# chunhualiao/Smith-Waterman

Measured on AMD Instinct MI355X. Metric: GCUPS (DP cell updates/s) on NxN random DNA pair, higher is better.
Workload: dtype int32; 1 GPU; 16384x16384 random DNA pair (reference generator, seed 1+rank), linear gap 3/-3/-2, int32 H + int32 P written to HBM, arg-max tracked; per_gpu=one pair per GPU, max_pos=268369846, max_score=11583, grid=256, column_tiles=1, strips=131, placement_held_gib=0, preheat_fills=640

## Files before the change

smith-waterman_amd/csrc/sw_api.hip:

```cpp
#include <hip/hip_runtime.h>
#include <algorithm>
#include <chrono>
#include <cstdio>
#include <cstdlib>
#include <cstring>
#include <iterator>
#include <map>
#include <mutex>
#include <string>
#include <thread>
#include <vector>
#include "sw_kernels.h"
#include "sw_plan.h"

namespace swh { void set_err(const char* fmt, ...); }
extern "C" int sw_place_pair_ratio(void* d_X, size_t xbytes, void* d_Y, size_t ybytes, float* ratio, float* ms_together);
using swh::set_err;

#define HIP_TRY(expr)                                                                 \
    do {                                                                              \
        hipError_t e_ = (expr);                                                       \
        if (e_ != hipSuccess) {                                                       \
            set_err("%s failed: %s (%s:%d)", #expr, hipGetErrorString(e_), __FILE__, __LINE__); \
            return SW_EDEVICE;                                                        \
        }                                                                             \
    } while (0)

struct DevState {
    std::mutex mu;
    bool any = false;
    hipStream_t last_stream = nullptr;
    hipEvent_t ev = nullptr;
    int concurrent_ok = 0;
};
static DevState g_dev[64];

struct sw_ctx {
    int device = 0;
    int num_cus = 256;
    unsigned epoch = 0;
    unsigned long long* d_edge = nullptr;
    size_t edge_cap = 0;
    unsigned long long* d_key = nullptr;
    unsigned long long* d_keys = nullptr; size_t keys_cap = 0;
    unsigned char* d_cb = nullptr;
    size_t cb_cap = 0;
    unsigned int* d_edge4 = nullptr;
    size_t edge4_cap = 0;
    unsigned epoch8 = 0;
    unsigned char* d_alpha = nullptr;
    unsigned int* d_part = nullptr;
    unsigned int* d_sync = nullptr;
    unsigned char* d_priv = nullptr; size_t priv_cap = 0;
    int64_t opt_place_hold_gib = 0;
    int64_t opt_place_budget_ms = 1500;
    int place_spacer_gib = 0;
    int64_t last_place_held_gib = 0;
    float last_place_ratio = 0.f;
    bool key_dirty = false;
    bool last_fused = false;
    swp::PlanOptions opt;
    swp::FillPlan last_plan;
    int64_t last_grid = 0;
    int s2_per_cu = 0;
    int64_t opt_xcd_order = 0;
    int64_t opt_pace_ps = 0;
    int64_t opt_dbg_ptr = 0;
    int64_t opt_band_wait_ms = 20000;
    unsigned char* d_bcodes = nullptr; size_t bcodes_cap = 0;
    int* d_bnd = nullptr; size_t bnd_cap = 0;
    int64_t opt_batch_lds = 0;
    int64_t last_batch_kernel = 0;
    signed char* d_sprof = nullptr; size_t sprof_cap = 0;
    int* d_sbnd = nullptr; size_t sbnd_cap = 0;
    swk::SearchItem* d_sitems = nullptr; swk::SearchItem* h_sitems = nullptr; size_t sitems_cap = 0;
    hipEvent_t sitems_ev = nullptr;
    unsigned int* d_sctr = nullptr;
    int64_t last_search_grid = 0;
    int search_per_cu[swp::kSearchKernels] = {};
    bool search_per_cu_known = false;
    bool xcd_round_robin = false;
    std::map<void*, void*> out_base;
    std::map<void*, float> pair_ratio;
};

template <typename K> struct Indexed { int index; K k; };
template <typename K, size_t N> constexpr bool at_their_indices(const Indexed<K> (&t)[N]) {
    for (size_t i = 0; i < N; ++i)
        if (t[i].index != (int)i) return false;
    return true;
}

extern "C" {

int sw_create(int device, sw_ctx** out) {
    if (!out) { set_err("sw_create: out is NULL"); return SW_EINVAL; }
    int n = 0;
    if (hipGetDeviceCount(&n) != hipSuccess || n <= 0) { set_err("sw_create: no HIP device"); return SW_ENODEV; }
    if (device < 0 || device >= n) { set_err("sw_create: device %d out of range (%d)", device, n); return SW_EINVAL; }
    HIP_TRY(hipSetDevice(device));
    sw_ctx* c = new sw_ctx();
    c->device = device;
    hipDeviceProp_t prop;
    HIP_TRY(hipGetDeviceProperties(&prop, device));
    c->num_cus = prop.multiProcessorCount;
    HIP_TRY(hipMalloc((void**)&c->d_key, 64));
    HIP_TRY(hipMemset(c->d_key, 0, 64));
    HIP_TRY(hipMalloc((void**)&c->d_alpha, 2048));
    HIP_TRY(hipMemset(c->d_alpha, 0, 2048));
    HIP_TRY(hipMalloc((void**)&c->d_part, 2048 * 32));
    HIP_TRY(hipMalloc((void**)&c->d_sync, 256));
    HIP_TRY(hipMemset(c->d_sync, 0, 256));
    if (c->num_cus == 256) {
        unsigned int h[256];
        hipLaunchKernelGGL(swk::sw_xcc_probe, dim3(256), dim3(768), 0, nullptr, c->d_part);
        if (hipMemcpy(h, c->d_part, sizeof h, hipMemcpyDeviceToHost) == hipSuccess) {
            c->xcd_round_robin = true;
            for (int i = 0; i < 256; ++i) c->xcd_round_robin = c->xcd_round_robin && h[i] == (unsigned)(i & 7);
        } else {
            (void)hipGetLastError();
        }
    }
    *out = c;
    return SW_OK;
}

void sw_destroy(sw_ctx* c) {
    if (!c) return;
    (void)hipSetDevice(c->device);
    if (c->d_edge) (void)hipFree(c->d_edge);
    if (c->d_key) (void)hipFree(c->d_key);
    if (c->d_cb) (void)hipFree(c->d_cb);
    if (c->d_edge4) (void)hipFree(c->d_edge4);
    if (c->d_alpha) (void)hipFree(c->d_alpha);
    if (c->d_part) (void)hipFree(c->d_part);
    if (c->d_sync) (void)hipFree(c->d_sync);
    if (c->d_priv) (void)hipFree(c->d_priv);
    if (c->d_keys) (void)hipFree(c->d_keys);
    if (c->d_bcodes) (void)hipFree(c->d_bcodes);
    if (c->d_bnd) (void)hipFree(c->d_bnd);
    if (c->sitems_ev) { (void)hipEventSynchronize(c->sitems_ev); (void)hipEventDestroy(c->sitems_ev); }
    if (c->d_sprof) (void)hipFree(c->d_sprof);
    if (c->d_sbnd) (void)hipFree(c->d_sbnd);
    if (c->d_sitems) (void)hipFree(c->d_sitems);
    if (c->h_sitems) (void)hipHostFree(c->h_sitems);
    if (c->d_sctr) (void)hipFree(c->d_sctr);
    delete c;
}

int sw_set_option(sw_ctx* c, const char* name, int64_t v) {
    if (!c || !name) { set_err("sw_set_option: bad argument"); return SW_EINVAL; }
    if (!strcmp(name, "waves_per_block")) {
        if (v != 0 && v != 1 && v != 2 && v != 4 && v != 8) { set_err("waves_per_block must be 1,2,4,8"); return SW_EINVAL; }
        c->opt.waves_per_block = v ? v : 4;
        return SW_OK;
    }
    if (!strcmp(name, "max_blocks")) { c->opt.max_blocks = v < 0 ? 0 : v; return SW_OK; }
    if (!strcmp(name, "strips_per_group")) { c->opt.strips_per_group = v; return SW_OK; }
    if (!strcmp(name, "consumers")) { c->opt.consumers = v; return SW_OK; }
    if (!strcmp(name, "debug_flags")) { c->opt.debug_flags = v; return SW_OK; }
    if (!strcmp(name, "xcd_chain")) { c->opt.xcd_chain = v; return SW_OK; }
    if (!strcmp(name, "filler_hop_ps")) { c->opt.filler_hop_ps = v < 0 ? 0 : v; return SW_OK; }
    if (!strcmp(name, "filler_tau_ps")) { c->opt.filler_tau_ps = v < 1000 ? 1000 : v; return SW_OK; }
    if (!strcmp(name, "filler_bw_gbs")) { c->opt.filler_bw_gbs = v < 100 ? 100 : v; return SW_OK; }
    if (!strcmp(name, "pace_ps")) { c->opt_pace_ps = v; return SW_OK; }
    if (!strcmp(name, "store_policy")) { if (v < 0 || v > 2) return SW_EINVAL; c->opt.store_policy = v; return SW_OK; }
    if (!strcmp(name, "xcd_order")) { c->opt_xcd_order = v ? 1 : 0; return SW_OK; }
    if (!strcmp(name, "importers")) { if (v < 0 || v > 8) return SW_EINVAL; c->opt.importers = v; return SW_OK; }
    if (!strcmp(name, "debug_buf")) { c->opt_dbg_ptr = v; return SW_OK; }
    if (!strcmp(name, "batch_lds")) { c->opt_batch_lds = v < 0 ? 0 : v; return SW_OK; }
    if (!strcmp(name, "band_wait_ms")) { c->opt_band_wait_ms = v > 0 ? v : 20000; return SW_OK; }
    if (!strcmp(name, "placement_budget_ms")) { c->opt_place_budget_ms = v > 0 ? v : 1500; return SW_OK; }
    if (!strcmp(name, "placement_hold_gib")) { c->opt_place_hold_gib = v < 0 ? 0 : (v > 128 ? 128 : v); return SW_OK; }
    if (!strcmp(name, "probe_foreign_pairs")) { c->opt.probe_foreign_pairs = v ? 1 : 0; return SW_OK; }
    if (!strcmp(name, "s2w")) { if (v != 0 && v != 126 && v != 110) return SW_EINVAL; c->opt.s2w = v; return SW_OK; }
    if (!strcmp(name, "split_blk")) { c->opt.split_blk = v > 0 ? v : 0; return SW_OK; }
    if (!strcmp(name, "split_from")) { c->opt.split_from = v > 0 ? v : 0; return SW_OK; }
    if (!strcmp(name, "debug_epoch8")) { c->epoch8 = (unsigned)(v & 255); return SW_OK; }
    if (!strcmp(name, "engine")) {
        if (v != 0 && v != 1) { set_err("engine must be 0 (systolic) or 1 (strip_scan)"); return SW_EINVAL; }
        c->opt.engine = v;
        return SW_OK;
    }
    set_err("sw_set_option: unknown option '%s'", name);
    return SW_EINVAL;
}

int64_t sw_get_option(sw_ctx* c, const char* name) {
    if (!c || !name) return -1;
    if (!strcmp(name, "waves_per_block")) return c->opt.waves_per_block;
    if (!strcmp(name, "max_blocks")) return c->opt.max_blocks;
    if (!strcmp(name, "engine")) return c->opt.engine;
    if (!strcmp(name, "strips_per_group")) return c->opt.strips_per_group;
    if (!strcmp(name, "consumers")) return c->opt.consumers;
    if (!strcmp(name, "store_policy")) return c->opt.store_policy;
    if (!strcmp(name, "xcd_order")) return c->opt_xcd_order;
    if (!strcmp(name, "importers")) return c->opt.importers;
    if (!strcmp(name, "pace_ps")) return c->opt_pace_ps;
    if (!strcmp(name, "band_wait_ms")) return c->opt_band_wait_ms;
    if (!strcmp(name, "num_cus")) return c->num_cus;
    if (!strcmp(name, "debug_edge4_ptr")) return (int64_t)(uintptr_t)c->d_edge4;
    if (!strcmp(name, "debug_edge4_cap")) return (int64_t)c->edge4_cap;
    if (!strcmp(name, "last_grid")) return c->last_grid;
    const swp::TilePlan& last_tile = c->last_plan.tile[c->last_plan.ntile - 1];
    if (!strcmp(name, "last_strips")) return c->last_plan.S;
    if (!strcmp(name, "last_strips2")) return last_tile.strips;
    if (!strcmp(name, "last_scouts")) return last_tile.nscout;
    if (!strcmp(name, "last_xcd_mode")) return last_tile.xcd_mode;
    if (!strcmp(name, "last_tiles")) return c->last_plan.ntile;
    if (!strcmp(name, "last_split_from")) return last_tile.split_blk ? last_tile.split_from : 0;
    if (!strcmp(name, "xcd_round_robin")) return c->xcd_round_robin ? 1 : 0;
    if (!strcmp(name, "last_batch_kernel")) return c->last_batch_kernel;
    if (!strcmp(name, "last_search_grid")) return c->last_search_grid;
    if (!strcmp(name, "placement_budget_ms")) return c->opt_place_budget_ms;
    if (!strcmp(name, "placement_hold_gib")) return c->opt_place_hold_gib;
    if (!strcmp(name, "probe_foreign_pairs")) return c->opt.probe_foreign_pairs;
    if (!strcmp(name, "last_placement_held_gib")) return c->last_place_held_gib;
    if (!strcmp(name, "last_placement_ratio_x1000")) return (int64_t)(c->last_place_ratio * 1000.f);
    return -1;
}

static int check_dims(int64_t cols, int64_t rows, const sw_scores* sc, int64_t gc = -1, int64_t gr = -1) {
    if (gc < cols) gc = cols;
    if (gr < rows) gr = rows;
    if (cols < 0 || rows < 0 || cols > swk::SW_MAX_DIM || rows > swk::SW_MAX_DIM || gc > swk::SW_MAX_DIM || gr > swk::SW_MAX_DIM) {
        set_err("dimensions out of range: cols=%lld rows=%lld (max %lld)", (long long)cols, (long long)rows,
                (long long)swk::SW_MAX_DIM);
        return SW_EINVAL;
    }
    if (sc->gap > 0) { set_err("gap score must be <= 0 (got %d)", sc->gap); return SW_EINVAL; }
    if (sc->match < 0) { set_err("match score must be >= 0 (got %d)", sc->match); return SW_EINVAL; }
    if (sc->mismatch > sc->match) { set_err("mismatch score must not exceed the match score"); return SW_EINVAL; }
    const int64_t lo = std::min(gc, gr);
    const int64_t gmax = (int64_t)sc->match * lo + (int64_t)(-sc->gap) * (rows + cols + 2);
    const int64_t step = std::max<int64_t>(std::llabs((int64_t)sc->mismatch), (int64_t)sc->match) + 2 * (int64_t)(-sc->gap);
    if (gmax + step >= (1ll << 31) || step >= (1ll << 24) || (int64_t)sc->match * lo >= (1ll << 24)) {
        set_err("scores too large for this problem size (32-bit cell / 24-bit arg-max key)");
        return SW_EINVAL;
    }
    return SW_OK;
}

struct FillJob {
    const char* d_a; int64_t cols; const char* d_b; int64_t rows;
    void* d_H; int h_elem_bytes; void* d_P; int64_t stride;
    const int32_t* d_top; const int32_t* d_left; int32_t* d_right;
    int64_t npairs; int64_t a_pstride, b_pstride, hp_pstride;
    unsigned long long* d_keys;
    int p_elem_bytes = 4;
    const unsigned long long* d_top_gran = nullptr; unsigned long long* d_bot_gran = nullptr; unsigned int* d_bot_done = nullptr;
    unsigned int top_tag = 0, bot_tag = 0;
    int reserve_cus = 0;
    bool concurrent = false;
    int64_t total_rows = 0;
    bool zero_key = false;
    sw_result* d_result = nullptr;
};

static int order_after_previous_fill(DevState& d, hipStream_t stream, bool allow_concurrent) {
    if (d.any && d.last_stream != stream && !allow_concurrent && d.ev) HIP_TRY(hipStreamWaitEvent(stream, d.ev, 0));
    return SW_OK;
}

struct DevOrder {
    std::unique_lock<std::mutex> lk;
    DevState& d;
    hipStream_t stream;
    int rc;
    DevOrder(sw_ctx* c, hipStream_t st, bool concurrent) : lk(g_dev[c->device & 63].mu), d(g_dev[c->device & 63]), stream(st) {
        rc = order_after_previous_fill(d, stream, concurrent);
    }
    ~DevOrder() {
        if (!d.ev && hipEventCreateWithFlags(&d.ev, hipEventDisableTiming) != hipSuccess) { d.ev = nullptr; (void)hipGetLastError(); }
        if (d.ev && hipEventRecord(d.ev, stream) == hipSuccess) { d.any = true; d.last_stream = stream; }
        else { (void)hipGetLastError(); d.any = false; }
    }
};

static int grow_workspace(void** buf, size_t& cap, size_t need, size_t elem, size_t slack, hipStream_t stream, bool& fresh) {
    fresh = false;
    if (need <= cap) return SW_OK;
    HIP_TRY(hipStreamSynchronize(stream));
    if (*buf) HIP_TRY(hipFree(*buf));
    *buf = nullptr; cap = 0;
    const size_t bytes = need * elem + slack;
    if (hipMalloc(buf, bytes) != hipSuccess) { set_err("workspace allocation of %zu bytes failed", bytes); return SW_ENOMEM; }
    cap = need; fresh = true;
    return SW_OK;
}

static int ensure_workspaces(sw_ctx* c, const swp::FillPlan& f, hipStream_t stream) {
    bool fresh = false;
    if (int rc = grow_workspace((void**)&c->d_edge, c->edge_cap, f.edge_need, 8, 0, stream, fresh)) return rc;
    if (fresh) { HIP_TRY(hipMemsetAsync(c->d_edge, 0, c->edge_cap * 8, stream)); c->epoch = 0; }
    if (int rc = grow_workspace((void**)&c->d_cb, c->cb_cap, f.cb_need, 4, 64, stream, fresh)) return rc;
    if (int rc = grow_workspace((void**)&c->d_edge4, c->edge4_cap, f.edge4_need, 4, 0, stream, fresh)) return rc;
    if (fresh) c->epoch8 = 255;
    return grow_workspace((void**)&c->d_priv, c->priv_cap, f.priv_need, 1, 0, stream, fresh);
}

static unsigned next_gbias(sw_ctx* c, hipStream_t stream) {
    if (++c->epoch8 >= (unsigned)((c->opt.debug_flags & swk::DBG_EPOCH8_WRAP_EARLY) ? 4 : 256)) {
        const unsigned nb = (unsigned)std::max<size_t>(1, std::min<size_t>((c->edge4_cap + 255) / 256, 2048));
        hipLaunchKernelGGL(swk::sw_wipe_u32, dim3(nb), dim3(256), 0, stream, c->d_edge4, c->edge4_cap);
        c->epoch8 = 1;
    }
    return (c->epoch8 << 24) | 0x10000u;
}

static swp::DeviceFacts device_facts(const sw_ctx* c) {
    swp::DeviceFacts dev;
    dev.num_cus = c->num_cus; dev.xcd_round_robin = c->xcd_round_robin; dev.s2_per_cu = c->s2_per_cu;
    std::copy(std::begin(c->search_per_cu), std::end(c->search_per_cu), dev.search_per_cu);
    return dev;
}

static int plan_for(sw_ctx* c, const swp::PlanJob& pj, swp::FillPlan& plan) {
    if (c->opt.engine == 0 && c->s2_per_cu < 1)
        HIP_TRY(hipOccupancyMaxActiveBlocksPerMultiprocessor(&c->s2_per_cu, swk::sw_systolic2<6, false>, 768, 0));
    plan = swp::plan_fill(pj, device_facts(c), c->opt);
    return SW_OK;
}

using SystolicKernel = void (*)(const unsigned char*, const unsigned char*, const unsigned char*, swk::FillParams);
static const struct { int ns, nc; SystolicKernel h32, h64; } kSystolic[] = {
    {2, 2, swk::sw_systolic<int32_t, 2, 2>, swk::sw_systolic<int64_t, 2, 2>}, {2, 3, swk::sw_systolic<int32_t, 2, 3>, swk::sw_systolic<int64_t, 2, 3>},
    {2, 4, swk::sw_systolic<int32_t, 2, 4>, swk::sw_systolic<int64_t, 2, 4>}, {1, 2, swk::sw_systolic<int32_t, 1, 2>, swk::sw_systolic<int64_t, 1, 2>},
    {1, 3, swk::sw_systolic<int32_t, 1, 3>, swk::sw_systolic<int64_t, 1, 3>}, {1, 4, swk::sw_systolic<int32_t, 1, 4>, swk::sw_systolic<int64_t, 1, 4>},
    {1, 6, swk::sw_systolic<int32_t, 1, 6>, swk::sw_systolic<int64_t, 1, 6>}, {1, 7, swk::sw_systolic<int32_t, 1, 7>, swk::sw_systolic<int64_t, 1, 7>},
};
using Systolic2Kernel = void (*)(const unsigned char*, const unsigned char*, swk::FillParams);
static const Systolic2Kernel kSystolic2[4][2] = {
    {swk::sw_systolic2<4, false>, swk::sw_systolic2<4, true>}, {swk::sw_systolic2<5, false>, swk::sw_systolic2<5, true>},
    {swk::sw_systolic2<6, false>, swk::sw_systolic2<6, true>}, {swk::sw_systolic2<7, false>, swk::sw_systolic2<7, true>},
};

static swp::PlanJob plan_job(const FillJob& j, const sw_scores* sc) {
    swp::PlanJob pj;
    pj.cols = j.cols; pj.rows = j.rows; pj.npairs = j.npairs; pj.full_stride = j.stride == j.cols + 1;
    pj.h_elem_bytes = j.h_elem_bytes; pj.p_elem_bytes = j.p_elem_bytes; pj.has_H = j.d_H; pj.has_P = j.d_P;
    pj.has_top = j.d_top; pj.has_left = j.d_left; pj.has_right = j.d_right; pj.has_top_gran = j.d_top_gran; pj.has_bot_gran = j.d_bot_gran;
    pj.has_result = j.d_result; pj.total_rows = j.total_rows; pj.reserve_cus = j.reserve_cus;
    pj.h_aligned = ((uintptr_t)j.d_H & (j.h_elem_bytes == 8 ? 15u : 7u)) == 0; pj.p_aligned = ((uintptr_t)j.d_P & 7u) == 0;
    pj.match = sc->match; pj.mismatch = sc->mismatch; pj.gap = sc->gap;
    return pj;
}

static int launch_fill(sw_ctx* c, const sw_scores* sc, const FillJob& j, hipStream_t stream) {
    const int64_t cols = j.cols, rows = j.rows;
    const bool systolic = (c->opt.engine == 0);
    c->last_fused = false;
    const bool tile_features = j.d_left || j.d_right || j.stride != cols + 1 || j.npairs != 1 || !j.d_H || !j.d_P || j.d_top_gran || j.d_bot_gran;
    if (!systolic && tile_features) { set_err("tiles / batches / bands / matrix-less fills need the systolic engine (engine 0)"); return SW_EINVAL; }
    if (j.p_elem_bytes == 1 && !systolic) { set_err("compact (int8) P needs the systolic engine"); return SW_EINVAL; }
    if (((uintptr_t)j.d_b & 15) != 0 || (j.b_pstride & 15) != 0) { set_err("d_b (and the batch stride of b) must be 16-byte aligned"); return SW_EINVAL; }
    swp::PlanJob pj = plan_job(j, sc);
    auto known = j.d_P ? c->pair_ratio.find(j.d_P) : c->pair_ratio.end();
    if (known != c->pair_ratio.end()) pj.pair_ratio = known->second;
    swp::FillPlan plan;
    if (int rc = plan_for(c, pj, plan)) return rc;
    if (plan.probe_pair_class) {
        float r = 0.f, ms = 0.f;
        if (c->pair_ratio.size() >= 64) c->pair_ratio.clear();
        if (hipStreamSynchronize(stream) == hipSuccess && sw_place_pair_ratio(j.d_H, plan.h_bytes, j.d_P, plan.p_bytes, &r, &ms) == SW_OK) {
            c->pair_ratio[j.d_P] = pj.pair_ratio = r;
            if (int rc = plan_for(c, pj, plan)) return rc;
        }
    }
    const auto* one_col = systolic ? std::find_if(std::begin(kSystolic), std::end(kSystolic), [&](const auto& k) { return k.ns == plan.NS && k.nc == plan.NC; })
                                   : std::end(kSystolic);
    if (systolic && one_col == std::end(kSystolic)) { set_err("unsupported strips_per_group/consumers combination %d/%d", plan.NS, plan.NC); return SW_EINVAL; }
    if (int rc = ensure_workspaces(c, plan, stream)) return rc;
    if (++c->epoch >= 4096) {
        HIP_TRY(hipMemsetAsync(c->d_edge, 0, c->edge_cap * 8, stream));
        c->epoch = 1;
    }
    c->last_plan = plan;
    const int64_t S = plan.S;
    swk::FillParams p;
    memset(&p, 0, sizeof p);
    p.cols = cols; p.rows = rows; p.M = j.stride;
    p.H = j.d_H; p.P = (int32_t*)j.d_P; p.top = j.d_top; p.left = j.d_left; p.right = j.d_right;
    p.top_gran = j.d_top_gran; p.bot_gran = j.d_bot_gran; p.bot_done = j.d_bot_done; p.top_tag = j.top_tag; p.bot_tag = j.bot_tag;
    p.top_wait_ticks = (unsigned)std::min<int64_t>(0x7fffffff, c->opt_band_wait_ms * 100000 >> 10);
    p.mm = sc->match - 2 * sc->gap; p.xm = sc->mismatch - 2 * sc->gap; p.ngap = -sc->gap;
    p.edge = c->d_edge; p.tag_base = c->epoch << 20;
    p.result_key = j.d_keys; p.abort_flag = (unsigned int*)(c->d_key + 1);
    p.nstrips = (int)S;
    p.debug_flags = (int)c->opt.debug_flags;
    p.pace_ps = (int)c->opt_pace_ps;
    p.store_nt = plan.store_nt;
    p.xcd_order = (int)c->opt_xcd_order;
    p.dbg = (unsigned long long*)(uintptr_t)c->opt_dbg_ptr;
    p.npairs = (int)j.npairs; p.store_hp = (j.d_H || j.d_P) ? 1 : 0;
    p.p_bytes = j.p_elem_bytes;
    p.a_pstride = j.a_pstride; p.b_pstride = j.b_pstride; p.hp_pstride = j.hp_pstride;
    p.edge_pstride = S * (rows + 1);
    const unsigned char* ua = (const unsigned char*)j.d_a;
    const unsigned char* ub = (const unsigned char*)j.d_b;
    if (!systolic) {
        c->key_dirty = true;
        c->last_grid = plan.grid;
        if (j.h_elem_bytes == 4)
            hipLaunchKernelGGL((swk::sw_strip_scan<int32_t, 16>), dim3(plan.grid), dim3(plan.threads), 0, stream, ua, ub, p);
        else
            hipLaunchKernelGGL((swk::sw_strip_scan<int64_t, 16>), dim3(plan.grid), dim3(plan.threads), 0, stream, ua, ub, p);
        HIP_TRY(hipGetLastError());
        return SW_OK;
    }
    const size_t cb16 = ((c->cb_cap + 15) / 16) * 16;
    unsigned short* d_cb16 = (unsigned short*)(c->d_cb + cb16);
    unsigned char* d_cbc = c->d_cb + cb16 + ((2 * c->cb_cap + 15) / 16) * 16;
    if (plan.perm) {
        p.edge4 = c->d_edge4; p.e4stride = plan.e4stride; p.edge4_pstride = S * plan.e4stride;
        p.gbias = next_gbias(c, stream);
    }
    p.bcode = d_cbc;
    p.atab = c->d_alpha + 64;
    p.phi_base = plan.fast ? (int)S - 1 : -1;
    p.bfront = (int)plan.bfront;
    p.bpad16 = d_cb16;
    p.bpad8 = c->d_cb;
    p.bpad_pstride = plan.per;
    if (plan.two_cols) {
        if (c->key_dirty) { HIP_TRY(hipMemsetAsync(c->d_key, 0, 16, stream)); c->key_dirty = false; }
        for (int64_t tile = 0; tile < plan.ntile; ++tile) {
            const swp::TilePlan& t = plan.tile[tile];
            swk::FillParams p2 = p;
            p2.nstrips = (int)t.strips; p2.cols = t.cols; p2.h_bytes = j.h_elem_bytes; p2.s2w = plan.W2; p2.store_nt = t.store_nt;
            p2.alpha_a = ua; p2.alpha_cols = cols;
            p2.idx_off = t.c0; p2.final_launch = tile + 1 == plan.ntile ? 1 : 0;
            if (plan.ntile > 1) {
                p2.H = (char*)j.d_H + t.c0 * 4; p2.P = (int32_t*)((char*)j.d_P + t.c0 * 4);
                p2.tile_left = tile ? (const int32_t*)j.d_H + t.c0 : nullptr;
                if (tile) p2.gbias = next_gbias(c, stream);
            }
            p2.nscout = t.nscout; p2.scout_double = t.scout_double; p2.xcd_mode = t.xcd_mode;
            p2.split_blk = t.split_blk; p2.split_from = t.split_from; p2.split_extra = t.split_extra;
            p2.filler_end_steps = t.filler_end_steps; p2.filler_full_steps = t.filler_full_steps;
            p2.filler_hop_ps = t.filler_hop_ps; p2.filler_tau_ps = t.filler_tau_ps; p2.filler_bw_gbs = t.filler_bw_gbs;
            p2.sync = c->d_sync; p2.priv = c->d_priv; p2.priv_stride = plan.priv_stride;
            p2.bpad16_w = d_cb16; p2.bpad8_w = c->d_cb; p2.bcode_w = d_cbc; p2.atab_w = c->d_alpha + 64;
            p2.result = j.d_result; p2.skip_row0 = (j.d_top || j.d_top_gran) ? 1 : 0;
            hipLaunchKernelGGL(kSystolic2[t.consumers - 4][plan.W2 == 110], dim3(t.grid), dim3(768), 0, stream, ua + t.c0, ub, p2);
        }
        p.skip_if_perm = 1;
        p.sync = c->d_sync; p.atab_w = c->d_alpha + 64; p.result = j.d_result; p.final_launch = 1;
        c->last_fused = true;
    } else {
        const int64_t total = (cols + rows) * j.npairs;
        const unsigned nscan = (unsigned)std::max<int64_t>(1, std::min<int64_t>((total + 1023) / 1024, 2048));
        hipLaunchKernelGGL(swk::sw_prep_scan, dim3(nscan), dim3(256), 0, stream, ua, cols, j.a_pstride, ub, rows, j.b_pstride, j.npairs, c->d_part);
        const unsigned npad = (unsigned)((plan.per + 255) / 256);
        hipLaunchKernelGGL(swk::sw_prep_code, dim3(npad, (unsigned)j.npairs), dim3(256), 0, stream, ub, rows, plan.bfront, j.b_pstride, c->d_cb, d_cb16,
                           d_cbc, (const unsigned int*)c->d_part, (int)nscan, c->d_alpha + 64, plan.per, (int)npad, (void*)nullptr, j.h_elem_bytes,
                           (void*)nullptr, j.p_elem_bytes, cols + 1, rows + 1, 0, j.zero_key ? j.d_keys : nullptr);
        c->key_dirty = true;
    }
    const SystolicKernel kern = j.h_elem_bytes == 4 ? one_col->h32 : one_col->h64;
    int per_cu = 0;
    HIP_TRY(hipOccupancyMaxActiveBlocksPerMultiprocessor(&per_cu, kern, plan.threads, 0));
    if (per_cu < 1) { set_err("the fill kernel does not fit a CU on this device"); return SW_EDEVICE; }
    c->last_grid = std::min<int64_t>(plan.grid, (int64_t)per_cu * c->num_cus);
    hipLaunchKernelGGL(kern, dim3((unsigned)c->last_grid), dim3(plan.threads), 0, stream, ua, ub, (const unsigned char*)c->d_cb, p);
    HIP_TRY(hipGetLastError());
    return SW_OK;
}

static const sw_scores kDefaultScores = {3, -3, -2};

static int fill_one(sw_ctx* c, const sw_scores* scores, FillJob j, int64_t gcols, int64_t grows, sw_result* d_result, void* stream_,
                    const char* who) {
    const sw_scores* sc = scores ? scores : &kDefaultScores;
    const int64_t cols = j.cols, rows = j.rows;
    if (!c || !d_result || (j.h_elem_bytes != 4 && j.h_elem_bytes != 8) || (j.p_elem_bytes != 4 && j.p_elem_bytes != 1) ||
        j.stride < cols + 1) {
        set_err("%s: bad argument", who);
        return SW_EINVAL;
    }
    if (int rc = check_dims(cols, rows, sc, gcols, grows)) return rc;
    if ((cols > 0 && !j.d_a) || (rows > 0 && !j.d_b)) { set_err("%s: NULL sequence", who); return SW_EINVAL; }
    hipStream_t stream = (hipStream_t)stream_;
    HIP_TRY(hipSetDevice(c->device));
    DevOrder order(c, stream, j.concurrent);
    if (order.rc) return order.rc;
    j.d_keys = c->d_key;
    j.d_result = d_result;
    j.zero_key = c->opt.engine == 0 && cols > 0 && rows > 0;
    if (!j.zero_key) { HIP_TRY(hipMemsetAsync(c->d_key, 0, 16, stream)); c->key_dirty = true; }
    c->last_fused = false;
    if (cols == 0 || rows == 0) {
        if (j.stride != cols + 1 || j.d_left || j.d_right || j.d_top_gran || j.d_bot_gran) { set_err("%s: empty tiles / bands are not supported", who); return SW_EINVAL; }
        const int64_t M = cols + 1;
        if (j.d_H) HIP_TRY(hipMemsetAsync(j.d_H, 0, (size_t)(M * (rows + 1)) * j.h_elem_bytes, stream));
        if (j.d_P) HIP_TRY(hipMemsetAsync(j.d_P, 0, (size_t)(M * (rows + 1)) * j.p_elem_bytes, stream));
        if (j.d_H && j.d_top && j.h_elem_bytes == 4) HIP_TRY(hipMemcpyAsync(j.d_H, j.d_top, (size_t)M * 4, hipMemcpyDeviceToDevice, stream));
        if (j.d_H && j.d_top && j.h_elem_bytes == 8) { set_err("top halo with an empty int64 band is unsupported"); return SW_EINVAL; }
    } else {
        if (int rc = launch_fill(c, sc, j, stream)) return rc;
    }
    if (!c->last_fused) hipLaunchKernelGGL(swk::sw_finalize, dim3(1), dim3(64), 0, stream, c->d_key, (const unsigned int*)(c->d_key + 1), d_result, 1);
    HIP_TRY(hipGetLastError());
    return SW_OK;
}

static FillJob make_job(const char* d_a, int64_t cols, const char* d_b, int64_t rows, void* d_H, int h_elem_bytes, void* d_P, int p_elem_bytes,
                        int64_t row_stride, const int32_t* d_top, const int32_t* d_left, int32_t* d_right) {
    FillJob j = {d_a, cols, d_b, rows, d_H, h_elem_bytes, d_P, row_stride, d_top, d_left, d_right, 1, 0, 0, 0, nullptr};
    j.p_elem_bytes = p_elem_bytes;
    return j;
}

int sw_fill_tile_device(sw_ctx* c, const char* d_a, int64_t cols, const char* d_b, int64_t rows, const sw_scores* scores,
                        void* d_H, int h_elem_bytes, int32_t* d_P, int64_t row_stride, const int32_t* d_top,
                        const int32_t* d_left, int32_t* d_right, sw_result* d_result, void* stream_) {
    if (!d_H || !d_P) { set_err("sw_fill_tile_device: bad argument"); return SW_EINVAL; }
    return fill_one(c, scores, make_job(d_a, cols, d_b, rows, d_H, h_elem_bytes, d_P, 4, row_stride, d_top, d_left, d_right), -1, -1, d_result,
                    stream_, "sw_fill_tile_device");
}

int sw_fill_device(sw_ctx* c, const char* d_a, int64_t cols, const char* d_b, int64_t rows, const sw_scores* scores,
                   void* d_H, int h_elem_bytes, int32_t* d_P, const int32_t* d_top, sw_result* d_result, void* stream_) {
    if (!d_H || !d_P) { set_err("sw_fill_device: bad argument"); return SW_EINVAL; }
    return fill_one(c, scores, make_job(d_a, cols, d_b, rows, d_H, h_elem_bytes, d_P, 4, cols + 1, d_top, nullptr, nullptr), -1, -1, d_result,
                    stream_, "sw_fill_device");
}

int sw_fill_device_ex(sw_ctx* c, const char* d_a, int64_t cols, const char* d_b, int64_t rows, const sw_scores* scores,
                      void* d_H, int h_elem_bytes, void* d_P, int p_elem_bytes, const int32_t* d_top, sw_result* d_result,
                      void* stream_) {
    return fill_one(c, scores, make_job(d_a, cols, d_b, rows, d_H, h_elem_bytes, d_P, p_elem_bytes, cols + 1, d_top, nullptr, nullptr), -1, -1,
                    d_result, stream_, "sw_fill_device_ex");
}

int sw_fill_band_device(sw_ctx* c, const char* d_a, int64_t cols, const char* d_b, int64_t rows, int64_t total_rows,
                        const sw_scores* scores, void* d_H, int h_elem_bytes, void* d_P, int p_elem_bytes,
                        const uint64_t* d_top_gran, uint32_t top_tag, uint64_t* d_bot_gran, uint32_t bot_tag, uint32_t* d_bot_done,
                        int reserve_cus, int concurrent, sw_result* d_result, void* stream_) {
    if ((d_top_gran && top_tag == 0) || (d_bot_gran && bot_tag == 0) || (d_bot_done && !d_bot_gran) || reserve_cus < 0 || total_rows < rows) {
        set_err("sw_fill_band_device: bad argument");
        return SW_EINVAL;
    }
    if (c && c->opt.engine != 0) { set_err("sw_fill_band_device needs the systolic engine"); return SW_EINVAL; }
    FillJob j = make_job(d_a, cols, d_b, rows, d_H, h_elem_bytes, d_P, p_elem_bytes, cols + 1, nullptr, nullptr, nullptr);
    j.d_top_gran = (const unsigned long long*)d_top_gran; j.d_bot_gran = (unsigned long long*)d_bot_gran; j.d_bot_done = d_bot_done;
    j.top_tag = top_tag; j.bot_tag = bot_tag; j.reserve_cus = reserve_cus; j.concurrent = concurrent != 0; j.total_rows = total_rows;
    return fill_one(c, scores, j, cols, total_rows, d_result, stream_, "sw_fill_band_device");
}

using BatchKernel = void (*)(swk::BatchParams);
static constexpr Indexed<BatchKernel> kBatch[] = {
    {swp::batch_wave_index(4, 0), swk::sw_batch_wave<4, 0>}, {swp::batch_wave_index(4, 1), swk::sw_batch_wave<4, 1>},
    {swp::batch_wave_index(4, 4), swk::sw_batch_wave<4, 4>}, {swp::batch_wave_index(8, 0), swk::sw_batch_wave<8, 0>},
    {swp::batch_wave_index(8, 1), swk::sw_batch_wave<8, 1>}, {swp::batch_wave_index(8, 4), swk::sw_batch_wave<8, 4>},
    {swp::batch_wave_index(16, 0), swk::sw_batch_wave<16, 0>}, {swp::batch_wave_index(16, 1), swk::sw_batch_wave<16, 1>},
    {swp::batch_wave_index(16, 4), swk::sw_batch_wave<16, 4>},
    {swp::batch_wave16_index(false, false, false), swk::sw_batch_wave16<false, false, false>},
    {swp::batch_wave16_index(false, false, true), swk::sw_batch_wave16<false, false, true>},
    {swp::batch_wave16_index(false, true, false), swk::sw_batch_wave16<false, true, false>},
    {swp::batch_wave16_index(false, true, true), swk::sw_batch_wave16<false, true, true>},
    {swp::batch_wave16_index(true, false, false), swk::sw_batch_wave16<true, false, false>},
    {swp::batch_wave16_index(true, false, true), swk::sw_batch_wave16<true, false, true>},
    {swp::batch_wave16_index(true, true, false), swk::sw_batch_wave16<true, true, false>},
    {swp::batch_wave16_index(true, true, true), swk::sw_batch_wave16<true, true, true>},
};
static_assert(std::size(kBatch) == swp::kBatchKernels && at_their_indices(kBatch));

static int batch_one_pair_per_wave(sw_ctx* c, const swp::BatchPlan& plan, const char* d_a, int64_t a_stride, int64_t cols, const char* d_b,
                                   int64_t b_stride, int64_t rows, int64_t npairs, const sw_scores* sc, int32_t* d_H, void* d_P, int p_elem_bytes,
                                   sw_result* d_results, hipStream_t stream) {
    bool fresh = false;
    if (int rc = grow_workspace((void**)&c->d_bcodes, c->bcodes_cap, plan.bcodes_need, 1, 64, stream, fresh)) return rc;
    if (int rc = grow_workspace((void**)&c->d_bnd, c->bnd_cap, plan.bnd_need, 4, 0, stream, fresh)) return rc;
    const unsigned char* ua = (const unsigned char*)d_a;
    const unsigned char* ub = (const unsigned char*)d_b;
    hipLaunchKernelGGL(swk::sw_prep_scan, dim3((unsigned)plan.scan_blocks), dim3(256), 0, stream, ua, cols, a_stride, ub, rows, b_stride, npairs, c->d_part);
    hipLaunchKernelGGL(swk::sw_prep_reduce, dim3(1), dim3(256), 0, stream, c->d_part, plan.scan_blocks);
    if (plan.bnd_need) HIP_TRY(hipMemsetAsync(c->d_bnd, 0, plan.bnd_need * 4, stream));
    const int64_t cells = (cols + 1) * (rows + 1);
    const int pb = d_P ? p_elem_bytes : 0;
    unsigned int nletters = 0;
    for (int64_t k0 = 0; k0 < npairs; k0 += plan.chunk) {
        const int64_t n = std::min(plan.chunk, npairs - k0);
        hipLaunchKernelGGL(swk::sw_batch_codes, dim3((unsigned)plan.codes_blocks, (unsigned)std::min<int64_t>(n, 65535)), dim3(256), 0, stream,
                           ub + k0 * b_stride, rows, b_stride, c->d_bcodes, plan.per, plan.front, (const unsigned int*)c->d_part, 1, c->d_alpha + 64, n);
        HIP_TRY(hipGetLastError());
        if (k0 == 0) {
            HIP_TRY(hipMemcpyAsync(&nletters, c->d_alpha + 64 + 256, 4, hipMemcpyDeviceToHost, stream));
            HIP_TRY(hipStreamSynchronize(stream));
        }
        const int k = swp::batch_kernel(plan, nletters, n, pb);
        if (k < 0) return 1;
        swk::BatchParams bp;
        memset(&bp, 0, sizeof bp);
        bp.a = ua + k0 * a_stride; bp.a_pstride = a_stride; bp.cols = cols;
        bp.bcode = c->d_bcodes; bp.bcode_pstride = plan.per; bp.bfront = plan.front;
        bp.rows = rows; bp.npairs = n; bp.atab = c->d_alpha + 64;
        bp.H = d_H ? d_H + k0 * cells : nullptr;
        bp.P = d_P ? (void*)((char*)d_P + k0 * cells * p_elem_bytes) : nullptr;
        bp.hp_pstride = cells;
        bp.match = sc->match; bp.mismatch = sc->mismatch; bp.ngap = -sc->gap;
        bp.bnd = c->d_bnd; bp.bnd_pstride = plan.bnd_per;
        bp.results = d_results + k0;
        bp.debug = (int)(c->opt.debug_flags & swk::DBG_BATCH_MASK);
        const bool two = k >= swp::kBatchWave16;
        const int64_t per_block = two ? 8 : 4;
        hipLaunchKernelGGL(kBatch[k].k, dim3((unsigned)((n + per_block - 1) / per_block)), dim3(256), two ? 0 : (size_t)c->opt_batch_lds, stream, bp);
        HIP_TRY(hipGetLastError());
        if (two) c->last_batch_kernel = 2;
    }
    if (c->last_batch_kernel != 2) c->last_batch_kernel = 1;
    c->last_grid = plan.grid; c->last_plan.S = plan.nstrips;
    return SW_OK;
}

int sw_fill_band_reserve(sw_ctx* c, int64_t cols, int64_t rows, int64_t total_rows, const sw_scores* scores, int h_elem_bytes, int p_elem_bytes, int want_h,
                         void* stream_) {
    const sw_scores* sc = scores ? scores : &kDefaultScores;
    if (!c || cols <= 0 || rows <= 0) { set_err("sw_fill_band_reserve: bad argument"); return SW_EINVAL; }
    if (c->opt.engine != 0) { set_err("sw_fill_band_reserve needs the systolic engine"); return SW_EINVAL; }
    if (int rc = check_dims(cols, rows, sc, cols, total_rows)) return rc;
    HIP_TRY(hipSetDevice(c->device));
    swp::PlanJob pj;
    pj.cols = cols; pj.rows = rows; pj.total_rows = total_rows; pj.h_elem_bytes = h_elem_bytes; pj.p_elem_bytes = p_elem_bytes; pj.has_H = want_h != 0;
    pj.has_top_gran = pj.has_bot_gran = true;
    pj.match = sc->match; pj.mismatch = sc->mismatch; pj.gap = sc->gap;
    swp::FillPlan plan;
    if (int rc = plan_for(c, pj, plan)) return rc;
    std::unique_lock<std::mutex> lk(g_dev[c->device & 63].mu);
    if (int rc = ensure_workspaces(c, plan, (hipStream_t)stream_)) return rc;
    HIP_TRY(hipStreamSynchronize((hipStream_t)stream_));
    return SW_OK;
}

int sw_batch_device_ex(sw_ctx* c, const char* d_a, int64_t a_stride, int64_t cols, const char* d_b, int64_t b_stride, int64_t rows,
                       int64_t npairs, const sw_scores* scores, int32_t* d_H, void* d_P, int p_elem_bytes, sw_result* d_results,
                       void* stream_) {
    const sw_scores* sc = scores ? scores : &kDefaultScores;
    if (!c || !d_a || !d_b || !d_results || npairs <= 0 || cols <= 0 || rows <= 0 || a_stride < cols || b_stride < rows ||
        (p_elem_bytes != 4 && p_elem_bytes != 1)) {
        set_err("sw_batch_device: bad argument");
        return SW_EINVAL;
    }
    if (c->opt.engine != 0) { set_err("sw_batch_device needs the systolic engine"); return SW_EINVAL; }
    if (int rc = check_dims(cols, rows, sc)) return rc;
    hipStream_t stream = (hipStream_t)stream_;
    HIP_TRY(hipSetDevice(c->device));
    DevOrder order(c, stream, false);
    if (order.rc) return order.rc;
    swp::BatchJob bj;
    bj.cols = cols; bj.rows = rows; bj.npairs = npairs; bj.has_H = d_H; bj.has_P = d_P; bj.p_elem_bytes = p_elem_bytes;
    bj.match = sc->match; bj.mismatch = sc->mismatch; bj.gap = sc->gap;
    const swp::BatchPlan plan = swp::plan_batch(bj, c->opt);
    c->last_batch_kernel = 0;
    if (plan.wave) {
        int rc = batch_one_pair_per_wave(c, plan, d_a, a_stride, cols, d_b, b_stride, rows, npairs, sc, d_H, d_P, p_elem_bytes, d_results, stream);
        if (rc != 1) return rc;
    }
    bool fresh = false;
    if (int rc = grow_workspace((void**)&c->d_keys, c->keys_cap, (size_t)plan.single_chunk, 8, 0, stream, fresh)) return rc;
    HIP_TRY(hipMemsetAsync(c->d_key, 0, 16, stream));
    c->key_dirty = true;
    const int64_t cells = (cols + 1) * (rows + 1);
    for (int64_t k0 = 0; k0 < npairs; k0 += plan.single_chunk) {
        const int64_t n = std::min(plan.single_chunk, npairs - k0);
        HIP_TRY(hipMemsetAsync(c->d_keys, 0, (size_t)n * 8, stream));
        FillJob j = {d_a + k0 * a_stride, cols, d_b + k0 * b_stride, rows, d_H ? (void*)(d_H + k0 * cells) : nullptr, 4,
                     d_P ? (void*)((char*)d_P + k0 * cells * p_elem_bytes) : nullptr, cols + 1, nullptr, nullptr, nullptr, n, a_stride, b_stride,
                     cells, c->d_keys};
        j.p_elem_bytes = p_elem_bytes;
        if (int rc = launch_fill(c, sc, j, stream)) return rc;
        hipLaunchKernelGGL(swk::sw_finalize, dim3((unsigned)((n + 63) / 64)), dim3(64), 0, stream, c->d_keys,
                           (const unsigned int*)(c->d_key + 1), d_results + k0, (int)n);
        HIP_TRY(hipGetLastError());
    }
    return SW_OK;
}
int sw_batch_device(sw_ctx* c, const char* d_a, int64_t a_stride, int64_t cols, const char* d_b, int64_t b_stride, int64_t rows,
                    int64_t npairs, const sw_scores* scores, int32_t* d_H, int32_t* d_P, sw_result* d_results, void* stream_) {
    return sw_batch_device_ex(c, d_a, a_stride, cols, d_b, b_stride, rows, npairs, scores, d_H, d_P, 4, d_results, stream_);
}

using SearchKernel = void (*)(swk::SearchParams);
static constexpr Indexed<SearchKernel> kSearch[] = {
    {swp::search_kernel_index(4, false), swk::sw_search_wave<4, false>}, {swp::search_kernel_index(4, true), swk::sw_search_wave<4, true>},
    {swp::search_kernel_index(8, false), swk::sw_search_wave<8, false>}, {swp::search_kernel_index(8, true), swk::sw_search_wave<8, true>},
    {swp::search_kernel_index(16, false), swk::sw_search_wave<16, false>}, {swp::search_kernel_index(16, true), swk::sw_search_wave<16, true>},
};
static_assert(std::size(kSearch) == swp::kSearchKernels && at_their_indices(kSearch));

static int grow_schedule(sw_ctx* c, size_t need, hipStream_t stream) {
    if (need <= c->sitems_cap) return SW_OK;
    HIP_TRY(hipStreamSynchronize(stream));
    if (c->d_sitems) HIP_TRY(hipFree(c->d_sitems));
    if (c->h_sitems) HIP_TRY(hipHostFree(c->h_sitems));
    c->d_sitems = nullptr; c->h_sitems = nullptr; c->sitems_cap = 0;
    if (hipMalloc((void**)&c->d_sitems, need * sizeof(swk::SearchItem)) != hipSuccess ||
        hipHostMalloc((void**)&c->h_sitems, need * sizeof(swk::SearchItem), 0) != hipSuccess) {
        set_err("sw_search_device: workspace allocation failed");
        return SW_ENOMEM;
    }
    c->sitems_cap = need;
    return SW_OK;
}

int sw_search_device(sw_ctx* c, const char* d_query, int64_t qlen, const char* d_db, const int64_t* offsets, int64_t ntargets,
                     const sw_scores* scores, sw_result* d_results, void* stream_) {
    const sw_scores* sc = scores ? scores : &kDefaultScores;
    if (!c || !d_query || !d_db || !offsets || !d_results || ntargets < 0) { set_err("sw_search_device: NULL pointer or negative target count"); return SW_EINVAL; }
    if (qlen < 1 || qlen > swk::SW_MAX_DIM) { set_err("sw_search_device: query length %lld out of range 1..%lld", (long long)qlen, (long long)swk::SW_MAX_DIM); return SW_EINVAL; }
    if (offsets[0] < 0) { set_err("sw_search_device: offsets[0] = %lld is negative", (long long)offsets[0]); return SW_EINVAL; }
    int64_t maxlen = 0, nonempty = 0;
    for (int64_t k = 0; k < ntargets; ++k) {
        const int64_t len = offsets[k + 1] - offsets[k];
        if (len < 0) { set_err("sw_search_device: offsets decrease at target %lld", (long long)k); return SW_EINVAL; }
        if (len > swk::SW_MAX_DIM) { set_err("sw_search_device: target %lld has length %lld (max %lld)", (long long)k, (long long)len, (long long)swk::SW_MAX_DIM); return SW_EINVAL; }
        maxlen = std::max(maxlen, len);
        nonempty += len > 0;
    }
    if (int rc = check_dims(qlen, maxlen, sc)) return rc;
    if (ntargets == 0) return SW_OK;
    hipStream_t stream = (hipStream_t)stream_;
    HIP_TRY(hipSetDevice(c->device));
    DevOrder order(c, stream, false);
    if (order.rc) return order.rc;
    HIP_TRY(hipMemsetAsync(d_results, 0, (size_t)ntargets * sizeof(sw_result), stream));
    if (nonempty == 0) return SW_OK;
    if (!c->search_per_cu_known) {
        for (int k = 0; k < swp::kSearchKernels; ++k) HIP_TRY(hipOccupancyMaxActiveBlocksPerMultiprocessor(&c->search_per_cu[k], kSearch[k].k, 256, 0));
        c->search_per_cu_known = true;
    }
    swp::SearchJob sj;
    sj.qlen = qlen; sj.maxlen = maxlen; sj.ntargets = nonempty; sj.match = sc->match; sj.mismatch = sc->mismatch; sj.gap = sc->gap;
    const swp::SearchPlan plan = swp::plan_search(sj, device_facts(c));
    if (c->search_per_cu[plan.kernel] < 1) { set_err("the search kernel does not fit a CU on this device"); return SW_EDEVICE; }
    if (c->sitems_ev) HIP_TRY(hipEventSynchronize(c->sitems_ev));
    else HIP_TRY(hipEventCreateWithFlags(&c->sitems_ev, hipEventDisableTiming));
    bool fresh = false;
    if (int rc = grow_schedule(c, (size_t)nonempty, stream)) return rc;
    if (int rc = grow_workspace((void**)&c->d_sprof, c->sprof_cap, plan.prof_need, 1, 0, stream, fresh)) return rc;
    if (int rc = grow_workspace((void**)&c->d_sbnd, c->sbnd_cap, plan.bnd_need, 4, 0, stream, fresh)) return rc;
    if (!c->d_sctr) HIP_TRY(hipMalloc((void**)&c->d_sctr, 64));
// ... 444 lines not shown
```

smith-waterman_amd/csrc/sw_debug.h:

```cpp
#pragma once

namespace swk {

enum DebugFlag : int {
    DBG_NO_STORES = 1 << 0,
    DBG_PRODUCER_ONLY = 1 << 1,
    DBG_GENERIC_PRODUCER = 1 << 2,
    DBG_SKIP_STRIP1 = 1 << 3,
    DBG_NO_PERM = 1 << 4,
    DBG_NO_POLL_BACKOFF = 1 << 5,
    DBG_WAVE_PLACEMENT = 1 << 6,
    DBG_BLOCK_STAMPS = 1 << 7,
    DBG_NO_CONSUMER_LOOP = 1 << 8,
    DBG_EDGE_DUMP = 1 << 9,
    DBG_EPOCH8_WRAP_EARLY = 1 << 10,
    DBG_POISON_HALO = 1 << 11,
    DBG_ONE_IMPORTER = 1 << 12,
    DBG_PROGRESS_FORM = 1 << 13,
    DBG_NO_TWO_COLUMNS = 1 << 14,
    DBG_FORCE_TWO_COLUMNS = 1 << 15,
    DBG_BATCH_SINGLE_PAIR = 1 << 16,
    DBG_NO_SCOUTS = 1 << 17,
    DBG_BATCH_NO_WAVE16 = 1 << 18,
    DBG_NO_TILES = 1 << 19,
    DBG_NO_SPLIT = 1 << 20,
    DBG_BATCH_NO_PACKED_P = 1 << 21,
    DBG_S2_SCOUTS_NO_EXPORT = 1 << 21,
    DBG_S2_SYNTH_HALO = 1 << 22,
    DBG_NO_XCD_DEALING = 1 << 23,
    DBG_S2_IMPORTERS = 3 << 24,
    DBG_NO_PACING = 1 << 27,
};
constexpr int DBG_S2_IMPORTERS_SHIFT = 24;
constexpr int DBG_BATCH_MASK = DBG_NO_STORES | DBG_PRODUCER_ONLY | DBG_GENERIC_PRODUCER;

}
```

smith-waterman_amd/csrc/sw_filler_producer.inc:

```
__device__ __forceinline__ int producer_perm2(u32 palo, u32 pahi, u32 pblo, u32 pbhi, u32 ngap_v, u32 wA, u32 wB, u32 voff, u32 z0, u32 ga1, u32 gb1, u32 ta,
                                              u32 tb, u32 expoff, u32 expoff_local, const unsigned char* cbase, u32 hb, u32 lowb, u32 cons_addr, u32 right_addr,
                                              u32 prog_addr, int UT, int kc, int kr, sw_i32x4p erc, int (&polls)[2]) {
    int status;
    const int kc32 = kc + 32, kr32 = kr + 32;
    asm volatile(
        "s_setprio 3\n\t"
        "s_mov_b32 %[status], 0\n\t"
        "s_mov_b32 s94, 0\n\t"
        "s_mov_b32 s95, 0\n\t"
        "s_mov_b32 s88, 1\n\t"
        "s_mov_b32 s90, 0\n\t"
        "s_mov_b32 s91, 0\n\t"
        "s_mov_b32 s75, 0\n\t"
        "s_mov_b32 s76, %[e0]\n\t"
        "s_mov_b32 s77, %[e1]\n\t"
        "s_mov_b32 s78, %[e2]\n\t"
        "s_mov_b32 s79, %[e3]\n\t"
        "s_mov_b64 s[72:73], 1\n\t"
        "s_mov_b64 s[92:93], %[cbase]\n\t"
        "v_mov_b32 v96, %[voff]\n\t"
        "v_mov_b32 v97, %[expoff]\n\t"
        "v_mov_b32 v39, %[consaddr]\n\t"
        "v_mov_b32 v30, %[rightaddr]\n\t"
        "v_mov_b32 v31, %[progaddr]\n\t"
        "v_mov_b32 v29, 0\n\t"
        "v_mov_b32 v79, %[ga1]\n\t"
        "v_mov_b32 v95, %[gb1]\n\t"
        "v_mov_b32 v117, %[ta]\n\t"
        "v_mov_b32 v119, %[tb]\n\t"
        "v_mov_b32 v121, %[z0]\n\t"
        "v_mov_b32 v64, %[ga1]\n\tv_mov_b32 v65, %[ga1]\n\tv_mov_b32 v66, %[ga1]\n\tv_mov_b32 v67, %[ga1]\n\t"
        "v_mov_b32 v68, %[ga1]\n\tv_mov_b32 v69, %[ga1]\n\tv_mov_b32 v70, %[ga1]\n\tv_mov_b32 v71, %[ga1]\n\t"
        "v_mov_b32 v72, %[ga1]\n\tv_mov_b32 v73, %[ga1]\n\tv_mov_b32 v74, %[ga1]\n\tv_mov_b32 v75, %[ga1]\n\t"
        "v_mov_b32 v76, %[ga1]\n\tv_mov_b32 v77, %[ga1]\n\tv_mov_b32 v78, %[ga1]\n\t"
        "v_mov_b32 v124, 0\n\tv_mov_b32 v125, 0\n\tv_mov_b32 v126, 0\n\tv_mov_b32 v127, 0\n\t"
        "v_mov_b32 v32, 0\n\tv_mov_b32 v33, 0\n\tv_mov_b32 v34, 0\n\tv_mov_b32 v35, 0\n\tv_mov_b32 v36, 0\n\t"
        "v_mov_b32 v103, 0\n\tv_mov_b32 v107, 0\n\tv_mov_b32 v111, 0\n\tv_mov_b32 v115, 0\n\t"
        "s_nop 4\n\t"
        "global_load_dwordx4 v[48:51], v96, s[92:93] offset:1\n\t"
        "global_load_dwordx4 v[52:55], v96, s[92:93] offset:2\n\t"
        "global_load_dwordx4 v[56:59], v96, s[92:93] offset:17\n\t"
        "global_load_dwordx4 v[60:63], v96, s[92:93] offset:18\n\t"
        "s_waitcnt vmcnt(0)\n"
        "Lchunk_%=:\n\t"
        P2_BPCHECK("A", "%[kc]", "%[kr]")
        "v_add_u32 v99, s90, %[wa]\n\t"
        "v_add_u32 v123, s90, %[wb]\n\t"
        "v_mov_b32 v98, %[hb]\n\t"
        "v_add_u32 v98, s91, v98\n\t"
        "v_mov_b32 v27, %[lowb]\n\t"
        "s_add_i32 s91, s91, 256\n\t"
        "s_and_b32 s91, s91, 4095\n\t"
        "v_cndmask_b32_e64 v98, v27, v98, s[72:73]\n\t"
        "v_mov_b32 v28, %[hb]\n\t"
        "v_add_u32 v28, s91, v28\n\t"
        "s_nop 0\n\t"
        "v_cndmask_b32_e64 v28, v27, v28, s[72:73]\n\t"
        P2_BLOCK(0, "v48", "v49", "v50", "v51", "v52", "v53", "v54", "v55", "v[48:51]", "v[52:55]", "33", "34", "0", "16", "32", "48",
                 "v98 offset:64", "v98 offset:80", "v98 offset:96", "v98 offset:112", "")
        P2_BLOCK(16, "v56", "v57", "v58", "v59", "v60", "v61", "v62", "v63", "v[56:59]", "v[60:63]", "49", "50", "64", "80", "96", "112",
                 "v98 offset:128", "v98 offset:144", "v98 offset:160", "v98 offset:176", P2_BPFETCH)
        P2_BPCHECK("B", "%[kc32]", "%[kr32]")
        P2_BLOCK(32, "v48", "v49", "v50", "v51", "v52", "v53", "v54", "v55", "v[48:51]", "v[52:55]", "65", "66", "128", "144", "160", "176",
                 "v98 offset:192", "v98 offset:208", "v98 offset:224", "v98 offset:240", "")
        P2_BLOCK(48, "v56", "v57", "v58", "v59", "v60", "v61", "v62", "v63", "v[56:59]", "v[60:63]", "81", "82", "192", "208", "224", "240",
                 "v28", "v28 offset:16", "v28 offset:32", "v28 offset:48", P2_BPFETCH)
        "s_add_i32 s90, s90, 256\n\t"
        "s_and_b32 s90, s90, 1023\n\t"
        "s_add_i32 s75, s75, 256\n\t"
        "s_add_u32 s92, s92, 64\n\t"
        "s_addc_u32 s93, s93, 0\n\t"
        "s_add_i32 s88, s88, 64\n\t"
        "s_cmp_gt_i32 s88, %[ut]\n\t"
        "s_cbranch_scc0 Lchunk_%=\n\t"
        "s_branch Lexit_%=\n"
        P2_SLOW(0, "0", "16", "32", "48") P2_SLOW(16, "64", "80", "96", "112") P2_SLOW(32, "128", "144", "160", "176") P2_SLOW(48, "192", "208", "224", "240")
        "Lfail_%=:\n\t"
        "s_mov_b32 %[status], 1\n"
        "Lexit_%=:\n\t"
        "s_setprio 0\n\t"
        "s_waitcnt vmcnt(0) lgkmcnt(0)\n\t"
        "s_mov_b32 %[nbp], s94\n\t"
        "s_mov_b32 %[nhalo], s95\n\t"
        : [status] "=&s"(status), [nbp] "=&s"(polls[0]), [nhalo] "=&s"(polls[1])
        : [palo] "v"(palo), [pahi] "v"(pahi), [pblo] "v"(pblo), [pbhi] "v"(pbhi), [ngap] "v"(ngap_v), [wa] "v"(wA), [wb] "v"(wB), [voff] "v"(voff),
          [z0] "v"(z0), [ga1] "v"(ga1), [gb1] "v"(gb1), [ta] "v"(ta), [tb] "v"(tb), [expoff] "v"(expoff), [expoffl] "v"(expoff_local), [cbase] "s"(cbase), [hb] "s"(hb), [lowb] "s"(lowb),
          [consaddr] "s"(cons_addr), [rightaddr] "s"(right_addr), [progaddr] "s"(prog_addr), [ut] "s"(UT), [kc] "s"(kc), [kr] "s"(kr), [kc32] "s"(kc32),
          [kr32] "s"(kr32), [e0] "s"(erc.x), [e1] "s"(erc.y), [e2] "s"(erc.z), [e3] "s"(erc.w)
        : "vcc", "scc", "memory", "s72", "s73", "s75", "s76", "s77", "s78", "s79", "s85", "s86", "s87", "s88", "s89", "s90", "s91", "s92", "s93", "s94", "s95",
          "v27", "v28", "v29", "v30", "v31", "v32", "v33", "v34", "v35", "v36", "v37", "v38", "v39", "v40", "v41", "v42", "v43", "v44", "v45", "v46", "v47", "v48",
          "v49", "v50", "v51", "v52", "v53", "v54", "v55", "v56", "v57", "v58", "v59", "v60", "v61", "v62", "v63", "v64", "v65", "v66", "v67", "v68", "v69", "v70",
          "v71", "v72", "v73", "v74", "v75", "v76", "v77", "v78", "v79", "v80", "v81", "v82", "v83", "v84", "v85", "v86", "v87", "v88", "v89", "v90", "v91", "v92",
          "v93", "v94", "v95", "v96", "v97", "v98", "v99", "v100", "v101", "v102", "v103", "v104", "v105", "v106", "v107", "v108", "v109", "v110", "v111",
          "v112", "v113", "v114", "v115", "v116", "v117", "v118", "v119", "v120", "v121", "v122", "v123", "v124", "v125", "v126", "v127");
    return status;
}
```

smith-waterman_amd/csrc/sw_kernels.h:

```cpp
#pragma once
#include <hip/hip_runtime.h>
#include <stdint.h>
#include "../../include/swhip.h"
#include "sw_plan.h"

namespace swk {

constexpr unsigned long long SW_KEY_IDX_MASK = (1ull << 40) - 1;
constexpr int64_t SW_MAX_DIM = (1 << 20) - 1;

struct FillParams {
    int64_t cols, rows, M;
    void* H;
    int32_t* P;
    const int32_t* top;
    const int32_t* left;
    int32_t* right;
    int npairs;
    int store_hp;
    int64_t a_pstride, b_pstride, bpad_pstride, hp_pstride, edge_pstride;
    int32_t mm, xm, ngap;
    unsigned long long* edge;
    unsigned int tag_base;
    unsigned long long* result_key;
    unsigned int* abort_flag;
    int phi_base;
    int bfront;
    const unsigned short* bpad16;
    const unsigned char* bpad8;
    unsigned long long* dbg;
    int p_bytes;
    int store_nt;
    int xcd_order;
    int pace_ps;
    int debug_flags;
    int nstrips;
    const unsigned long long* top_gran;
    unsigned long long* bot_gran;
    unsigned int* bot_done;
    unsigned int top_tag, bot_tag;
    unsigned int top_wait_ticks;
    const unsigned char* bcode;
    const unsigned char* atab;
    unsigned int* edge4;
    int64_t e4stride, edge4_pstride;
    unsigned int gbias;
    int skip_if_perm;
    int h_bytes;
    int scout_double;
    int nscout;
    int filler_hop_ps, filler_tau_ps, filler_bw_gbs;
    int xcd_mode;
    unsigned int* sync;
    unsigned char* priv;
    int64_t priv_stride;
    unsigned short* bpad16_w;
    unsigned char* bpad8_w; unsigned char* bcode_w; unsigned char* atab_w;
    sw_result* result;
    int skip_row0;
    const int32_t* tile_left;
    int64_t idx_off;
    int final_launch;
    const unsigned char* alpha_a;
    int64_t alpha_cols;
    int split_blk, split_from;
    int split_extra;
    int filler_end_steps;
    int filler_full_steps;
    int s2w;
};
constexpr int SW_XTAB_OFF = 448;
constexpr int SW_PERM_PAD = -100;

struct BatchParams {
    const unsigned char* a; int64_t a_pstride, cols;
    const unsigned char* bcode; int64_t bcode_pstride; int bfront;
    int64_t rows, npairs;
    const unsigned char* atab;
    int32_t* H; void* P;
    int64_t hp_pstride;
    int match, mismatch, ngap;
    int* bnd; int64_t bnd_pstride;
    sw_result* results;
    int debug;
};
__global__ void sw_batch_codes(const unsigned char* b, int64_t rows, int64_t b_pstride, unsigned char* bcode, int64_t per, int front,
                               const unsigned int* part, int npart, unsigned char* atab, int64_t npairs);
template <int C, int PB>
__global__ void sw_batch_wave(BatchParams p);
template <bool LE4, bool K12, bool PB1>
__global__ void sw_batch_wave16(BatchParams p);

struct SearchParams {
    const unsigned char* db;
    const SearchItem* items; int64_t nitems;
    const signed char* prof; int64_t qpad;
    int64_t qlen;
    int match, mismatch, ngap;
    int* bnd; int64_t bnd_per;
    unsigned int* counter;
    sw_result* results;
};
__global__ void sw_search_profile(const unsigned char* q, int64_t qlen, int64_t qpad, signed char* prof, int match, int mismatch, int wide);
template <int C, bool WIDE>
__global__ void sw_search_wave(SearchParams p);

template <typename HT, int B>
__global__ void sw_strip_scan(const unsigned char* a, const unsigned char* b, FillParams p);
template <typename HT, int NS, int NC>
__global__ void sw_systolic(const unsigned char* a, const unsigned char* b, const unsigned char* bpad, FillParams p);
__global__ void sw_wipe_u32(unsigned int* buf, size_t n);
template <int NC, bool OV>
__global__ void sw_systolic2(const unsigned char* a, const unsigned char* b, FillParams p);
__global__ void sw_prep_scan(const unsigned char* a, int64_t cols, int64_t a_pstride, const unsigned char* b, int64_t rows, int64_t b_pstride, int64_t npairs,
                             unsigned int* part);
__global__ void sw_prep_code(const unsigned char* b, int64_t rows, int64_t front, int64_t b_pstride, unsigned char* bpad, unsigned short* bpad16,
                             unsigned char* bcode, const unsigned int* part, int npart, unsigned char* atab, int64_t per, int npad, void* H, int h_bytes,
                             void* P, int p_bytes, int64_t M, int64_t rows1, int skip_row0, unsigned long long* key);
__global__ void sw_xcc_probe(unsigned int* xcc_of_block);
__global__ void sw_prep_reduce(unsigned int* part, int npart);
__global__ void sw_finalize(const unsigned long long* key, const unsigned int* abort_flag, sw_result* res, int n);
template <typename PT>
__global__ void sw_traceback_wave(PT* P, int64_t M, int64_t rows1, int64_t pstride, int64_t start_pos, int64_t* paths, int64_t cap, sw_result* res,
                                  int64_t* stop, unsigned int* pathbits);
template <typename T> __global__ void sw_row_checksums(const T* X, int64_t m, unsigned long long* cs);
__global__ void sw_widen_p8(const signed char* P8, int32_t* P32, size_t n);
struct P2Cells { unsigned char v; };
template <typename PT> __global__ void sw_pack_p2(const PT* P, unsigned char* P2, unsigned int* bits, size_t n);
__global__ void sw_unpack_p2(const unsigned char* P2, const unsigned int* bits, int32_t* P32, size_t n);

}
```

smith-waterman_amd/csrc/sw_plan.cpp:

```cpp
#include "sw_plan.h"
#include <algorithm>
#include <vector>

namespace swp {

constexpr double kOneStripPerCu = 4.5;
constexpr double kChainBoundCells = 3.5e8;
constexpr double kStreamCells = 6.0e8;
constexpr double kChainSecPerStrip = 3.1e-6, kHbmBytesPerSec = 3.2e12;
constexpr int64_t kScoutStrips = 170;
constexpr double kOneClassCells = 2.0e8;
constexpr float kOneClassRatio = 1.7f;
constexpr int64_t kTileStrips = 160;
constexpr double kTileHopSec = 2.4e-6, kTileRowSec = 26e-9, kTileBytesPerSec = 3.0e12;
constexpr double kClassicHopSec = 7.6e-6, kClassicRowSec = 35e-9, kClassicBytesPerSec = 3.3e12;
constexpr double kTileGain = 0.98;
constexpr int64_t kXcdChainStrips = 384;
constexpr double kScoutLeadSec = 21.5e-9;
constexpr int64_t kSplitRows = 4096;

constexpr int64_t kC4Cols = 256, kC8Cols = 512;
constexpr int64_t kBndSlackRows = 160;
constexpr int64_t kWaveSlackRows = 132;
constexpr double kWaveMatrixBytes = 2147483648.0;
constexpr int kWaveScore = 127;
constexpr unsigned kWaveLetters = 8, kLE4Letters = 4;
constexpr int kCodesFront = 64;
constexpr int64_t kCodesTail = 80 + 72;
constexpr int64_t kBatchWorkspaceBytes = 1ll << 30;
constexpr int64_t kScanLetters = 4096, kScanBlocks = 2048, kCodesBlocks = 64;
constexpr int64_t kWave16Score = 32000, kWave16Rows = 65000;
constexpr int64_t kKeyedScore = 4096;
constexpr int64_t kSingleChunk = 4096;
constexpr int64_t kSearchBndBytes = 1ll << 30;
constexpr int64_t kProfileBlocks = 4096;

namespace {

struct Deal { bool fits = true; int scouts = 0, doubles = 0; };
Deal deal_per_xcd(int64_t S2, bool last_strip_scout) {
    Deal r;
    for (int x = 0; x < 8 && r.fits; ++x) {
        const int nf = (int)(S2 / 8) + (x < (int)(S2 % 8) ? 1 : 0), ns = (x ? nf : nf - 1) + (last_strip_scout && x == 7 ? 1 : 0);
        const int ndx = std::max(0, ns - (32 - nf));
        r.fits = nf <= 31 && 2 * ndx <= ns;
        r.scouts += ns - ndx; r.doubles += ndx;
    }
    return r;
}

}

FillPlan plan_fill(const PlanJob& j, const DeviceFacts& dev, const PlanOptions& o) {
    using namespace swk;
    FillPlan f;
    const int64_t cols = j.cols, rows = j.rows;
    const bool systolic = o.engine == 0;
    f.engine = systolic ? 0 : 1;
    const int64_t S = f.S = systolic ? (cols + 62) / 63 : (cols + 63) / 64;
    f.edge_need = (size_t)S * (size_t)(rows + 1) * (size_t)j.npairs;
    f.h_bytes = (size_t)(cols + 1) * (size_t)(rows + 1) * (size_t)j.h_elem_bytes;
    f.p_bytes = (size_t)(cols + 1) * (size_t)(rows + 1) * (size_t)j.p_elem_bytes;
    f.store_nt = o.store_policy == 2 || (o.store_policy == 0 && (double)cols * (double)rows * (double)j.npairs <= kStreamCells);
    if (!systolic) {
        const int wpb = (int)o.waves_per_block;
        const int64_t maxb = o.max_blocks > 0 ? o.max_blocks : 2ll * dev.num_cus;
        f.grid = (int)std::max<int64_t>(1, std::min<int64_t>((S + wpb - 1) / wpb, maxb));
        f.threads = 64 * wpb;
        return f;
    }
    int NS = (int)o.strips_per_group, NC = (int)o.consumers;
    if (NS == 0) NS = (j.npairs == 1 ? (double)S <= kOneStripPerCu * dev.num_cus : (double)S * (double)j.npairs <= (double)dev.num_cus) ? 1 : 2;
    const bool chain_bound = NS == 1 && j.npairs == 1 && (double)cols * (double)rows <= kChainBoundCells;
    if (NC == 0) NC = (NS == 1) ? (chain_bound ? 4 : 6) : 4;
    f.importers = o.importers > 0 ? (int)o.importers : (chain_bound && NC <= 4 ? 4 : 2);
    if (NS == 1 && NC > 7) NC = 7;
    if (NS == 1 && NC == 5) NC = 4;
    f.NS = NS; f.NC = NC;
    f.bfront = ((S + 64 + 32 + 127) / 128) * 128;
    f.per = ((rows + f.bfront + 512 + 15) / 16) * 16;
    f.cb_need = (size_t)f.per * (size_t)j.npairs;
    const int64_t mm = j.match - 2 * j.gap, xm = j.mismatch - 2 * j.gap;
    const int64_t lo = std::min(cols, rows);
    const int64_t gmax = (int64_t)j.match * std::max<int64_t>(lo, std::min(cols, j.total_rows)) + (int64_t)(-j.gap) * (rows + cols + 2);
    const bool halo_unbounded = (j.has_top || j.has_left) && j.total_rows == 0;
    f.perm = !halo_unbounded && mm <= 127 && mm >= -127 && xm <= 127 && xm >= -127 && gmax + 0x10000 + 1024 < (1ll << 24) &&
             !(o.debug_flags & DBG_NO_PERM);
    if (f.perm) {
        f.e4stride = ((rows + S + 160 + 31) / 32) * 32;
        f.edge4_need = (size_t)S * (size_t)f.e4stride * (size_t)j.npairs;
    }
    f.fast = !j.has_top && !j.has_top_gran && j.mismatch <= 0 && !(o.debug_flags & DBG_GENERIC_PRODUCER);
    const int64_t ngroups = ((S + NS - 1) / NS) * j.npairs;
    const int64_t maxb = o.max_blocks > 0 ? o.max_blocks : std::max<int64_t>(8, (int64_t)dev.num_cus - j.reserve_cus);
    f.grid = (int)std::max<int64_t>(1, std::min<int64_t>(ngroups, maxb));
    if (NS == 1) {
        const int K = std::min<int>(9, NC + 1 + std::max(1, f.importers));
        f.threads = 64 * (K + (K - 1) / 3 + 1);
    } else {
        f.threads = 64 * (NS * (1 + NC) + 2);
    }

    const bool base_mode = j.has_H && j.has_P && j.h_elem_bytes == 4 && j.p_elem_bytes == 4 && !j.has_top && !j.has_top_gran && !j.has_bot_gran;
    const double est_chain = (double)S * kChainSecPerStrip;
    const double est_hbm = (double)(cols + 1) * (double)(rows + 1) * ((j.has_H ? (double)j.h_elem_bytes : 0.0) + (j.has_P ? (double)j.p_elem_bytes : 0.0)) / kHbmBytesPerSec;
    const bool pays = (j.has_H && j.has_P && j.p_elem_bytes == 4) || (j.has_H && j.h_elem_bytes == 8) || est_chain >= (j.has_H ? 0.5 : 2.0) * est_hbm ||
                      (o.debug_flags & DBG_FORCE_TWO_COLUMNS) ||
                      (j.has_H && j.h_elem_bytes == 4 && (!j.has_P || j.p_elem_bytes == 1) && cols % 2 == 0 && cols > 126 * kScoutStrips);
    f.two_cols = pays && f.perm && o.strips_per_group == 0 && (o.consumers == 0 || o.consumers >= 4) && j.npairs == 1 &&
                 !j.has_left && !j.has_right && j.full_stride && (rows % 16 == 0 || !j.has_bot_gran) && rows >= 1 && cols >= 1 &&
                 (base_mode || (cols % 2 == 0)) &&
                 !(o.debug_flags & (DBG_PRODUCER_ONLY | DBG_SKIP_STRIP1 | DBG_WAVE_PLACEMENT | DBG_BLOCK_STAMPS | DBG_EDGE_DUMP | DBG_NO_TWO_COLUMNS)) &&
                 dev.s2_per_cu >= 1 && j.has_result;
    f.priv_stride = ((2 * f.per + 255) / 256) * 256;
    if (!f.two_cols) return f;
    f.priv_need = (size_t)f.priv_stride * (size_t)dev.s2_per_cu * (size_t)dev.num_cus;

    const bool band_io = j.has_top || j.has_top_gran || j.has_bot_gran;
    const bool wl_fmt = !band_io && j.has_H && (!j.has_P || j.p_elem_bytes == 4 || (j.h_elem_bytes == 4 && cols % 2 == 0)) && (j.has_P || cols % 2 == 0) &&
                        j.full_stride && j.h_aligned && j.p_aligned;
    const int64_t S126 = cols <= 126 ? 1 : (cols - 126 + 125) / 126 + 1, S110 = cols <= 126 ? 1 : (cols - 126 + 109) / 110 + 1;
    bool one_class = false;
    if (j.has_P && (double)cols * (double)rows >= kOneClassCells) {
        f.probe_pair_class = j.pair_ratio == 0.f && o.probe_foreign_pairs && o.s2w == 0 && wl_fmt && S126 <= kScoutStrips;
        one_class = j.pair_ratio >= kOneClassRatio;
    }
    int64_t W2 = 126;
    if (o.s2w == 110 ? (!band_io && (cols % 2 == 0 || wl_fmt))
                     : (o.s2w == 0 && wl_fmt && (S126 > kScoutStrips || (j.h_elem_bytes == 8 && S110 > kScoutStrips) || one_class)))
        W2 = 110;
    f.W2 = (int)W2;
    const bool ov_auto = W2 == 110 && o.s2w == 0;
    auto strips_of = [&](int64_t ncols) { return ncols <= 126 ? (int64_t)1 : (ncols - 126 + W2 - 1) / W2 + 1; };
    const int64_t S2all = strips_of(cols);
    f.tstrips = S2all;
    if (S2all > kScoutStrips && base_mode && j.full_stride && j.has_result && !ov_auto && !(o.debug_flags & DBG_NO_TILES)) {
        const int64_t nt = (S2all + kTileStrips - 1) / kTileStrips, st = (S2all + nt - 1) / nt;
        const double bytes = (double)(cols + 1) * (double)(rows + 1) * 8.0;
        const double t_tiles = (double)nt * std::max((double)st * kTileHopSec + (double)(rows + 200) * kTileRowSec, bytes / (double)nt / kTileBytesPerSec);
        const double t_classic = std::max((double)S2all * kClassicHopSec + (double)rows * kClassicRowSec, bytes / kClassicBytesPerSec);
        if (t_tiles < kTileGain * t_classic) { f.ntile = nt; f.tstrips = st; }
    }
    const int64_t per_cu = dev.s2_per_cu;
    for (int64_t tile = 0; tile < f.ntile; ++tile) {
        TilePlan& t = f.tile[tile];
        t.c0 = tile * f.tstrips * W2;
        t.cols = tile + 1 == f.ntile ? cols - t.c0 : f.tstrips * W2;
        const int64_t S2 = t.strips = strips_of(t.cols);
        t.store_nt = f.store_nt;
        if (f.ntile > 1) t.store_nt = o.store_policy == 2 || (o.store_policy == 0 && (double)t.cols * (double)rows <= kStreamCells);
        if (W2 == 110 && wl_fmt && o.store_policy == 0) t.store_nt = 1;
        t.grid = (int)std::max<int64_t>(1, std::min<int64_t>(std::min<int64_t>(S2, maxb), per_cu * dev.num_cus));
        const int64_t avail = std::min<int64_t>(maxb, per_cu * dev.num_cus);
        const int64_t ndouble = std::max<int64_t>(0, 2 * S2 - 1 - avail);
        const int64_t nsc = S2 - 1 - ndouble;
        const bool scouts = S2 >= 4 && 2 * ndouble <= S2 - 1 && nsc >= 1 && !(o.debug_flags & DBG_NO_SCOUTS);
        t.nscout = scouts ? (int)nsc : 0;
        t.scout_double = scouts ? (int)ndouble : 0;
        if (scouts) t.grid = (int)(S2 + nsc);
        if (scouts && dev.xcd_round_robin && avail >= 256 && S2 >= 16 && !(o.debug_flags & DBG_NO_XCD_DEALING)) {
            const Deal d = deal_per_xcd(S2, false);
            if (d.fits) { t.xcd_mode = 1; t.nscout = d.scouts; t.scout_double = d.doubles; t.grid = 256; }
        }
        if (t.xcd_mode == 1 && (rows >= kSplitRows || o.split_blk > 0) && !j.has_top && !j.has_top_gran && !j.has_bot_gran && o.filler_hop_ps > 0 &&
            !(o.debug_flags & (DBG_NO_PACING | DBG_NO_SPLIT))) {
            const Deal d = deal_per_xcd(S2, true);
            const double hop = (double)o.filler_hop_ps * 1e-12, tf = (double)o.filler_tau_ps * 1e-12, ts = kScoutLeadSec;
            const int64_t nblk = (rows + 15) / 16;
            const int64_t sblk = (int64_t)((double)nblk * tf / (2.0 * tf - std::min(ts, tf)));
            const bool forced = o.split_blk > 0;
            if (d.fits && forced && o.split_blk < nblk) {
                t.split_blk = (int)o.split_blk; t.split_from = (int)std::max<int64_t>(1, o.split_from); t.split_extra = 1;
                t.filler_end_steps = (int)((o.split_blk * 16 + 126) / 64 * 64 + 64); t.filler_full_steps = (int)((nblk * 16 + 126) / 64 * 64 + 64);
                t.nscout = d.scouts; t.scout_double = d.doubles;
            } else if (d.fits && sblk >= 16 && sblk < nblk && rows >= kSplitRows) {
                const int64_t full_steps = (nblk * 16 + 126) / 64 * 64 + 64, end_steps = (sblk * 16 + 126) / 64 * 64 + 64;
                const double lead = ((double)full_steps - (double)end_steps) * tf / hop;
                const int64_t from = std::max<int64_t>(1, (int64_t)((double)(S2 - 1) - lead) + 1);
                if (from < S2) {
                    t.split_blk = (int)sblk; t.split_from = (int)from; t.split_extra = 1;
                    t.filler_end_steps = (int)end_steps; t.filler_full_steps = (int)full_steps;
                    t.nscout = d.scouts; t.scout_double = d.doubles;
                }
            }
        }
        const bool xcd_chain_pays = S2 >= kXcdChainStrips && W2 != 110;
        if (!scouts && dev.xcd_round_robin && t.grid >= 64 && !(o.debug_flags & DBG_NO_XCD_DEALING) &&
            (o.xcd_chain == 1 || (o.xcd_chain == 0 && xcd_chain_pays)))
            t.xcd_mode = 2;
        t.filler_hop_ps = (scouts && !(o.debug_flags & DBG_NO_PACING)) ? (int)o.filler_hop_ps : 0;
        t.filler_tau_ps = (int)o.filler_tau_ps;
        t.filler_bw_gbs = (int)o.filler_bw_gbs;
        t.consumers = o.consumers == 0 ? ((scouts || W2 == 110) ? 7 : (chain_bound ? 5 : 6)) : (int)std::min<int64_t>(7, o.consumers);
    }
    return f;
}

namespace {
int lane_columns(int64_t cols) { return cols <= kC4Cols ? 4 : cols <= kC8Cols ? 8 : 16; }
int64_t boundary_ints(int64_t nstrips, int64_t rows) { return nstrips > 1 ? ((rows + kBndSlackRows + 3) / 4) * 4 : 0; }
}

BatchPlan plan_batch(const BatchJob& j, const PlanOptions& o) {
    using namespace swk;
    BatchPlan b;
    const int64_t cols = j.cols, rows = j.rows;
    b.wave = !(o.debug_flags & DBG_BATCH_SINGLE_PAIR) && j.match <= kWaveScore && j.match >= -kWaveScore && j.mismatch <= kWaveScore &&
             j.mismatch >= -kWaveScore && (double)(rows + kWaveSlackRows) * (double)(cols + 1) * 4.0 < kWaveMatrixBytes;
    b.single_chunk = std::min(j.npairs, kSingleChunk);
    b.C = lane_columns(cols);
    b.nstrips = (cols + 64 * b.C - 1) / (64 * b.C);
    b.front = kCodesFront;
    b.per = ((rows + kCodesFront + kCodesTail + 15) / 16) * 16;
    b.bnd_per = boundary_ints(b.nstrips, rows);
    b.chunk = std::max<int64_t>(1, std::min<int64_t>(j.npairs, std::min<int64_t>(kBatchWorkspaceBytes / b.per,
                                                                                  b.bnd_per ? kBatchWorkspaceBytes / (b.bnd_per * 4) : j.npairs)));
    b.grid = (b.chunk + 3) / 4;
    b.scan_blocks = (int)std::max<int64_t>(1, std::min<int64_t>(((cols + rows) * j.npairs + kScanLetters - 1) / kScanLetters, kScanBlocks));
    b.codes_blocks = (int)std::min<int64_t>((b.per + 255) / 256, kCodesBlocks);
    b.bcodes_need = (size_t)(b.chunk * b.per);
    b.bnd_need = (size_t)(b.chunk * b.bnd_per);
    const int64_t smax = (int64_t)j.match * std::min(cols, rows);
    b.fits16 = j.npairs >= 2 && b.C == 16 && smax < kWave16Score && -j.gap < kWave16Score && rows < kWave16Rows && !(o.debug_flags & DBG_BATCH_NO_WAVE16);
    b.k12 = smax < kKeyedScore;
    b.packed16 = b.fits16 && !j.has_H && (!j.has_P || (j.p_elem_bytes == 1 && !(o.debug_flags & DBG_BATCH_NO_PACKED_P)));
    return b;
}

int batch_kernel(const BatchPlan& b, unsigned nletters, int64_t n, int p_bytes) {
    if (nletters > kWaveLetters) return -1;
    if (b.packed16 && n >= 2)
        return batch_wave16_index(nletters <= kLE4Letters, b.k12, p_bytes != 0);
    return batch_wave_index(b.C, p_bytes);
}

SearchPlan plan_search(const SearchJob& j, const DeviceFacts& dev) {
    using swk::SW_SEARCH_ROWS;
    SearchPlan s;
    s.C = lane_columns(j.qlen);
    s.wide = j.match > kWaveScore || j.mismatch < -kWaveScore;
    s.kernel = search_kernel_index(s.C, s.wide);
    s.nstrips = (j.qlen + 64 * s.C - 1) / (64 * s.C);
    s.qpad = s.nstrips * 64 * s.C;
    s.bnd_per = boundary_ints(s.nstrips, j.maxlen);
    s.grid = std::min<int64_t>((int64_t)dev.search_per_cu[s.kernel] * dev.num_cus, (j.ntargets + 3) / 4);
    if (s.bnd_per) s.grid = std::max<int64_t>(1, std::min<int64_t>(s.grid, kSearchBndBytes / (s.bnd_per * 4 * 4)));
    s.prof_need = (size_t)(SW_SEARCH_ROWS * s.qpad);
    s.prof_blocks = (int)std::min<int64_t>((SW_SEARCH_ROWS * s.qpad + 255) / 256, kProfileBlocks);
    s.bnd_need = s.bnd_per ? (size_t)(s.grid * 4 * s.bnd_per) : 0;
    return s;
}

void search_schedule(const int64_t* offsets, int64_t ntargets, swk::SearchItem* items) {
    std::vector<int64_t> order;
    order.reserve((size_t)ntargets);
    for (int64_t k = 0; k < ntargets; ++k)
        if (offsets[k + 1] > offsets[k]) order.push_back(k);
    std::stable_sort(order.begin(), order.end(), [&](int64_t x, int64_t y) { return offsets[x + 1] - offsets[x] > offsets[y + 1] - offsets[y]; });
    for (size_t i = 0; i < order.size(); ++i) {
        const int64_t k = order[i];
        items[i] = swk::SearchItem{offsets[k], k, offsets[k + 1] - offsets[k]};
    }
}

}
```

smith-waterman_amd/csrc/sw_plan.h:

```cpp
#pragma once
#include <cstddef>
#include <cstdint>
#include "sw_debug.h"

namespace swk {

constexpr int SW_SEARCH_ROWS = 257;
struct SearchItem { int64_t start, idx, len; };

}

namespace swp {

struct PlanJob {
    int64_t cols = 0, rows = 0, npairs = 1;
    bool full_stride = true;
    int h_elem_bytes = 4, p_elem_bytes = 4;
    bool has_H = true, has_P = true;
    bool has_top = false;
    bool has_left = false, has_right = false;
    bool has_top_gran = false, has_bot_gran = false;
    bool has_result = true;
    int64_t total_rows = 0;
    int reserve_cus = 0;
    bool h_aligned = true, p_aligned = true;
    int match = 3, mismatch = -3, gap = -2;
    float pair_ratio = 0.f;
};

constexpr int kSearchKernels = 6;
constexpr int search_kernel_index(int C, bool wide) { return 2 * (C / 8) + wide; }

struct DeviceFacts {
    int num_cus = 256;
    bool xcd_round_robin = false;
    int s2_per_cu = 0;
    int search_per_cu[kSearchKernels] = {};
};

struct PlanOptions {
    int64_t engine = 0, strips_per_group = 0, consumers = 0, importers = 0, max_blocks = 0, waves_per_block = 4, store_policy = 0;
    int64_t s2w = 0, xcd_chain = 0, split_blk = 0, split_from = 0;
    int64_t filler_hop_ps = 2400000, filler_tau_ps = 25000, filler_bw_gbs = 4200;
    int64_t probe_foreign_pairs = 0, debug_flags = 0;
};

struct TilePlan {
    int64_t c0 = 0, cols = 0, strips = 0;
    int grid = 0, nscout = 0, scout_double = 0, xcd_mode = 0;
    int split_blk = 0, split_from = 0, split_extra = 0, filler_end_steps = 0, filler_full_steps = 0;
    int filler_hop_ps = 0, filler_tau_ps = 0, filler_bw_gbs = 0;
    int store_nt = 0;
    int consumers = 0;
};

constexpr int kMaxTiles = 64;

struct FillPlan {
    int engine = 0;
    int64_t S = 0;
    int store_nt = 0;
    int NS = 0, NC = 0, importers = 0, threads = 0;
    int grid = 0;
    bool fast = false;
    int64_t bfront = 0, per = 0;
    bool perm = false;
    int64_t e4stride = 0;
    bool two_cols = false;
    int W2 = 126;
    int64_t ntile = 1, tstrips = 0;
    TilePlan tile[kMaxTiles];
    int64_t priv_stride = 0;
    size_t edge_need = 0, cb_need = 0, edge4_need = 0, priv_need = 0;
    size_t h_bytes = 0, p_bytes = 0;
    bool probe_pair_class = false;
};

FillPlan plan_fill(const PlanJob& job, const DeviceFacts& dev, const PlanOptions& opt);

struct BatchJob {
    int64_t cols = 0, rows = 0, npairs = 1;
    bool has_H = true, has_P = true;
    int p_elem_bytes = 4;
    int match = 3, mismatch = -3, gap = -2;
};

struct BatchPlan {
    bool wave = false;
    int C = 0;
    int64_t nstrips = 0;
    int front = 0;
    int64_t per = 0;
    int64_t bnd_per = 0;
    int64_t chunk = 0;
    int64_t grid = 0;
    int scan_blocks = 0, codes_blocks = 0;
    bool fits16 = false, k12 = false, packed16 = false;
    size_t bcodes_need = 0, bnd_need = 0;
    int64_t single_chunk = 0;
};

BatchPlan plan_batch(const BatchJob& job, const PlanOptions& opt);

constexpr int kBatchWave16 = 9, kBatchKernels = 17;
constexpr int batch_wave_index(int C, int pb) { return 3 * (C / 8) + (pb == 4 ? 2 : pb); }
constexpr int batch_wave16_index(bool le4, bool k12, bool pb1) { return kBatchWave16 + 4 * le4 + 2 * k12 + pb1; }
int batch_kernel(const BatchPlan& plan, unsigned nletters, int64_t n, int p_bytes);

struct SearchJob {
    int64_t qlen = 0, maxlen = 0;
    int64_t ntargets = 0;
    int match = 3, mismatch = -3, gap = -2;
};

struct SearchPlan {
    int C = 0;
    bool wide = false;
    int kernel = 0;
    int64_t nstrips = 0, qpad = 0;
    int64_t bnd_per = 0;
    int64_t grid = 0;
    int prof_blocks = 0;
    size_t prof_need = 0, bnd_need = 0;
};

SearchPlan plan_search(const SearchJob& job, const DeviceFacts& dev);

void search_schedule(const int64_t* offsets, int64_t ntargets, swk::SearchItem* items);

}
```

smith-waterman_amd/csrc/sw_scout_producer.inc:

```
__device__ __forceinline__ int P2S_FN(u32 palo, u32 pahi, u32 pblo, u32 pbhi, u32 ngap_v, u32 voff, u32 z0, u32 ga1, u32 gb1, u32 ta, u32 tb,
                                               u32 expoff, const unsigned char* cbase, u32 hb, u32 lowb, u32 prog_addr, int UT, sw_i32x4p erc, int (&polls)[2]) {
    int status;
    asm volatile(
        "s_setprio 3\n\t"
        "s_mov_b32 %[status], 0\n\t"
        "s_mov_b32 s95, 0\n\t"
        "s_mov_b32 s88, 1\n\t"
        "s_mov_b32 s91, 0\n\t"
        "s_mov_b32 s75, 0\n\t"
        "s_mov_b32 s76, %[e0]\n\t"
        "s_mov_b32 s77, %[e1]\n\t"
        "s_mov_b32 s78, %[e2]\n\t"
        "s_mov_b32 s79, %[e3]\n\t"
        "s_mov_b64 s[72:73], 1\n\t"
        "s_mov_b32 s70, 0\n\t"
        "s_mov_b32 s71, 0x80000000\n\t"
        "v_mov_b32 v26, %[hb]\n\t"
        "v_add_u32 v26, 0x8000, v26\n\t"
        "v_add_u32 v25, 0x800, v26\n\t"
        "v_mov_b32 v20, 0\n\tv_mov_b32 v21, 0\n\tv_mov_b32 v22, 0\n\tv_mov_b32 v23, 0\n\t"
        "s_mov_b64 s[92:93], %[cbase]\n\t"
        "v_mov_b32 v96, %[voff]\n\t"
        "v_mov_b32 v97, %[expoff]\n\t"
        "v_mov_b32 v31, %[progaddr]\n\t"
        "v_mov_b32 v29, 0\n\t"
        "v_mov_b32 v79, %[ga1]\n\t"
        "v_mov_b32 v95, %[gb1]\n\t"
        "v_mov_b32 v117, %[ta]\n\t"
        "v_mov_b32 v119, %[tb]\n\t"
        "v_mov_b32 v121, %[z0]\n\t"
        "v_mov_b32 v64, %[ga1]\n\tv_mov_b32 v65, %[ga1]\n\tv_mov_b32 v66, %[ga1]\n\tv_mov_b32 v67, %[ga1]\n\t"
        "v_mov_b32 v68, %[ga1]\n\tv_mov_b32 v69, %[ga1]\n\tv_mov_b32 v70, %[ga1]\n\tv_mov_b32 v71, %[ga1]\n\t"
        "v_mov_b32 v72, %[ga1]\n\tv_mov_b32 v73, %[ga1]\n\tv_mov_b32 v74, %[ga1]\n\tv_mov_b32 v75, %[ga1]\n\t"
        "v_mov_b32 v76, %[ga1]\n\tv_mov_b32 v77, %[ga1]\n\tv_mov_b32 v78, %[ga1]\n\t"
        "v_mov_b32 v103, 0\n\tv_mov_b32 v107, 0\n\tv_mov_b32 v111, 0\n\tv_mov_b32 v115, 0\n\t"
        "s_nop 4\n\t"
        "global_load_dwordx4 v[48:51], v96, s[92:93] offset:1\n\t"
        "global_load_dwordx4 v[52:55], v96, s[92:93] offset:2\n\t"
        "global_load_dwordx4 v[56:59], v96, s[92:93] offset:17\n\t"
        "global_load_dwordx4 v[60:63], v96, s[92:93] offset:18\n\t"
        "s_waitcnt vmcnt(0)\n"
        "Lchunk_%=:\n\t"
        "v_mov_b32 v98, %[hb]\n\t"
        "v_add_u32 v98, s91, v98\n\t"
        "v_mov_b32 v27, %[lowb]\n\t"
        "s_add_i32 s91, s91, 256\n\t"
        "s_and_b32 s91, s91, 4095\n\t"
        "v_cndmask_b32_e64 v98, v27, v98, s[72:73]\n\t"
        "v_mov_b32 v28, %[hb]\n\t"
        "v_add_u32 v28, s91, v28\n\t"
        "s_nop 0\n\t"
        "v_cndmask_b32_e64 v28, v27, v28, s[72:73]\n\t"
        P2S_BLOCK(0, "v48", "v49", "v50", "v51", "v52", "v53", "v54", "v55", "v[48:51]", "v[52:55]", "33", "34", "0", "16", "32", "48",
                  "v98 offset:64", "v98 offset:80", "v98 offset:96", "v98 offset:112")
        P2S_BLOCK(16, "v56", "v57", "v58", "v59", "v60", "v61", "v62", "v63", "v[56:59]", "v[60:63]", "49", "50", "64", "80", "96", "112",
                  "v98 offset:128", "v98 offset:144", "v98 offset:160", "v98 offset:176")
        P2S_BLOCK(32, "v48", "v49", "v50", "v51", "v52", "v53", "v54", "v55", "v[48:51]", "v[52:55]", "65", "66", "128", "144", "160", "176",
                  "v98 offset:192", "v98 offset:208", "v98 offset:224", "v98 offset:240")
        P2S_BLOCK(48, "v56", "v57", "v58", "v59", "v60", "v61", "v62", "v63", "v[56:59]", "v[60:63]", "81", "82", "192", "208", "224", "240",
                  "v28", "v28 offset:16", "v28 offset:32", "v28 offset:48")
        "s_add_i32 s75, s75, 256\n\t"
        "s_add_u32 s92, s92, 64\n\t"
        "s_addc_u32 s93, s93, 0\n\t"
        "s_add_i32 s88, s88, 64\n\t"
        "s_cmp_gt_i32 s88, %[ut]\n\t"
        "s_cbranch_scc0 Lchunk_%=\n\t"
        "s_branch Lexit_%=\n"
        P2_SLOW(0, "0", "16", "32", "48") P2_SLOW(16, "64", "80", "96", "112") P2_SLOW(32, "128", "144", "160", "176") P2_SLOW(48, "192", "208", "224", "240")
        "Lfail_%=:\n\t"
        "s_mov_b32 %[status], 1\n"
        "Lexit_%=:\n\t"
        "s_setprio 0\n\t"
        "s_waitcnt vmcnt(0) lgkmcnt(0)\n\t"
        "s_mov_b32 %[nhalo], s95\n\t"
        : [status] "=&s"(status), [nhalo] "=&s"(polls[1])
        : [palo] "v"(palo), [pahi] "v"(pahi), [pblo] "v"(pblo), [pbhi] "v"(pbhi), [ngap] "v"(ngap_v), [voff] "v"(voff),
          [z0] "v"(z0), [ga1] "v"(ga1), [gb1] "v"(gb1), [ta] "v"(ta), [tb] "v"(tb), [expoff] "v"(expoff), [cbase] "s"(cbase), [hb] "s"(hb), [lowb] "s"(lowb),
          [progaddr] "s"(prog_addr), [ut] "s"(UT), [e0] "s"(erc.x), [e1] "s"(erc.y), [e2] "s"(erc.z), [e3] "s"(erc.w)
        : "vcc", "scc", "memory", "s70", "s71", "s72", "s73", "s75", "s76", "s77", "s78", "s79", "s85", "s86", "s88", "s89", "s91", "s92", "s93", "s95",
          "v20", "v21", "v22", "v23", "v25", "v26", "v27", "v28", "v29", "v31", "v40", "v41", "v42", "v43", "v44", "v45", "v46", "v47", "v48",
          "v49", "v50", "v51", "v52", "v53", "v54", "v55", "v56", "v57", "v58", "v59", "v60", "v61", "v62", "v63", "v64", "v65", "v66", "v67", "v68", "v69", "v70",
          "v71", "v72", "v73", "v74", "v75", "v76", "v77", "v78", "v79", "v80", "v81", "v82", "v83", "v84", "v85", "v86", "v87", "v88", "v89", "v90", "v91", "v92",
          "v93", "v94", "v95", "v96", "v97", "v98", "v100", "v101", "v102", "v103", "v104", "v105", "v106", "v107", "v108", "v109", "v110", "v111",
          "v112", "v113", "v114", "v115", "v116", "v117", "v118", "v119", "v120", "v121", "v122");
    polls[0] = 0;
    return status;
}
```

smith-waterman_amd/csrc/sw_systolic2.inc:

```

constexpr int S2_W = 126;
template <bool OV> __device__ __forceinline__ constexpr int s2_stride() { return OV ? 110 : S2_W; }
template <bool OV> __device__ __forceinline__ constexpr int s2_xlane() { return s2_stride<OV>() >> 1; }

struct S2Side {
    __attribute__((aligned(16))) u32 halo[SY_RH];
    __attribute__((aligned(16))) u32 lowv[128];
    int topv[128];
    int prod_u, halo_ready, never, pad;
};
struct Sys2Lds {
    __attribute__((aligned(16))) unsigned char ringA[64 * SY_LSTR];
    __attribute__((aligned(16))) unsigned char ringB[64 * SY_LSTR];
    __attribute__((aligned(16))) int cons_blk[8];
    S2Side side;
};

#define P2_STEP(GA, GB, GA1, GB1, TAP, TAN, TBP, TBN, HIN, SA, SB, BYTE)                                                   \
    "v_add_u32 v121, v121, %[ngap]\n\t"                                                                                   \
    "v_max3_i32 v120, " TBP ", " GB1 ", v121\n\t"                                                                         \
    "v_max3_i32 v122, " TAP ", " GB1 ", v121\n\t"                                                                         \
    "v_add_u32_sdwa " TBN ", " GB1 ", sext(" SA ") dst_sel:DWORD dst_unused:UNUSED_PAD src0_sel:DWORD src1_sel:" BYTE "\n\t" \
    "v_max_i32_dpp " GA ", v120, " GA1 " wave_shr:1 row_mask:0xf bank_mask:0xf\n\t"                                       \
    "v_max3_i32 " GB ", v122, " GA ", " HIN "\n\t"                                                                        \
// ... 12 lines not shown
    "ds_write_b128 v99, v[" GA0 ":" GA3 "] offset:" WO "\n\t"                                                              \
    "ds_write_b128 v123, v[" GB0 ":" GB3 "] offset:" WO "\n\t"                                                             \
    "buffer_store_dwordx4 v[" GB0 ":" GB3 "], v97, s[76:79], s75 offen offset:" WO " sc1\n\t"                               \
    "buffer_store_dwordx4 v[" GB0 ":" GB3 "], %[expoffl], s[76:79], s75 offen offset:" WO " sc0\n\t"                        \
    "ds_read_b128 v[" H0 ":" H3 "], " HADDR "\n\t"
#define P2_CHK(V0, V1, LBL)                                                                                                \
    "s_waitcnt lgkmcnt(7)\n\t"                                                                                            \
    "v_readfirstlane_b32 s85, " V0 "\n\t"                                                                                 \
    "v_readfirstlane_b32 s86, " V1 "\n\t"                                                                                 \
    "s_and_b32 s85, s85, s86\n\t"                                                                                         \
    "s_cbranch_scc0 " LBL "\n"
#define P2_BLOCK(KB, CA0, CA1, CA2, CA3, CB0, CB1, CB2, CB3, NA, NB, PF, PF1, W0, W1, W2, W3, N0, N1, N2, N3, BPF)         \
    P2_CHK("v103", "v107", "LslowA" #KB "_%=")                                                                            \
    "LgoA" #KB "_%=:\n\t"                                                                                                 \
    "s_waitcnt vmcnt(18)\n\t"                  \
    "v_perm_b32 v40, %[pahi], %[palo], " CA0 "\n\t"                                                                       \
    "v_perm_b32 v41, %[pahi], %[palo], " CA1 "\n\t"                                                                       \
    "v_perm_b32 v42, %[pahi], %[palo], " CA2 "\n\t"                                                                       \
    "v_perm_b32 v43, %[pahi], %[palo], " CA3 "\n\t"                                                                       \
    "v_perm_b32 v44, %[pbhi], %[pblo], " CB0 "\n\t"                                                                       \
    "v_perm_b32 v45, %[pbhi], %[pblo], " CB1 "\n\t"                                                                       \
    "v_perm_b32 v46, %[pbhi], %[pblo], " CB2 "\n\t"                                                                       \
    "v_perm_b32 v47, %[pbhi], %[pblo], " CB3 "\n\t"                                                                       \
    "global_load_dwordx4 " NA ", v96, s[92:93] offset:" PF "\n\t"                                                         \
    "global_load_dwordx4 " NB ", v96, s[92:93] offset:" PF1 "\n\t"                                                        \
    P2_GRP0 P2_TAIL("64", "67", "80", "83", "100", "103", W0, N0)                                                         \
    P2_GRP1 P2_TAIL("68", "71", "84", "87", "104", "107", W1, N1)                                                         \
    P2_CHK("v111", "v115", "LslowB" #KB "_%=")                                                                            \
    "LgoB" #KB "_%=:\n\t"                                                                                                 \
    P2_GRP2 P2_TAIL("72", "75", "88", "91", "108", "111", W2, N2)                                                         \
    BPF                                                                                                                   \
    P2_GRP3 P2_TAIL("76", "79", "92", "95", "112", "115", W3, N3)                                                         \
    "v_add_u32 v29, 16, v29\n\t"                                                                                          \
    "ds_write_b32 v31, v29\n\t"
#define P2_BPFETCH "ds_read_b128 v[124:127], v39\n\tds_read_b128 v[32:35], v39 offset:16\n\tds_read_b32 v36, v30\n\t"
#define P2_BPCHECK(T, KC, KR)                                                                                             \
    "s_waitcnt lgkmcnt(4)\n\t"                         \
    "v_min3_i32 v37, v124, v125, v126\n\t"                                                                                \
    "v_min3_i32 v38, v127, v32, v33\n\t"                                                                                  \
    "v_min3_i32 v37, v37, v34, v35\n\t"                                                                                   \
    "v_min_i32 v37, v37, v38\n\t"                                                                                         \
    "s_mov_b32 s89, 0\n\t"                                                                                                \
    "v_readfirstlane_b32 s86, v36\n\t"                                                                                    \
    "v_readfirstlane_b32 s85, v37\n"                                                                                      \
    "Lbpe" T "_%=:\n\t"                                                                                                   \
    "s_lshl_b32 s85, s85, 4\n\t"                                                                                          \
    "s_add_i32 s85, s85, 16\n\t"                                                                                          \
    "s_add_i32 s87, s88, " KC "\n\t"                                                                                      \
    "s_cmp_ge_i32 s85, s87\n\t"                                                                                           \
    "s_cbranch_scc0 Lbpw" T "_%=\n\t"                                                                                     \
    "s_add_i32 s87, s88, " KR "\n\t"                                                                                      \
    "s_cmp_ge_i32 s86, s87\n\t"                                                                                           \
    "s_cbranch_scc1 Lbpok" T "_%=\n"                                                                                      \
    "Lbpw" T "_%=:\n\t"                                                                                                   \
    "s_sleep 1\n\t"                                                                                                       \
    "s_add_i32 s89, s89, 1\n\t"                                                                                           \
    "s_add_i32 s94, s94, 1\n\t"                                                                                           \
    "s_cmp_lt_u32 s89, 0x1000000\n\t"                                                                                     \
    "s_cbranch_scc0 Lfail_%=\n\t"                                                                                         \
    "ds_read_b128 v[124:127], v39\n\t"                                                                                    \
    "ds_read_b128 v[32:35], v39 offset:16\n\t"                                                                            \
    "ds_read_b32 v36, v30\n\t"                                                                                            \
    "s_waitcnt lgkmcnt(0)\n\t"                                                                                            \
    "v_min3_i32 v37, v124, v125, v126\n\t"                                                                                \
    "v_min3_i32 v38, v127, v32, v33\n\t"                                                                                  \
    "v_min3_i32 v37, v37, v34, v35\n\t"                                                                                   \
    "v_min_i32 v37, v37, v38\n\t"                                                                                         \
    "s_nop 1\n\t"                                                                                                         \
    "v_readfirstlane_b32 s85, v37\n\t"                                                                                    \
    "v_readfirstlane_b32 s86, v36\n\t"                                                                                    \
    "s_branch Lbpe" T "_%=\n"                                                                                             \
    "Lbpok" T "_%=:\n\t"
#define P2_SLOW(KB, R0, R1, R2, R3)                                                                                       \
    "LslowA" #KB "_%=:\n\t"                                                                                               \
    "s_mov_b32 s89, 0\n"                                                                                                  \
    "LpollA" #KB "_%=:\n\t"                                                                                               \
    "ds_read_b128 v[100:103], v98 offset:" R0 "\n\t"                                                                      \
    "ds_read_b128 v[104:107], v98 offset:" R1 "\n\t"                                                                      \
    "s_waitcnt lgkmcnt(0)\n\t"                                                                                            \
    "v_readfirstlane_b32 s85, v103\n\t"                                                                                   \
    "v_readfirstlane_b32 s86, v107\n\t"                                                                                   \
    "s_and_b32 s85, s85, s86\n\t"                                                                                         \
    "s_cbranch_scc1 LgoA" #KB "_%=\n\t"                                                                                   \
    "s_add_i32 s89, s89, 1\n\t"                                                                                           \
    "s_add_i32 s95, s95, 1\n\t"                                                                                           \
    "s_cmp_lt_u32 s89, 0x1000000\n\t"                                                                                     \
    "s_cbranch_scc1 LpollA" #KB "_%=\n\t"                                                                                 \
    "s_branch Lfail_%=\n"                                                                                                 \
    "LslowB" #KB "_%=:\n\t"                                                                                               \
    "s_mov_b32 s89, 0\n"                                                                                                  \
    "LpollB" #KB "_%=:\n\t"                                                                                               \
    "ds_read_b128 v[108:111], v98 offset:" R2 "\n\t"                                                                      \
    "ds_read_b128 v[112:115], v98 offset:" R3 "\n\t"                                                                      \
    "s_waitcnt lgkmcnt(0)\n\t"                                                                                            \
    "v_readfirstlane_b32 s85, v111\n\t"                                                                                   \
    "v_readfirstlane_b32 s86, v115\n\t"                                                                                   \
    "s_and_b32 s85, s85, s86\n\t"                                                                                         \
    "s_cbranch_scc1 LgoB" #KB "_%=\n\t"                                                                                   \
    "s_add_i32 s89, s89, 1\n\t"                                                                                           \
    "s_add_i32 s95, s95, 1\n\t"                                                                                           \
    "s_cmp_lt_u32 s89, 0x1000000\n\t"                                                                                     \
    "s_cbranch_scc1 LpollB" #KB "_%=\n\t"                                                                                 \
    "s_branch Lfail_%=\n"

#define C2_P32(PA, PB, PP, POL) "buffer_store_dwordx2 " PP ", %[voffP], %[rP], s82 offen" POL "\n\t"
#define C2_P8(PA, PB, PP, POL)                                                                                             \
    "buffer_store_byte " PA ", %[voffP], %[rP], s82 offen" POL "\n\t"                                                      \
    "buffer_store_byte " PB ", %[voffP], %[rP], s82 offen offset:1" POL "\n\t"
#define C2_NOTRK(HA, HB, K2) ""
#define C2_TRK(HA, HB, K2)                                                                                                 \
    "v_cmp_gt_i32_e64 s[72:73], " HA ", %[bv]\n\t"                                                                         \
    "v_max_i32 %[bv], %[bv], " HA "\n\t"                                                                                   \
    "v_cndmask_b32_e64 %[bi], %[bi], " K2 ", s[72:73]\n\t"                                                                 \
    "v_cmp_gt_i32_e64 s[72:73], " HB ", %[bv]\n\t"                                                                         \
    "v_max_i32 %[bv], %[bv], " HB "\n\t"                                                                                   \
    "v_cndmask_b32_e64 %[bi], %[bi], " K2 "+1, s[72:73]\n\t"
#define C2_ROW(GA0, GA1, GB0, GB1, CH, BYTE, HA, HB, HP, PA, PB, PP, POL, HST, PST, TRK, K2)                                    \
    "v_sub_u32 %[nz], %[nz], %[ngap]\n\t"                                                                                 \
    "v_cmp_eq_u32_sdwa s[68:69], %[aA], " CH " src0_sel:DWORD src1_sel:" BYTE "\n\t"                                       \
    "v_cmp_eq_u32_sdwa s[70:71], %[aB], " CH " src0_sel:DWORD src1_sel:" BYTE "\n\t"                                       \
    "v_add_u32 " HA ", " GA1 ", %[nz]\n\t"                                                                                \
    "v_add3_u32 " HB ", " GB1 ", %[nz], v112\n\t"                                                                     \
    "v_cndmask_b32_e64 v113, %[xm], %[mm], s[68:69]\n\t"                                                                  \
    "v_cndmask_b32_e64 v114, %[xm], %[mm], s[70:71]\n\t"                                                                  \
    HST(HP, POL)                                                                                                           \
    "v_cmp_eq_u32_e64 s[60:61], " GA0 ", " GA1 "\n\t"                                                                     \
    "v_cmp_eq_u32_e64 s[64:65], " GB0 ", " GB1 "\n\t"                                                                     \
    "v_add_u32_dpp v115, " GB0 ", v113 wave_shr:1 row_mask:0xf bank_mask:0xf bound_ctrl:0\n\t"                            \
    "v_add_u32 v116, " GA0 ", v114\n\t"                                                                                   \
    "v_cndmask_b32_e64 " PA ", 2, 1, s[60:61]\n\t"                                                                        \
    "v_cndmask_b32_e64 " PB ", 2, 1, s[64:65]\n\t"                                                                        \
    "v_cmp_eq_u32_e64 s[62:63], v115, " GA1 "\n\t"                                                                        \
    "v_cmp_eq_u32_e64 s[66:67], v116, " GB1 "\n\t"                                                                        \
    "v_max3_i32 %[bm], %[bm], " HA ", " HB "\n\t"                                                                         \
    "v_cmp_eq_u32_e64 s[68:69], 0, " HA "\n\t"                                                                            \
    "v_cndmask_b32_e64 " PA ", " PA ", 3, s[62:63]\n\t"                                                                   \
    "v_cndmask_b32_e64 " PB ", " PB ", 3, s[66:67]\n\t"                                                                   \
    "v_cmp_eq_u32_e64 s[70:71], 0, " HB "\n\t"                                                                            \
    "s_add_u32 s80, s80, %[rowbH]\n\t"                                                                                    \
    "v_cndmask_b32_e64 " PA ", " PA ", 0, s[68:69]\n\t"                                                                   \
    TRK(HA, HB, K2)                                                                                                        \
    "v_cndmask_b32_e64 " PB ", " PB ", 0, s[70:71]\n\t"                                                                   \
    PST(PA, PB, PP, POL)                                                                                                   \
    "s_add_u32 s82, s82, %[rowbP]\n\t"
#define C2_H32(HP, POL) "buffer_store_dwordx2 " HP ", %[voffH], %[rH], s80 offen" POL "\n\t"
#define C2_H64(HP, POL) "buffer_store_dwordx4 " HP ", %[voffH], %[rH], s80 offen" POL "\n\t"
#define C2_EV32(GA0, GA1, GB0, GB1, CH, BYTE, POL, PST, TRK, K2) C2_ROW(GA0, GA1, GB0, GB1, CH, BYTE, "v100", "v101", "v[100:101]", "v102", "v103", "v[102:103]", POL, C2_H32, PST, TRK, K2)
#define C2_OD32(GA0, GA1, GB0, GB1, CH, BYTE, POL, PST, TRK, K2) C2_ROW(GA0, GA1, GB0, GB1, CH, BYTE, "v104", "v105", "v[104:105]", "v106", "v107", "v[106:107]", POL, C2_H32, PST, TRK, K2)
#define C2_EV64(GA0, GA1, GB0, GB1, CH, BYTE, POL, PST, TRK, K2) C2_ROW(GA0, GA1, GB0, GB1, CH, BYTE, "v100", "v102", "v[100:103]", "v104", "v105", "v[104:105]", POL, C2_H64, PST, TRK, K2)
#define C2_OD64(GA0, GA1, GB0, GB1, CH, BYTE, POL, PST, TRK, K2) C2_ROW(GA0, GA1, GB0, GB1, CH, BYTE, "v106", "v108", "v[106:109]", "v110", "v111", "v[110:111]", POL, C2_H64, PST, TRK, K2)
#define C2_RD(K, KB, OFF) "ds_read_b32 v" #K ", %[ea] offset:" #OFF "\n\tds_read_b32 v" #KB ", %[eb] offset:" #OFF "\n\t"
#define C2_RDW(K, KB, I)                                                                                                   \
    "v_add_u32 v98, " #I ", %[ew]\n\t"                                                                                   \
    "v_and_b32 v98, 1020, v98\n\t"                                                                                        \
    "v_add_u32 v99, v98, %[eb]\n\t"                                                                                       \
    "v_add_u32 v98, v98, %[ea]\n\t"                                                                                       \
    "ds_read_b32 v" #K ", v98\n\t"                                                                                        \
    "ds_read_b32 v" #KB ", v99\n\t"
#define C2_READS_FLAT                                                                                                      \
    C2_RD(64, 81, 0) C2_RD(65, 82, 4) C2_RD(66, 83, 8) C2_RD(67, 84, 12) C2_RD(68, 85, 16) C2_RD(69, 86, 20) C2_RD(70, 87, 24) C2_RD(71, 88, 28)      \
    C2_RD(72, 89, 32) C2_RD(73, 90, 36) C2_RD(74, 91, 40) C2_RD(75, 92, 44) C2_RD(76, 93, 48) C2_RD(77, 94, 52) C2_RD(78, 95, 56) C2_RD(79, 96, 60) \
    C2_RD(80, 97, 64)
#define C2_READS_WRAP                                                                                                      \
    C2_RDW(64, 81, 0) C2_RDW(65, 82, 4) C2_RDW(66, 83, 8) C2_RDW(67, 84, 12) C2_RDW(68, 85, 16) C2_RDW(69, 86, 20) C2_RDW(70, 87, 24)              \
    C2_RDW(71, 88, 28) C2_RDW(72, 89, 32) C2_RDW(73, 90, 36) C2_RDW(74, 91, 40) C2_RDW(75, 92, 44) C2_RDW(76, 93, 48) C2_RDW(77, 94, 52)            \
    C2_RDW(78, 95, 56) C2_RDW(79, 96, 60) C2_RDW(80, 97, 64)
#define C2_ASM(READS, POL, PST, TRK, C2_EV, C2_OD)                                                                                       \
    asm volatile(                                                                                                          \
        "s_load_dwordx4 s[76:79], %[cptr], 0x0\n\t"                                                                       \
        READS                                                                                                              \
        "ds_write_b32 %[slot], %[qv]\n\t"            \
        "s_mov_b32 s80, 0\n\t"                                                                                            \
        "s_mov_b32 s82, 0\n\t"                                                                                            \
        "v_sub_u32 v112, 0, %[ngap]\n\t"                                                                                  \
        "v_mov_b32 v101, 0\n\tv_mov_b32 v103, 0\n\tv_mov_b32 v107, 0\n\tv_mov_b32 v109, 0\n\t"    \
        "s_waitcnt lgkmcnt(0)\n\t"                                    \
        "s_cmp_lg_u32 %[first], 0\n\t"                                                                                    \
        "s_cbranch_scc0 Lc2_%=\n\t"                                                                                       \
        "v_mov_b32 v64, %[g0a]\n\t"                  \
        "v_mov_b32 v81, %[g0b]\n"                                                                                          \
        "Lc2_%=:\n\t"                                                                                                     \
        C2_EV("v64", "v65", "v81", "v82", "s76", "BYTE_0", POL, PST, TRK, "0") C2_OD("v65", "v66", "v82", "v83", "s76", "BYTE_1", POL, PST, TRK, "2")       \
        C2_EV("v66", "v67", "v83", "v84", "s76", "BYTE_2", POL, PST, TRK, "4") C2_OD("v67", "v68", "v84", "v85", "s76", "BYTE_3", POL, PST, TRK, "6")       \
        C2_EV("v68", "v69", "v85", "v86", "s77", "BYTE_0", POL, PST, TRK, "8") C2_OD("v69", "v70", "v86", "v87", "s77", "BYTE_1", POL, PST, TRK, "10")      \
        C2_EV("v70", "v71", "v87", "v88", "s77", "BYTE_2", POL, PST, TRK, "12") C2_OD("v71", "v72", "v88", "v89", "s77", "BYTE_3", POL, PST, TRK, "14")     \
        C2_EV("v72", "v73", "v89", "v90", "s78", "BYTE_0", POL, PST, TRK, "16") C2_OD("v73", "v74", "v90", "v91", "s78", "BYTE_1", POL, PST, TRK, "18")     \
        C2_EV("v74", "v75", "v91", "v92", "s78", "BYTE_2", POL, PST, TRK, "20") C2_OD("v75", "v76", "v92", "v93", "s78", "BYTE_3", POL, PST, TRK, "22")     \
        C2_EV("v76", "v77", "v93", "v94", "s79", "BYTE_0", POL, PST, TRK, "24") C2_OD("v77", "v78", "v94", "v95", "s79", "BYTE_1", POL, PST, TRK, "26")     \
        C2_EV("v78", "v79", "v95", "v96", "s79", "BYTE_2", POL, PST, TRK, "28") C2_OD("v79", "v80", "v96", "v97", "s79", "BYTE_3", POL, PST, TRK, "30")     \
        "v_mov_b32 %[gla], v80\n\t"                      \
        "v_mov_b32 %[glb], v97\n\t"                                                                                       \
        : [nz] "+v"(nz), [bm] "+v"(bm), [bv] "+v"(bv), [bi] "+v"(bi), [gla] "=&v"(gla), [glb] "=&v"(glb)                    \
        : [ea] "v"(ea), [eb] "v"(eb), [ew] "v"(ew), [slot] "v"(slot_addr), [qv] "v"(qv), [first] "s"(first), [g0a] "v"(g0a), [g0b] "v"(g0b),  \
          [aA] "v"(aA), [aB] "v"(aB), [mm] "v"(mm_v), [xm] "v"(xm_v), [ngap] "v"(ngap_v), [voffH] "v"(voffH),           \
          [voffP] "v"(voffP), [rH] "s"(rH), [rP] "s"(rP), [rowbH] "s"(rowbH), [rowbP] "s"(rowbP), [cptr] "s"(chars)           \
        : "vcc", "scc", "memory", "s60", "s61", "s62", "s63", "s64", "s65", "s66", "s67", "s68", "s69", "s70", "s71", "s72", "s73", "s76", "s77", "s78", "s79", \
          "s80", "s82", "v64", "v65", "v66", "v67", "v68", "v69", "v70", "v71", "v72", "v73", "v74", "v75", "v76", "v77", "v78", "v79", "v80", "v81", "v82",    \
          "v83", "v84", "v85", "v86", "v87", "v88", "v89", "v90", "v91", "v92", "v93", "v94", "v95", "v96", "v97", "v98", "v99", "v100", "v101", "v102", \
          "v103", "v104", "v105", "v106", "v107", "v108", "v109", "v110", "v111", "v112", "v113", "v114", "v115", "v116")
struct C2Out { u32 bm, gla, glb; };
__device__ __forceinline__ C2Out consumer_block2(bool flat, bool nt, bool p8, bool trk, bool h64, u32 ea, u32 eb, u32 ew, u32 slot_addr, u32 qv, int first, u32 g0a,
                                                 u32 g0b, u32& nz, u32& bv, u32& bi, u32 aA, u32 aB, u32 mm_v, u32 xm_v, u32 ngap_v, u32 voffH,
                                                 u32 voffP, sw_i32x4 rH, sw_i32x4 rP, u32 rowbH, u32 rowbP, const unsigned char* chars) {
    u32 bm = 0, gla, glb;
#define C2_PICK(READS)                                                                                                     \
    if (h64) {                                                           \
        if (p8) { if (nt) { C2_ASM(READS, " nt", C2_P8, C2_NOTRK, C2_EV64, C2_OD64); } else { C2_ASM(READS, "", C2_P8, C2_NOTRK, C2_EV64, C2_OD64); } }        \
        else { if (nt) { C2_ASM(READS, " nt", C2_P32, C2_NOTRK, C2_EV64, C2_OD64); } else { C2_ASM(READS, "", C2_P32, C2_NOTRK, C2_EV64, C2_OD64); } }         \
    } else if (trk) {                                                                                                      \
        if (p8) { if (nt) { C2_ASM(READS, " nt", C2_P8, C2_TRK, C2_EV32, C2_OD32); } else { C2_ASM(READS, "", C2_P8, C2_TRK, C2_EV32, C2_OD32); } }            \
        else { if (nt) { C2_ASM(READS, " nt", C2_P32, C2_TRK, C2_EV32, C2_OD32); } else { C2_ASM(READS, "", C2_P32, C2_TRK, C2_EV32, C2_OD32); } }             \
    } else {                                                                                                               \
        if (p8) { if (nt) { C2_ASM(READS, " nt", C2_P8, C2_NOTRK, C2_EV32, C2_OD32); } else { C2_ASM(READS, "", C2_P8, C2_NOTRK, C2_EV32, C2_OD32); } }        \
        else { if (nt) { C2_ASM(READS, " nt", C2_P32, C2_NOTRK, C2_EV32, C2_OD32); } else { C2_ASM(READS, "", C2_P32, C2_NOTRK, C2_EV32, C2_OD32); } }         \
    }
    if (flat) { C2_PICK(C2_READS_FLAT) } else { C2_PICK(C2_READS_WRAP) }
#undef C2_PICK
    return C2Out{bm, gla, glb};
}

#include "sw_wholeline_consumer.inc"

#include "sw_filler_producer.inc"


#define P2S_TAIL(GB0, GB3, H0, H3, WO, HADDR)                                                                              \
    "buffer_store_dwordx4 v[" GB0 ":" GB3 "], v97, s[76:79], s75 offen offset:" WO P2S_EXP_MOD "\n\t"                       \
    "ds_read_b128 v[" H0 ":" H3 "], " HADDR "\n\t"
#define P2S_LGKM "3"
#ifndef P2S_VMCNT
#define P2S_VMCNT "10"
#endif
#define P2S_CHK(V0, V1, LBL)                                                                                               \
    "s_waitcnt lgkmcnt(" P2S_LGKM ")\n\t"                                                                                            \
    "v_readfirstlane_b32 s85, " V0 "\n\t"                                                                                 \
    "v_readfirstlane_b32 s86, " V1 "\n\t"                                                                                 \
    "s_and_b32 s85, s85, s86\n\t"                                                                                         \
    "s_cbranch_scc0 " LBL "\n"
#define P2S_BLOCK(KB, CA0, CA1, CA2, CA3, CB0, CB1, CB2, CB3, NA, NB, PF, PF1, W0, W1, W2, W3, N0, N1, N2, N3)             \
    P2S_CHK("v103", "v107", "LslowA" #KB "_%=")                                                                           \
    "LgoA" #KB "_%=:\n\t"                                                                                                 \
    "s_waitcnt vmcnt(" P2S_VMCNT ")\n\t"                                                                                             \
    "v_perm_b32 v40, %[pahi], %[palo], " CA0 "\n\t"                                                                       \
    "v_perm_b32 v41, %[pahi], %[palo], " CA1 "\n\t"                                                                       \
    "v_perm_b32 v42, %[pahi], %[palo], " CA2 "\n\t"                                                                       \
    "v_perm_b32 v43, %[pahi], %[palo], " CA3 "\n\t"                                                                       \
    "v_perm_b32 v44, %[pbhi], %[pblo], " CB0 "\n\t"                                                                       \
    "v_perm_b32 v45, %[pbhi], %[pblo], " CB1 "\n\t"                                                                       \
    "v_perm_b32 v46, %[pbhi], %[pblo], " CB2 "\n\t"                                                                       \
    "v_perm_b32 v47, %[pbhi], %[pblo], " CB3 "\n\t"                                                                       \
    "global_load_dwordx4 " NA ", v96, s[92:93] offset:" PF "\n\t"                                                         \
    "global_load_dwordx4 " NB ", v96, s[92:93] offset:" PF1 "\n\t"                                                        \
    P2_GRP0 P2S_TAIL("80", "83", "100", "103", W0, N0)                                                                    \
    P2_GRP1 P2S_TAIL("84", "87", "104", "107", W1, N1)                                                                    \
    P2S_CHK("v111", "v115", "LslowB" #KB "_%=")                                                                           \
    "LgoB" #KB "_%=:\n\t"                                                                                                 \
    P2_GRP2 P2S_TAIL("88", "91", "108", "111", W2, N2)                                                                    \
    P2_GRP3 P2S_TAIL("92", "95", "112", "115", W3, N3)                                                                    \
    "v_add_u32 v29, 16, v29\n\t"                                                                                          \
    "ds_write_b32 v31, v29\n\t"

#define P2S_FN producer_scout2
#define P2S_EXP_MOD " sc1"
#include "sw_scout_producer.inc"
#undef P2S_FN
#undef P2S_EXP_MOD
#define P2S_FN producer_scout2_local
#define P2S_EXP_MOD " sc0"
#include "sw_scout_producer.inc"
#undef P2S_FN
#undef P2S_EXP_MOD
#include "sw_scoutfill_producer.inc"

template <bool OV>
__device__ __forceinline__ void s2_load_top(S2Side& sd, const FillParams& p, int s, int tid) {
    const int64_t jt = (int64_t)s * s2_stride<OV>() + tid;
    const bool want = tid < 127 && jt <= p.cols;
    int tv = 0;
    if (p.top_gran) {
        u64 gr = 0;
        uint64_t t0 = 0;
        unsigned n = 0;
        for (;;) {
            if (want) gr = __hip_atomic_load((gu64*)(p.top_gran + jt), __ATOMIC_RELAXED, __HIP_MEMORY_SCOPE_SYSTEM);
            const bool ok = !want || (u32)(gr >> 32) == p.top_tag;
            if (__builtin_amdgcn_ballot_w64(!ok) == 0) break;
            __builtin_amdgcn_s_sleep(8);
            if ((++n & 63u) == 0) {
                const uint64_t now = __builtin_amdgcn_s_memrealtime();
                if (t0 == 0) t0 = now;
                if (((now - t0) >> 10) > (uint64_t)p.top_wait_ticks)
                    __hip_atomic_store((gu32*)p.abort_flag, 1u, __ATOMIC_RELAXED, __HIP_MEMORY_SCOPE_AGENT);
                if (__builtin_amdgcn_readfirstlane((int)__hip_atomic_load((gu32*)p.abort_flag, __ATOMIC_RELAXED, __HIP_MEMORY_SCOPE_AGENT)) != 0) break;
            }
        }
        tv = (int)(u32)gr;
    } else if (p.top && want) {
        tv = p.top[jt];
    }
    sd.topv[tid] = tv;
}

struct S2Pace {
    bool on = false, set = false;
    int S = 0, s = 0, steps = 0, bps = 0;
    float inv = 0.f, start = 0.f;
    __device__ __forceinline__ void calibrate(const FillParams& p, float t_first) {
        int tau_ps = p.filler_tau_ps, hop_ps = p.filler_hop_ps, bw_gbs = p.filler_bw_gbs;
        asm volatile("" : "+s"(tau_ps), "+s"(hop_ps), "+s"(bw_gbs));
        const float tau_min = (float)tau_ps * 1e-4f, hop_host = (float)hop_ps * 1e-4f;
        const float bw_per_tick = (float)bw_gbs * 10.f, fsteps = (float)steps;
        const float hop = (s >= 8) ? fminf(fmaxf(t_first / (float)s, 0.5f * hop_host), 1.5f * hop_host) : hop_host;
        start = (s >= 8) ? t_first : (float)s * hop;
        const float esteps = p.filler_end_steps > 0 ? (float)p.filler_end_steps : fsteps;
        const float wsteps = p.filler_full_steps > 0 ? (float)p.filler_full_steps : fsteps;
        const float d_chain = (float)(S - 1) * hop + esteps * tau_min;
        const float x = bw_per_tick * hop / ((float)max(bps, 1) * wsteps);
        const float d_bw = (x < 20.f) ? (float)S * hop / (1.f - __expf(-x)) : 0.f;
        const float d = fmaxf(d_chain, d_bw);
        inv = (d > start + 1.f) ? fsteps / (d - start) : 0.f;
        set = true;
    }
};
template <bool OV>
__device__ __forceinline__ bool s2_importer(S2Side& sd, const FillParams& p, int s_real, int phi, int UT, int rows, int gb, int ngap, int lane, bool synth = false,
                                            S2Pace pace = S2Pace(), int stop_u = 0x7fffffff) {
    const int s = synth ? 0 : s_real;
    __builtin_amdgcn_s_setprio(2);
    const u32 row0v = (u32)(gb + sd.topv[0] + ngap * s_real * s2_stride<OV>());
    const int xl = s2_xlane<OV>();
    const int ulast = min(UT + 64, stop_u);
    const u32 tag = (u32)gb >> 24;
    const u32* e4 = (s > 0) ? p.edge4 + (int64_t)(s - 1) * p.e4stride : nullptr;
    int impu = 1;
    bool wide = true;
    Spin spin; spin.code = 3;
    const uint64_t pace_t0 = __builtin_amdgcn_s_memrealtime();
    while (impu <= ulast) {
        const int front = lds_load(&sd.halo_ready);
        if (front > 1) impu = max(impu, front);
        if (impu > ulast) break;
        int lim = min(ulast + 1, lds_load(&sd.prod_u) + SY_RH / 2 - 2 * SY_U);
        if (pace.set && pace.inv > 0.f) lim = min(lim, 64 + max(0, (int)(((float)(uint32_t)(__builtin_amdgcn_s_memrealtime() - pace_t0) - pace.start) * pace.inv)));
        int base = impu;
        auto windows = [&](auto NB) {
            constexpr int nbat = decltype(NB)::value;
            u32 vals[nbat];
            bool oks[nbat];
#pragma unroll
            for (int b4 = 0; b4 < nbat; ++b4) {
                const int u = impu + b4 * 64 + lane;
                const int r = u - phi;
                u32 v = row0v;
                bool ok = true;
                if (r > rows) v = (u32)gb;
                else if (r > 0) {
                    if (s == 0) v = (u32)(gb + ngap * r + (p.tile_left ? p.tile_left[(int64_t)r * p.M] : 0));
                    else {
                        v = __hip_atomic_load((gu32*)(e4 + u + xl), __ATOMIC_RELAXED, __HIP_MEMORY_SCOPE_AGENT);
                        ok = (v >> 24) == tag;
                    }
                }
                vals[b4] = v;
                oks[b4] = ok && (u < lim);
            }
            const int front2 = lds_load(&sd.halo_ready);
#pragma unroll
            for (int b4 = 0; b4 < nbat; ++b4) {
                const int u = impu + b4 * 64 + lane;
                const u64 okm = __ballot(oks[b4]);
                const int npre = (okm == ~0ull) ? 64 : __builtin_ctzll(~okm);
                if (base == impu + b4 * 64 && npre > 0) {
                    if (lane < npre && (front2 <= 1 || u >= front2)) {
                        __hip_atomic_store(&sd.halo[(u - 1) & (SY_RH - 1)], vals[b4], __ATOMIC_RELAXED, __HIP_MEMORY_SCOPE_WORKGROUP);
                        __hip_atomic_store(&sd.halo[(u - 1 + SY_RH / 2) & (SY_RH - 1)], 0u, __ATOMIC_RELAXED, __HIP_MEMORY_SCOPE_WORKGROUP);
                    }
                    base += npre;
                }
            }
        };
        if (wide) windows(std::integral_constant<int, 4>{});
        else windows(std::integral_constant<int, 1>{});
        wide = (base - impu) >= 64;
        if (base > impu) {
            asm volatile("" ::: "memory");
            if (pace.on && !pace.set && base > phi + 1)
                pace.calibrate(p, (float)(uint32_t)(__builtin_amdgcn_s_memrealtime() - pace_t0));
            impu = base;
            __hip_atomic_fetch_max(&sd.halo_ready, impu, __ATOMIC_RELAXED, __HIP_MEMORY_SCOPE_WORKGROUP);
        } else if (spin.fail(p.abort_flag)) {
            return false;
        }
    }
    __builtin_amdgcn_s_setprio(0);
    return true;
}

template <bool SCOUT, bool LOCAL, bool OV>
__device__ __forceinline__ int s2_produce(S2Side& sd, Sys2Lds* full, const FillParams& p, const unsigned char* seq_a, const unsigned char* ltab,
                                          const unsigned char* bcode, int s, int S, int phi, int UT, int lane, int gb, int ngap, int mm, int xm, bool exports,
                                          bool local_rt = false, bool stamps_as_scout = false, int ua = -1) {
    const int jA = s * s2_stride<OV>() + 2 * lane - 1, jB = jA + 1;
    const int topA = lane >= 1 ? sd.topv[2 * lane - 1] : 0, topB = sd.topv[2 * lane];
    const int jn = jA + 2;
    const u32 ca = (lane < 63 && jn >= 1 && jn <= p.cols) ? (u32)ltab[seq_a[jn - 1]] : 8u;
    const u32 cb = (lane >= 1 && jB <= p.cols) ? (u32)ltab[seq_a[jB - 1]] : 8u;
    u32 palo = 0, pahi = 0, pblo = 0, pbhi = 0;
#pragma unroll
    for (int c = 0; c < 4; ++c) {
        palo |= ((u32)(unsigned char)(signed char)((u32)c == ca ? mm : xm)) << (8 * c);
        pblo |= ((u32)(unsigned char)(signed char)((u32)c == cb ? mm : xm)) << (8 * c);
    }
#pragma unroll
    for (int c = 4; c < 7; ++c) {
        pahi |= ((u32)(unsigned char)(signed char)((u32)c == ca ? mm : xm)) << (8 * (c - 4));
        pbhi |= ((u32)(unsigned char)(signed char)((u32)c == cb ? mm : xm)) << (8 * (c - 4));
    }
    pahi |= ((u32)(unsigned char)(signed char)SW_PERM_PAD) << 24;
    pbhi |= ((u32)(unsigned char)(signed char)SW_PERM_PAD) << 24;
    if (lane == 0) {
        const u32 pad4 = 0x01010101u * (u32)(unsigned char)(signed char)SW_PERM_PAD;
        pblo = pad4; pbhi = pad4;
    }
    const u32 ga1 = lane == 0 ? (u32)gb : (u32)(gb + topA + ngap * (int)jA), gb1 = (u32)(gb + topB + ngap * (int)jB);
    const u32 z0 = (u32)(gb + ngap * (1 - phi - lane + (int)jA));
    const unsigned char* cbase = bcode + (p.bfront - phi - 64);
    const u32 expoff = (exports && s + 1 < S && lane == s2_xlane<OV>()) ? 0u : SY_OOB;
    const uint64_t eb = (uint64_t)(uintptr_t)(p.edge4 + (int64_t)s * p.e4stride);
    const sw_i32x4p erc = {(int)(u32)eb, (int)(u32)(eb >> 32), 0x7FFFFF00, 0x00020000};
    int polls[2];
    u64* const dbg = p.dbg ? p.dbg + ((!SCOUT && p.nscout > 0 && !stamps_as_scout) ? 6 * p.nstrips + 32 : 0) : nullptr;
    if (dbg && lane == 0) {
        dbg[2 * s] = __builtin_amdgcn_s_memrealtime();
        if (s == 0 && dbg == p.dbg) p.dbg[6 * p.nstrips + 16] = __builtin_amdgcn_s_memtime();
    }
    int st;
    if constexpr (SCOUT) {
        if constexpr (LOCAL) {
            st = producer_scout2_local(palo, pahi, pblo, pbhi, (u32)ngap, 63u - (u32)lane, z0, ga1, gb1, ga1 + (u32)SW_PERM_PAD, gb1 + (u32)SW_PERM_PAD, expoff, cbase,
                                       (u32)(size_t)&sd.halo[0], (u32)(size_t)&sd.lowv[0], (u32)(size_t)&sd.prod_u, UT, erc, polls);
        } else
            st = producer_scout2(palo, pahi, pblo, pbhi, (u32)ngap, 63u - (u32)lane, z0, ga1, gb1, ga1 + (u32)SW_PERM_PAD, gb1 + (u32)SW_PERM_PAD, expoff, cbase,
                                 (u32)(size_t)&sd.halo[0], (u32)(size_t)&sd.lowv[0], (u32)(size_t)&sd.prod_u, UT, erc, polls);
    } else {
        const u32 wA = (u32)(size_t)&full->ringA[0] + (u32)lane * (u32)SY_LSTR, wB = (u32)(size_t)&full->ringB[0] + (u32)lane * (u32)SY_LSTR;
        const int kc = 30 - SY_R - phi, kr = -SY_R - phi - 32;
        if (ua >= 0)
            st = producer_scoutfill2(palo, pahi, pblo, pbhi, (u32)ngap, wA, wB, 63u - (u32)lane, z0, ga1, gb1, ga1 + (u32)SW_PERM_PAD, gb1 + (u32)SW_PERM_PAD,
                                     local_rt ? SY_OOB : expoff, local_rt ? expoff : SY_OOB, cbase, (u32)(size_t)&sd.halo[0], (u32)(size_t)&sd.lowv[0],
                                     (u32)(size_t)&full->cons_blk[0], (u32)(size_t)&sd.never, (u32)(size_t)&sd.prod_u, ua, UT, kc, kr, erc, polls);
        else
        st = producer_perm2(palo, pahi, pblo, pbhi, (u32)ngap, wA, wB, 63u - (u32)lane, z0, ga1, gb1, ga1 + (u32)SW_PERM_PAD, gb1 + (u32)SW_PERM_PAD,
                            local_rt ? SY_OOB : expoff, local_rt ? expoff : SY_OOB, cbase, (u32)(size_t)&sd.halo[0], (u32)(size_t)&sd.lowv[0],
                            (u32)(size_t)&full->cons_blk[0], (u32)(size_t)&sd.never, (u32)(size_t)&sd.prod_u, UT, kc, kr, erc, polls);
    }
    if (dbg && lane == 0) {
        dbg[2 * s + 1] = __builtin_amdgcn_s_memrealtime();
        if (s == 0 && dbg == p.dbg) p.dbg[6 * p.nstrips + 17] = __builtin_amdgcn_s_memtime();
        if (dbg == p.dbg) {
            dbg[4 * p.nstrips + 16 + 2 * s] = (u64)polls[0];
            dbg[4 * p.nstrips + 17 + 2 * s] = (u64)polls[1];
        }
    }
    return st;
}

struct XcdLayout { int f0, nf, s0, ns, ndx, w; };
__device__ __forceinline__ XcdLayout xcd_layout(int S, int x, int extra = 0) {
    const int base = S >> 3, rem = S & 7;
    XcdLayout l;
    l.nf = base + (x < rem ? 1 : 0);
    l.f0 = x * base + min(x, rem);
    l.s0 = x ? l.f0 - 1 : 0;
    l.ns = (x ? l.nf : l.nf - 1) + (x == 7 ? extra : 0);
    l.ndx = max(0, l.ns - (32 - l.nf));
    l.w = l.ns - l.ndx;
    return l;
}
__device__ __forceinline__ bool strip_has_single_scout(int S, int t, int extra) {
    for (int x = 0; x < 8; ++x) {
        const XcdLayout l = xcd_layout(S, x, extra);
        if (t >= l.s0 && t < l.s0 + l.ns && t <= S - 2 + extra) return t - l.s0 >= 2 * l.ndx;
    }
    return false;
}
__device__ __forceinline__ bool xcd_local_readers(const FillParams& p, int S, int s, unsigned my_xcc, int far_block, Spin& spin, bool& local) {
    const u32* xtab = (const u32*)(p.atab + SW_XTAB_OFF);
    int blocks[3] = {-1, -1, far_block};
    for (int x = 0; x < 8; ++x) {
        const XcdLayout l = xcd_layout(S, x, p.split_extra);
        const int t = s + 1;
        if (t >= l.f0 && t < l.f0 + l.nf) blocks[0] = 8 * (l.w + t - l.f0) + x;
        if (t <= S - 2 + p.split_extra && t >= l.s0 && t < l.s0 + l.ns) blocks[1] = 8 * ((t - l.s0 < 2 * l.ndx) ? (t - l.s0) / 2 : t - l.s0 - l.ndx) + x;
    }
    local = true;
    for (int i = 0; i < 3; ++i) {
        if (blocks[i] < 0) continue;
        u32 v;
        while ((v = __hip_atomic_load((gu32*)(xtab + blocks[i]), __ATOMIC_RELAXED, __HIP_MEMORY_SCOPE_AGENT)) == 0u)
            if (spin.fail(p.abort_flag)) return false;
        local = local && v == my_xcc + 1u;
    }
    return true;
}

struct S2Prep {
    __attribute__((aligned(16))) unsigned char tab[256];
    unsigned int pres[8];
    int nletters, ok;
};
constexpr int S2_SYNC_BAR = 0, S2_SYNC_OUT = 1, S2_SYNC_MAP = 8;

__device__ __forceinline__ int s2_prologue(S2Prep& pp, const FillParams& p, const unsigned char* __restrict__ seq_a, const unsigned char* __restrict__ seq_b) {
    const int tid = (int)threadIdx.x, nth = (int)blockDim.x, G = (int)gridDim.x, wg = (int)blockIdx.x;
    gu32* const sync = (gu32*)p.sync;
    if (tid < 8) pp.pres[tid] = 0u;
    __syncthreads();
    {
        const int64_t acols = p.alpha_cols, total = acols + p.rows, chunk = (total + G - 1) / G;
        const int64_t lo = (int64_t)wg * chunk, hi = min(total, lo + chunk);
        for (int64_t i = lo + tid; i < hi; i += nth) {
            const unsigned char ch = i < acols ? p.alpha_a[i] : seq_b[i - acols];
            atomicOr(&pp.pres[ch >> 5], 1u << (ch & 31));
        }
    }
    __syncthreads();
    if (tid < 64) {
        if (tid < 8 && pp.pres[tid]) (void)__hip_atomic_fetch_or(sync + S2_SYNC_MAP + tid, pp.pres[tid], __ATOMIC_RELAXED, __HIP_MEMORY_SCOPE_AGENT);
        __builtin_amdgcn_fence(__ATOMIC_RELEASE, "agent");
        if (tid == 0) (void)__hip_atomic_fetch_add(sync + S2_SYNC_BAR, 1u, __ATOMIC_RELAXED, __HIP_MEMORY_SCOPE_AGENT);
        Spin spin; spin.code = 17;
        bool ok = true;
        while ((u32)__builtin_amdgcn_readfirstlane((int)__hip_atomic_load(sync + S2_SYNC_BAR, __ATOMIC_RELAXED, __HIP_MEMORY_SCOPE_AGENT)) < (u32)G)
            if (spin.fail(p.abort_flag)) { ok = false; break; }
        if (tid < 8) pp.pres[tid] = __hip_atomic_load(sync + S2_SYNC_MAP + tid, __ATOMIC_RELAXED, __HIP_MEMORY_SCOPE_AGENT);
        if (tid == 0) pp.ok = ok ? 1 : 0;
    }
    __syncthreads();
    if (!pp.ok) return -1;
    if (tid < 256) {
        int rank = 0, nl = 0;
#pragma unroll
        for (int w = 0; w < 8; ++w) {
            const unsigned int m = pp.pres[w];
            nl += __popc(m);
            if (w < (tid >> 5)) rank += __popc(m);
            else if (w == (tid >> 5)) rank += __popc(m & ((1u << (tid & 31)) - 1u));
        }
        const bool here = (pp.pres[tid >> 5] >> (tid & 31)) & 1u;
        pp.tab[tid] = (here && nl <= 7) ? (unsigned char)rank : (unsigned char)7;
        if (tid == 0) pp.nletters = nl;
    }
    __syncthreads();
    const int nl = pp.nletters;
    const int64_t per = p.bpad_pstride, front = p.bfront, rows = p.rows;
    if (wg == 0) {
        if (tid < 256) p.atab_w[tid] = pp.tab[tid];
        if (tid == 0) *(unsigned int*)(p.atab_w + 256) = (unsigned int)nl;
        if (nl > 7)
            for (int64_t i = tid; i < per; i += nth) {
                const bool in = (i >= front && i - front < rows);
                const unsigned char ch = in ? seq_b[i - front] : (unsigned char)0;
                p.bpad8_w[i] = ch;
                p.bpad16_w[i] = in ? (unsigned short)ch : (unsigned short)0x100;
                p.bcode_w[i] = (unsigned char)7;
            }
    }
    if (nl <= 7) {
        unsigned char* const mine = p.priv + (int64_t)wg * p.priv_stride;
        for (int64_t i = 4 * (int64_t)tid; i < per; i += 4 * (int64_t)nth) {
            const int64_t k = i - front;
            u32 raw = 0u, code = 0x07070707u;
            if (k >= 0 && k + 4 <= rows) {
                raw = *(const u32*)(seq_b + k);
                code = (u32)pp.tab[raw & 255u] | ((u32)pp.tab[(raw >> 8) & 255u] << 8) | ((u32)pp.tab[(raw >> 16) & 255u] << 16) | ((u32)pp.tab[raw >> 24] << 24);
            } else if (k + 4 > 0 && k < rows) {
#pragma unroll
                for (int q = 0; q < 4; ++q)
                    if (k + q >= 0 && k + q < rows) {
                        const u32 ch = seq_b[k + q];
                        raw |= ch << (8 * q);
                        code = (code & ~(0xffu << (8 * q))) | ((u32)pp.tab[ch] << (8 * q));
                    }
            }
            *(u32*)(mine + i) = raw;
            *(u32*)(mine + per + i) = code;
        }
        const int64_t M = p.M, nrow0 = p.cols + 1, nedge = nrow0 + rows, chunk = (nedge + G - 1) / G;
        const int64_t lo = (int64_t)wg * chunk, hi = min(nedge, lo + chunk);
        void* const H = p.H; void* const P = (void*)p.P;
        const bool own_col0 = p.tile_left == nullptr;
        for (int64_t e = lo + tid; e < hi; e += nth) {
            if (e < nrow0) {
                if (!p.skip_row0 && (e > 0 || own_col0)) {
                    if (H) { if (p.h_bytes == 8) ((int64_t*)H)[e] = 0; else ((int32_t*)H)[e] = 0; }
                    if (P) { if (p.p_bytes == 1) ((signed char*)P)[e] = 0; else ((int32_t*)P)[e] = 0; }
                }
            } else if (own_col0) {
                const int64_t r = e - nrow0 + 1;
                if (H) { if (p.h_bytes == 8) ((int64_t*)H)[r * M] = 0; else ((int32_t*)H)[r * M] = 0; }
                if (P) { if (p.p_bytes == 1) ((signed char*)P)[r * M] = 0; else ((int32_t*)P)[r * M] = 0; }
            }
        }
    }
    __builtin_amdgcn_fence(__ATOMIC_RELEASE, "workgroup");
    __syncthreads();
    __builtin_amdgcn_fence(__ATOMIC_ACQUIRE, "workgroup");
    return nl;
}

__device__ __forceinline__ void s2_epilogue(const FillParams& p, bool worked) {
    asm volatile("s_waitcnt vmcnt(0)" ::: "memory");
    __syncthreads();
    if (threadIdx.x != 0) return;
    gu32* const sync = (gu32*)p.sync;
    const u32 prev = __hip_atomic_fetch_add(sync + S2_SYNC_OUT, 1u, __ATOMIC_RELAXED, __HIP_MEMORY_SCOPE_AGENT);
    if (prev != gridDim.x - 1u) return;
    if (worked && p.final_launch) {
        const u64 k = __hip_atomic_load((gu64*)p.result_key, __ATOMIC_RELAXED, __HIP_MEMORY_SCOPE_AGENT);
        const u32 ab = __hip_atomic_load((gu32*)p.abort_flag, __ATOMIC_RELAXED, __HIP_MEMORY_SCOPE_AGENT);
        if (p.result) {
            p.result->max_score = (int64_t)(k >> 40);
            p.result->max_pos = k ? (int64_t)(SW_KEY_IDX_MASK - (k & SW_KEY_IDX_MASK)) : 0;
            p.result->path_len = ab ? -(int64_t)ab : 0;
        }
        __hip_atomic_store((gu64*)p.result_key, 0ull, __ATOMIC_RELAXED, __HIP_MEMORY_SCOPE_AGENT);
        __hip_atomic_store((gu32*)p.abort_flag, 0u, __ATOMIC_RELAXED, __HIP_MEMORY_SCOPE_AGENT);
    }
    if (worked) {
        gu32* const xtab = (gu32*)(p.atab_w + SW_XTAB_OFF);
        for (int i = 0; i < 256; ++i) __hip_atomic_store(xtab + i, 0u, __ATOMIC_RELAXED, __HIP_MEMORY_SCOPE_AGENT);
    }
    for (int w = 0; w < 8; ++w) __hip_atomic_store(sync + S2_SYNC_MAP + w, 0u, __ATOMIC_RELAXED, __HIP_MEMORY_SCOPE_AGENT);
    __hip_atomic_store(sync + S2_SYNC_BAR, 0u, __ATOMIC_RELAXED, __HIP_MEMORY_SCOPE_AGENT);
    __hip_atomic_store(sync + S2_SYNC_OUT, 0u, __ATOMIC_RELAXED, __HIP_MEMORY_SCOPE_AGENT);
}

template <int NC, bool OV>
__device__ __forceinline__ void s2_body(Sys2Lds& lds, const unsigned char* ltab, const unsigned char* my_bpad8, const unsigned char* my_bcode,
                                        const unsigned char* seq_a, const FillParams& p) {
    const int lane = threadIdx.x & 63;
    const int wave = __builtin_amdgcn_readfirstlane((int)(threadIdx.x >> 6));
    const int64_t M = p.M;
    const int rows = (int)p.rows;
    const int ngap = p.ngap, mm = p.mm, xm = p.xm;
    const int S = p.nstrips;
    const int gb = (int)p.gbias;
    const int nscout = p.nscout;

    int sc_cnt = 0, sc_s0 = 0, sc_far = -1, sc_far_block = -1, fill_s = S, fill_step = S;
    unsigned my_xcc = 0;
    if (p.xcd_mode == 1) {
        const int x = (int)blockIdx.x & 7, k = (int)blockIdx.x >> 3;
        const XcdLayout l = xcd_layout(S, x, p.split_extra);
        const int nf = l.nf, f0 = l.f0, s0 = l.s0, ns = l.ns, ndx = l.ndx, w = l.w;
        asm volatile("s_getreg_b32 %0, hwreg(HW_REG_XCC_ID)" : "=s"(my_xcc));
        my_xcc &= 15u;
        if (threadIdx.x == 0) __hip_atomic_store((gu32*)(p.atab + SW_XTAB_OFF) + blockIdx.x, my_xcc + 1u, __ATOMIC_RELAXED, __HIP_MEMORY_SCOPE_AGENT);
        if (k < w) {
            sc_cnt = k < ndx ? 2 : 1;
            sc_s0 = s0 + (k < ndx ? 2 * k : k + ndx);
            sc_far = s0 + ns - 1;
            sc_far_block = 8 * ((ns - 1 < 2 * ndx) ? (ns - 1) / 2 : ns - 1 - ndx) + x;
        } else if (k - w < nf) {
            fill_s = f0 + k - w;
        } else {
            return;
        }
    } else if (p.xcd_mode == 2) {
        const int G = (int)gridDim.x, x = (int)blockIdx.x & 7, k = (int)blockIdx.x >> 3;
        int off = 0;
        for (int y = 0; y < x; ++y) off += (G - y + 7) >> 3;
        if (threadIdx.x == 0) {
            unsigned xcc;
            asm volatile("s_getreg_b32 %0, hwreg(HW_REG_XCC_ID)" : "=s"(xcc));
            __hip_atomic_store((gu32*)(p.atab + SW_XTAB_OFF) + blockIdx.x, (xcc & 15u) + 1u, __ATOMIC_RELAXED, __HIP_MEMORY_SCOPE_AGENT);
        }
        fill_s = off + k;
        fill_step = G;
    } else if ((int)blockIdx.x < nscout) {
        const int nd = p.scout_double, b = (int)blockIdx.x;
        sc_cnt = b < nd ? 2 : 1;
        sc_s0 = b < nd ? 2 * b : b + nd;
    } else {
        fill_s = (int)blockIdx.x - nscout;
        fill_step = (int)gridDim.x - nscout;
    }

    const int split_blk = (p.xcd_mode == 1) ? p.split_blk : 0;
    bool sf = false;
    if (split_blk > 0 && sc_cnt == 1 && sc_s0 >= p.split_from) { sf = true; fill_s = sc_s0; fill_step = S; sc_cnt = 0; }
    else if (sc_cnt == 1 && sc_s0 == S - 1) return;

    if (sc_cnt) {
        S2Side* sides = (S2Side*)&lds;
        const int cnt = sc_cnt, s0 = sc_s0;
        const int cls = wave & 3;
        const int nimp_dbg = (p.debug_flags >> DBG_S2_IMPORTERS_SHIFT) & 3;
        const bool producer = wave < cnt;
        const bool importer = !producer && (cnt == 2 ? (cls >= 2 && (wave >> 2) < (nimp_dbg ? nimp_dbg : 1))
                                                     : (nimp_dbg ? (cls == 2 && (wave >> 2) < nimp_dbg) : cls != 0));
        const int half = producer ? wave : (cnt == 2 ? cls - 2 : 0);
        if (threadIdx.x < 2) { sides[threadIdx.x].prod_u = 0; sides[threadIdx.x].halo_ready = 1; sides[threadIdx.x].never = 0x7fffffff; }
        for (int i = threadIdx.x; i < 2 * SY_RH; i += blockDim.x) sides[i / SY_RH].halo[i % SY_RH] = 0u;
        if (threadIdx.x < 256) sides[threadIdx.x >> 7].lowv[threadIdx.x & 127] = (u32)gb;
        if (threadIdx.x < 256 && (int)(threadIdx.x >> 7) < cnt && s0 + (int)(threadIdx.x >> 7) < S)
            s2_load_top<OV>(sides[threadIdx.x >> 7], p, s0 + (int)(threadIdx.x >> 7), (int)(threadIdx.x & 127));
        __syncthreads();
        if (p.top_gran && __builtin_amdgcn_readfirstlane((int)__hip_atomic_load((gu32*)p.abort_flag, __ATOMIC_RELAXED, __HIP_MEMORY_SCOPE_AGENT)) != 0) return;
        const int s = s0 + half;
        if (s < S && (producer || importer)) {
            const int phi = S - 1 - s;
            const int UT = ((rows + SY_U - 1) / SY_U * SY_U + 63 + phi + 63) / 64 * 64;
            if (producer) {
                bool local = false;
                if (p.xcd_mode == 1 && s != sc_far && my_xcc == (blockIdx.x & 7u)) {
                    Spin spin; spin.code = 16;
                    if (!xcd_local_readers(p, S, s, my_xcc, sc_far_block, spin, local)) return;
                }
                const int st = local ? s2_produce<true, true, OV>(sides[half], nullptr, p, seq_a, ltab, my_bcode, s, S, phi, UT, lane, gb, ngap, mm, xm, !(p.debug_flags & DBG_S2_SCOUTS_NO_EXPORT))
                                     : s2_produce<true, false, OV>(sides[half], nullptr, p, seq_a, ltab, my_bcode, s, S, phi, UT, lane, gb, ngap, mm, xm, !(p.debug_flags & DBG_S2_SCOUTS_NO_EXPORT));
                if (st) __hip_atomic_store((gu32*)p.abort_flag, 1u, __ATOMIC_RELAXED, __HIP_MEMORY_SCOPE_AGENT);
                if (p.xcd_mode == 1 && s == sc_far) __builtin_amdgcn_fence(__ATOMIC_RELEASE, "agent");
            } else {
                (void)s2_importer<OV>(sides[half], p, s, phi, UT, rows, gb, ngap, lane, (p.debug_flags & DBG_S2_SYNTH_HALO) != 0);
            }
        }
        return;
    }

    int32_t* const H = (int32_t*)p.H;
    const bool h64 = p.h_bytes == 8;
    const int hsh = h64 ? 1 : 0;
    char* const P = (char*)p.P;
    const bool p8 = p.p_bytes == 1;
    const bool has_top = p.top != nullptr || p.top_gran != nullptr;
    S2Side& sd = lds.side;
    const int k9 = wave - 1 - (wave >> 2);
    const bool off0 = (wave & 3) != 0;
    const int nc_eff = NC;
    const bool producer = wave == 0, consumer = off0 && k9 < nc_eff, importer = off0 && k9 >= nc_eff;

    for (int s = fill_s; s < S; s += fill_step) {
        const int nblk_all = (rows + SY_U - 1) / SY_U;
        const bool upper = split_blk > 0 && !sf && s >= p.split_from && strip_has_single_scout(S, s, p.split_extra);
        const int q_lo = sf ? min(split_blk, nblk_all) : 0, q_hi = upper ? min(split_blk, nblk_all) : nblk_all;
        if (threadIdx.x == 0) { sd.prod_u = 0; sd.halo_ready = 1; sd.never = 0x7fffffff; }
        if (threadIdx.x < 8) lds.cons_blk[threadIdx.x] = ((int)threadIdx.x < nc_eff) ? q_lo - 1 : 0x7fffffff;
        for (int i = threadIdx.x; i < SY_RH; i += blockDim.x) sd.halo[i] = 0u;
        if (threadIdx.x < 128) sd.lowv[threadIdx.x] = (u32)gb;
        if (threadIdx.x < 128) s2_load_top<OV>(sd, p, s, (int)threadIdx.x);
        __syncthreads();
        if (p.top_gran && __builtin_amdgcn_readfirstlane((int)__hip_atomic_load((gu32*)p.abort_flag, __ATOMIC_RELAXED, __HIP_MEMORY_SCOPE_AGENT)) != 0) return;
        const int topA = lane >= 1 ? sd.topv[2 * lane - 1] : 0, topB = sd.topv[2 * lane];
        const int phi = S - 1 - s;
        const int UT = (q_hi * SY_U + 63 + phi + 63) / 64 * 64;
        const int jA = s * s2_stride<OV>() + 2 * lane - 1, jB = jA + 1;
        if (producer) {
            bool local = false;
            if (p.xcd_mode == 2) {
                if (s == fill_s) {
                    unsigned xcc;
                    asm volatile("s_getreg_b32 %0, hwreg(HW_REG_XCC_ID)" : "=s"(xcc));
                    xcc &= 15u;
                    const int x = (int)blockIdx.x & 7, k = (int)blockIdx.x >> 3, nx = ((int)gridDim.x - x + 7) >> 3;
                    int dec = 0;
                    if (k + 1 < nx && xcc == (unsigned)x) {
                        Spin spin; spin.code = 16;
                        u32 v;
                        while ((v = (u32)__builtin_amdgcn_readfirstlane((int)__hip_atomic_load((gu32*)(p.atab + SW_XTAB_OFF) + 8 * (k + 1) + x, __ATOMIC_RELAXED,
                                                                                                __HIP_MEMORY_SCOPE_AGENT))) == 0u)
                            if (spin.fail(p.abort_flag)) return;
                        dec = (v == xcc + 1u) ? 1 : 0;
                    }
                    lds_store(&sd.pad, dec);
                }
                local = __builtin_amdgcn_readfirstlane(lds_load(&sd.pad)) == 1;
            }
            if (sf && s != sc_far && s + 1 < S && my_xcc == (blockIdx.x & 7u)) {
                Spin spin; spin.code = 16;
                if (!xcd_local_readers(p, S, s, my_xcc, sc_far_block, spin, local)) return;
            }
            const int st = s2_produce<false, false, OV>(sd, &lds, p, seq_a, ltab, my_bcode, s, S, phi, UT, lane, gb, ngap, mm, xm, nscout == 0 || sf, local, sf,
                                             sf ? max(0, (q_lo * SY_U + phi - 1) / 64 * 64) : -1);
            if (st) {
                __hip_atomic_store((gu32*)p.abort_flag, 16u, __ATOMIC_RELAXED, __HIP_MEMORY_SCOPE_AGENT);
                return;
            }
            if (sf && s == sc_far) __builtin_amdgcn_fence(__ATOMIC_RELEASE, "agent");
            if (local && s + fill_step >= S) __builtin_amdgcn_fence(__ATOMIC_RELEASE, "agent");
        } else if (consumer) {
            const int nblk = q_hi;
            const unsigned char* bchars = my_bpad8 + p.bfront;
            const u32* rA = (const u32*)&lds.ringA[lane * SY_LSTR];
            const u32* rB = (const u32*)&lds.ringB[lane * SY_LSTR];
            const bool okA = lane >= 1 && jA <= p.cols, okB = lane >= 1 && jB <= p.cols;
            const int aA = okA ? (int)seq_a[jA - 1] : SY_ASENT, aB = okB ? (int)seq_a[jB - 1] : SY_ASENT + 1;
            const u32 voff2 = okB ? (u32)jA * 4u : SY_OOB, voff1 = (okA && !okB) ? (u32)jA * 4u : SY_OOB;
            const bool tail1 = (s == S - 1) && (p.cols & 1);
            const u32 rowb = (u32)(M * 4);
            int best = 0, bestrow = 0, bestcol = 0, bestq = -1;
            Spin spin; spin.code = 2;
            if (!tail1) {
                const u32 laneA = (u32)(size_t)rA, laneB = (u32)(size_t)rB;
                const u32 mm_v = (u32)mm, xm_v = (u32)xm, ngap_v = (u32)ngap;
                const u32 slot_addr = (u32)(size_t)&lds.cons_blk[k9];
                const u32 g0a = (u32)(gb + topA + ngap * (int)jA), g0b = (u32)(gb + topB + ngap * (int)jB);
                const bool nostore = (p.debug_flags & DBG_NO_STORES) != 0;
                const bool nt = p.store_nt != 0, store_h = H != nullptr && !nostore, store_p = P != nullptr && !nostore, trk = H == nullptr;
                const u32 voffH = (okB && store_h) ? (u32)jA * (h64 ? 8u : 4u) : SY_OOB, voffP = (okB && store_p) ? (u32)jA * (p8 ? 1u : 4u) : SY_OOB;
                const u32 rowbH = (u32)(M * (h64 ? 8 : 4)), rowbP = (u32)(M * (p8 ? 1 : 4));
                int bestcode = 0;
                constexpr int W = s2_stride<OV>();
                const bool allod = (M & 1) == 0;
                const bool wlaunch = OV && H != nullptr && !(P != nullptr && p8 && (h64 || allod)) && !trk && !p.bot_gran && !has_top &&
                                     ((uintptr_t)H & (h64 ? 15u : 7u)) == 0 && ((uintptr_t)P & 7u) == 0;
                const bool wl = wlaunch && s > 0 && s < S - 1;
                const bool mine = !OV || wlaunch || s == S - 1 || lane <= (W >> 1);
                u32 wm = 0;
                if (wl) {
                    const int64_t c1 = (int64_t)s * W + 1;
                    const u32 f0H = (u32)(((uint64_t)(uintptr_t)H + (uint64_t)(((M + c1) * 4) << hsh)) & 63u), f0P = (u32)(((uint64_t)(uintptr_t)P + (uint64_t)((M + c1) * 4)) & 63u);
                    const u32 pszH = h64 ? 16u : 8u, spanH = h64 ? 880u : 440u;
#pragma nounroll
                    for (int k = 0; k < SY_U; ++k) {
                        const bool odr = allod || (k & 1);
                        const u32 pcH = pszH * (u32)(lane - 1) - (odr ? pszH / 2 : 0u), pcP = 8u * (u32)(lane - 1) - (odr ? 4u : 0u);
                        if (!((u32)(pcH - ((f0H + (u32)k * rowbH + pcH) & 63u)) < spanH)) wm |= 1u << k;
                        if (!((u32)(pcP - ((f0P + (u32)k * rowbP + pcP) & 63u)) < 440u)) wm |= 1u << (16 + k);
                    }
                }
                if (has_top && store_h && k9 == 0) {
                    if (h64) {
                        if (okA) ((int64_t*)H)[jA] = topA;
                        if (okB) ((int64_t*)H)[jB] = topB;
                        if (s == 0 && lane == 0) ((int64_t*)H)[0] = topB;
                    } else {
                        if (okA) H[jA] = topA;
                        if (okB) H[jB] = topB;
                        if (s == 0 && lane == 0) H[0] = topB;
                    }
                }
                for (int q = q_lo + k9; q < nblk; q += nc_eff) {
                    const int qs = __builtin_amdgcn_readfirstlane(q);
                    const int r0 = qs * SY_U + 1;
                    const int need = r0 + SY_U - 1 + 63 + phi;
                    if (sf && q == q_lo + k9 && need > 256) {
                        if (!s2_importer<OV>(sd, p, s, phi, UT, rows, gb, ngap, lane, false, S2Pace(), need - 192)) return;
                    }
                    while (lds_load(&sd.prod_u) < need)
                        if (spin.fail(p.abort_flag)) return;
                    asm volatile("" ::: "memory");
                    const u32 e0 = (u32)(r0 - 2 + lane + phi);
                    const bool flat = (((u32)(r0 - 2 + phi) & (SY_R - 1)) + 63 + SY_U) < (u32)SY_R;
                    const uint64_t bH = (uint64_t)(uintptr_t)(H + (((int64_t)r0 * M) << hsh)), bP = (uint64_t)(uintptr_t)(P + (int64_t)r0 * M * (p8 ? 1 : 4));
                    const int nbr = min(SY_U, rows - r0 + 1);
                    const int nrH = nbr == SY_U ? 0x7FFFFF00 : nbr * (int)rowbH, nrP = nbr == SY_U ? 0x7FFFFF00 : nbr * (int)rowbP;
                    const sw_i32x4 dH = {__builtin_amdgcn_readfirstlane((int)(u32)bH), __builtin_amdgcn_readfirstlane((int)(u32)(bH >> 32)), nrH, 0x00020000};
                    const sw_i32x4 dP = {__builtin_amdgcn_readfirstlane((int)(u32)bP), __builtin_amdgcn_readfirstlane((int)(u32)(bP >> 32)), nrP, 0x00020000};
                    u32 nz = (u32)(-(gb + ngap * (r0 - 1 + (int)jA)));
                    u32 bv = (u32)best, bi = 0;
                    const u32 eoff = (e0 & (SY_R - 1)) * 4u;
                    C2Out o;
                    if (wl) {
                        const int64_t c1 = (int64_t)s * W + 1;
                        const uint64_t fH = bH + (uint64_t)((c1 * 4) << hsh), fP = bP + (uint64_t)(c1 * 4);
                        const uint64_t bH2 = fH & ~(uint64_t)63, bP2 = fP & ~(uint64_t)63;
                        const u32 dlH = (u32)(bH2 - bH), dlP = (u32)(bP2 - bP);
                        const sw_i32x4 dH2 = {__builtin_amdgcn_readfirstlane((int)(u32)bH2), __builtin_amdgcn_readfirstlane((int)(u32)(bH2 >> 32)),
                                              nbr == SY_U ? 0x7FFFFF00 : __builtin_amdgcn_readfirstlane(nrH - (int)dlH), 0x00020000};
                        const sw_i32x4 dP2 = {__builtin_amdgcn_readfirstlane((int)(u32)bP2), __builtin_amdgcn_readfirstlane((int)(u32)(bP2 >> 32)),
                                              nbr == SY_U ? 0x7FFFFF00 : __builtin_amdgcn_readfirstlane(nrP - (int)dlP), 0x00020000};
                        const u32 vH = voffH == SY_OOB ? SY_OOB : voffH - dlH;
                        const u32 vP = p8 ? ((voffP == SY_OOB || lane > (W >> 1)) ? SY_OOB : voffP) : (voffP == SY_OOB ? SY_OOB : voffP - dlP);
                        o.bm = consumer_block3(flat, nt, h64, p8, flat ? laneA + eoff : laneA, flat ? laneB + eoff : laneB, eoff, slot_addr, (u32)qs,
                                               __builtin_amdgcn_readfirstlane(qs == 0 ? 1 : 0), g0a, g0b, nz, (u32)aA, (u32)aB, mm_v, xm_v, ngap_v, vH, vP,
                                               dH2, p8 ? dP : dP2, rowbH, rowbP, bchars + (r0 - 1), wm, allod);
                        o.gla = o.glb = 0u;
                    } else
                    o = consumer_block2(flat, nt, p8, trk, h64, flat ? laneA + eoff : laneA, flat ? laneB + eoff : laneB, eoff, slot_addr, (u32)qs,
                                                    __builtin_amdgcn_readfirstlane(qs == 0 ? 1 : 0), g0a, g0b, nz, bv, bi, (u32)aA, (u32)aB, mm_v, xm_v, ngap_v,
                                                    voffH, voffP, dH, dP, rowbH, rowbP, bchars + (r0 - 1));
                    if (trk) { if (okB && mine && (int)bv > best) { best = (int)bv; bestq = qs; bestcode = (int)bi; } }
                    else if (okB && mine && (int)o.bm > best) { best = (int)o.bm; bestq = qs; }
                    if (p.bot_gran && qs == nblk - 1) {
                        const int zl = gb + ngap * (rows + (int)jA);
                        if (okA) __hip_atomic_store((gu64*)(p.bot_gran + jA), ((u64)p.bot_tag << 32) | (u64)(u32)((int)o.gla - zl), __ATOMIC_RELAXED, __HIP_MEMORY_SCOPE_SYSTEM);
                        if (okB) __hip_atomic_store((gu64*)(p.bot_gran + jB), ((u64)p.bot_tag << 32) | (u64)(u32)((int)o.glb - zl - ngap), __ATOMIC_RELAXED, __HIP_MEMORY_SCOPE_SYSTEM);
                        if (s == 0 && lane == 0) __hip_atomic_store((gu64*)p.bot_gran, (u64)p.bot_tag << 32, __ATOMIC_RELAXED, __HIP_MEMORY_SCOPE_SYSTEM);
                        if (p.bot_done) {
                            __builtin_amdgcn_fence(__ATOMIC_RELEASE, "");
                            asm volatile("s_waitcnt vmcnt(0)" ::: "memory");
                            const int n63 = (int)((p.cols + 62) / 63);
                            if (lane < 2 && 2 * s + lane < n63)
                                __hip_atomic_store((gu32*)(p.bot_done + 2 * s + lane), p.bot_tag, __ATOMIC_RELAXED, __HIP_MEMORY_SCOPE_SYSTEM);
                        }
                    }
                }
                if (best > 0 && !nostore) {
                    if (trk) {
                        bestrow = bestq * SY_U + 1 + (bestcode >> 1);
                        bestcol = bestcode & 1;
                    } else {
                        __builtin_amdgcn_s_waitcnt(0);
                        const u32 psz = h64 ? 16u : 8u, span = h64 ? 880u : 440u, lc = psz * (u32)(lane - 1);
                        const u32 f0 = (u32)(((uint64_t)(uintptr_t)H + (uint64_t)(((((int64_t)bestq * SY_U + 1) * M + (int64_t)s * W + 1) * 4) << hsh)) & 63u);
                        auto inwin = [&](u32 rowoff, u32 pc) { return (u32)(pc - ((f0 + rowoff + pc) & 63u)) < span; };
                        const int nk = min(SY_U, rows - bestq * SY_U);
                        int hvA[SY_U], hvB[SY_U];
#pragma unroll
                        for (int k = 0; k < SY_U; ++k) {
                            const int64_t o = (int64_t)(bestq * SY_U + 1 + min(k, nk - 1)) * M + jA;
                            hvA[k] = (int)__builtin_nontemporal_load(&H[o << hsh]);
                            hvB[k] = (int)__builtin_nontemporal_load(&H[(o + 1) << hsh]);
                        }
#pragma unroll
                        for (int k = SY_U - 1; k >= 0; --k) {
                            bool stA = k < nk, stB = k < nk;
                            if (wl) {
                                const u32 rowoff = (u32)k * rowbH;
                                if (allod || (k & 1)) { stA = stA && inwin(rowoff, lc - psz / 2); stB = stB && lane < 63 && inwin(rowoff, lc + psz / 2); }
                                else stA = stB = stA && inwin(rowoff, lc);
                            }
                            if (stB && hvB[k] == best) { bestrow = bestq * SY_U + 1 + k; bestcol = 1; }
                            if (stA && hvA[k] == best) { bestrow = bestq * SY_U + 1 + k; bestcol = 0; }
                        }
                        if (bestrow == 0 && wlaunch) best = 0;
                    }
                }
            } else
            for (int q = q_lo + k9; q < nblk; q += nc_eff) {
                const int r0 = q * SY_U + 1;
                const int need = r0 + SY_U - 1 + 63 + phi;
                while (lds_load(&sd.prod_u) < need)
                    if (spin.fail(p.abort_flag)) return;
                asm volatile("" ::: "memory");
                u32 gA[SY_U + 1], gB[SY_U + 1];
                const u32 e0 = (u32)(r0 - 2 + lane + phi);
                if ((((u32)(r0 - 2 + phi) & (SY_R - 1)) + 63 + SY_U) < (u32)SY_R) {
                    const u32* qa = rA + (e0 & (SY_R - 1));
                    const u32* qb = rB + (e0 & (SY_R - 1));
#pragma unroll
                    for (int k = 0; k <= SY_U; ++k) {
                        gA[k] = __hip_atomic_load(qa + k, __ATOMIC_RELAXED, __HIP_MEMORY_SCOPE_WORKGROUP);
                        gB[k] = __hip_atomic_load(qb + k, __ATOMIC_RELAXED, __HIP_MEMORY_SCOPE_WORKGROUP);
                    }
                } else {
#pragma unroll
                    for (int k = 0; k <= SY_U; ++k) {
                        gA[k] = __hip_atomic_load(rA + ((e0 + k) & (SY_R - 1)), __ATOMIC_RELAXED, __HIP_MEMORY_SCOPE_WORKGROUP);
                        gB[k] = __hip_atomic_load(rB + ((e0 + k) & (SY_R - 1)), __ATOMIC_RELAXED, __HIP_MEMORY_SCOPE_WORKGROUP);
                    }
                }
                asm volatile("" ::: "memory");
                lds_store(&lds.cons_blk[k9], q);
                if (q == 0) {
                    gA[0] = (u32)(gb + ngap * (int)jA);
                    gB[0] = (u32)(gb + ngap * (int)jB);
                }
                const uint4 ch = *(const uint4*)(bchars + r0 - 1);
                const u32 chw[4] = {ch.x, ch.y, ch.z, ch.w};
                const int nbr = min(SY_U, rows - r0 + 1), nrec = nbr == SY_U ? 0x7FFFFF00 : nbr * (int)rowb;
                const __amdgpu_buffer_rsrc_t rH = __builtin_amdgcn_make_buffer_rsrc((void*)(H + (int64_t)r0 * M), 0, nrec, 0x00020000);
                const __amdgpu_buffer_rsrc_t rP = __builtin_amdgcn_make_buffer_rsrc((void*)((int32_t*)P + (int64_t)r0 * M), 0, nrec, 0x00020000);
                typedef int v2i __attribute__((ext_vector_type(2)));
                u32 zA = (u32)(gb + ngap * (r0 - 1 + (int)jA));
                int hAs[SY_U], hBs[SY_U];
#pragma unroll
                for (int k = 0; k < SY_U; ++k) {
                    const int c = (int)((chw[k >> 2] >> (8 * (k & 3))) & 0xffu);
                    zA += (u32)ngap;
                    const u32 zB = zA + (u32)ngap;
                    const u32 bl = (u32)__builtin_amdgcn_update_dpp(0, (int)gB[k], 0x138, 0xf, 0xf, false);
                    const u32 dA = bl + (u32)(aA == c ? mm : xm), dB = gA[k] + (u32)(aB == c ? mm : xm);
                    const int hA = (int)(gA[k + 1] - zA), hB = (int)(gB[k + 1] - zB);
                    int pA = (gA[k] == gA[k + 1]) ? 1 : 2, pB = (gB[k] == gB[k + 1]) ? 1 : 2;
                    pA = (dA == gA[k + 1]) ? 3 : pA;
                    pB = (dB == gB[k + 1]) ? 3 : pB;
                    pA = hA == 0 ? 0 : pA;
                    pB = hB == 0 ? 0 : pB;
                    v2i hv = {hA, hB}, pv = {pA, pB};
                    __builtin_amdgcn_raw_buffer_store_b64(hv, rH, (int)voff2, (int)(rowb * (u32)k), 0);
                    __builtin_amdgcn_raw_buffer_store_b64(pv, rP, (int)voff2, (int)(rowb * (u32)k), 0);
                    if (tail1) {
                        __builtin_amdgcn_raw_buffer_store_b32(hA, rH, (int)voff1, (int)(rowb * (u32)k), 0);
                        __builtin_amdgcn_raw_buffer_store_b32(pA, rP, (int)voff1, (int)(rowb * (u32)k), 0);
                    }
                    hAs[k] = okA ? hA : 0;
                    hBs[k] = okB ? hB : 0;
                }
                int bm = 0;
#pragma unroll
                for (int k = 0; k < SY_U; ++k) bm = max(bm, max(hAs[k], hBs[k]));
                if (__builtin_amdgcn_ballot_w64(bm > best) != 0) {
                    if (bm > best) {
                        best = bm;
#pragma unroll
                        for (int k = SY_U - 1; k >= 0; --k) {
                            if (hBs[k] == bm) { bestrow = r0 + k; bestcol = 1; }
                            if (hAs[k] == bm) { bestrow = r0 + k; bestcol = 0; }
                        }
                    }
                }
            }
            if (best > 0) atomicMax(p.result_key, ((u64)(u32)best << 40) | (SW_KEY_IDX_MASK - (u64)((int64_t)bestrow * M + jA + bestcol + p.idx_off)));
        } else if (importer) {
            S2Pace pace;
            if (p.filler_hop_ps > 0 && nscout > 0 && !p.top_gran && !sf) {
                pace.on = true;
                pace.bps = s2_stride<OV>() * ((H ? (h64 ? 8 : 4) : 0) + (P ? (p8 ? 1 : 4) : 0));
                pace.steps = UT + 64;
                pace.S = S; pace.s = s;
                if (s == 0) pace.calibrate(p, 0.f);
            }
            if (!s2_importer<OV>(sd, p, s, phi, UT, rows, gb, ngap, lane, false, pace)) return;
        }
        __syncthreads();
    }
}

template <int NC, bool OV>
__global__ void __launch_bounds__(768) sw_systolic2(const unsigned char* seq_a, const unsigned char* seq_b, FillParams p) {
    __shared__ Sys2Lds lds;
    __shared__ S2Prep prep;
    const int nl = s2_prologue(prep, p, seq_a, seq_b);
    if (nl >= 0 && nl <= 7) {
        const unsigned char* mine = p.priv + (int64_t)blockIdx.x * p.priv_stride;
        s2_body<NC, OV>(lds, prep.tab, mine, mine + p.bpad_pstride, seq_a, p);
    }
    s2_epilogue(p, nl <= 7);
}
template __global__ void sw_systolic2<4, false>(const unsigned char*, const unsigned char*, FillParams);
template __global__ void sw_systolic2<4, true>(const unsigned char*, const unsigned char*, FillParams);
template __global__ void sw_systolic2<5, false>(const unsigned char*, const unsigned char*, FillParams);
template __global__ void sw_systolic2<5, true>(const unsigned char*, const unsigned char*, FillParams);
template __global__ void sw_systolic2<6, false>(const unsigned char*, const unsigned char*, FillParams);
template __global__ void sw_systolic2<6, true>(const unsigned char*, const unsigned char*, FillParams);
template __global__ void sw_systolic2<7, false>(const unsigned char*, const unsigned char*, FillParams);
template __global__ void sw_systolic2<7, true>(const unsigned char*, const unsigned char*, FillParams);
```

Before: 334.7 GCUPS.

## Split tail strips into row bands restarted from scout checkpoints by helper blocks

Scouts write periodic per-lane checkpoints of the DP boundary state every band_rows rows. Blocks that finish early then act as helpers and compute later row bands of the last strips, restarting from those checkpoints. A planner model picks the start strip and helper count, and enables banding only when its predicted end time beats the existing split scheme. The aim is to shorten the serial tail of the wavefront where late strips keep few CUs busy, at the cost of checkpoint stores, extra restart steps per band and more synchronisation complexity.

```diff
diff --git a/smith-waterman_amd/csrc/sw_api.hip b/smith-waterman_amd/csrc/sw_api.hip
--- a/smith-waterman_amd/csrc/sw_api.hip
+++ b/smith-waterman_amd/csrc/sw_api.hip
@@ -176,6 +176,8 @@
     if (!strcmp(name, "s2w")) { if (v != 0 && v != 126 && v != 110) return SW_EINVAL; c->opt.s2w = v; return SW_OK; }
     if (!strcmp(name, "split_blk")) { c->opt.split_blk = v > 0 ? v : 0; return SW_OK; }
     if (!strcmp(name, "split_from")) { c->opt.split_from = v > 0 ? v : 0; return SW_OK; }
+    if (!strcmp(name, "band_rows")) { c->opt.band_rows = v; return SW_OK; }
+    if (!strcmp(name, "band_from")) { c->opt.band_from = v > 0 ? v : 0; return SW_OK; }
     if (!strcmp(name, "debug_epoch8")) { c->epoch8 = (unsigned)(v & 255); return SW_OK; }
     if (!strcmp(name, "engine")) {
         if (v != 0 && v != 1) { set_err("engine must be 0 (systolic) or 1 (strip_scan)"); return SW_EINVAL; }
@@ -209,6 +211,9 @@
     if (!strcmp(name, "last_xcd_mode")) return last_tile.xcd_mode;
     if (!strcmp(name, "last_tiles")) return c->last_plan.ntile;
     if (!strcmp(name, "last_split_from")) return last_tile.split_blk ? last_tile.split_from : 0;
+    if (!strcmp(name, "last_band_rows")) return last_tile.band_rows;
+    if (!strcmp(name, "last_band_from")) return last_tile.band_rows ? last_tile.band_from : 0;
+    if (!strcmp(name, "last_band_helpers")) return last_tile.band_rows ? last_tile.band_helpers : 0;
     if (!strcmp(name, "xcd_round_robin")) return c->xcd_round_robin ? 1 : 0;
     if (!strcmp(name, "last_batch_kernel")) return c->last_batch_kernel;
     if (!strcmp(name, "last_search_grid")) return c->last_search_grid;
@@ -438,6 +443,9 @@
             p2.nscout = t.nscout; p2.scout_double = t.scout_double; p2.xcd_mode = t.xcd_mode;
             p2.split_blk = t.split_blk; p2.split_from = t.split_from; p2.split_extra = t.split_extra;
             p2.filler_end_steps = t.filler_end_steps; p2.filler_full_steps = t.filler_full_steps;
+            p2.band_rows = t.band_rows; p2.band_from = t.band_from; p2.band_nb = t.band_nb; p2.band_helpers = t.band_helpers;
+            p2.band_scout_tau_ps = t.band_scout_tau_ps;
+            p2.ckpt = c->d_edge4 + plan.ckpt_off; p2.ckpt_stride = (int64_t)plan.ckpt_stride;
             p2.filler_hop_ps = t.filler_hop_ps; p2.filler_tau_ps = t.filler_tau_ps; p2.filler_bw_gbs = t.filler_bw_gbs;
             p2.sync = c->d_sync; p2.priv = c->d_priv; p2.priv_stride = plan.priv_stride;
             p2.bpad16_w = d_cb16; p2.bpad8_w = c->d_cb; p2.bcode_w = d_cbc; p2.atab_w = c->d_alpha + 64;
diff --git a/smith-waterman_amd/csrc/sw_debug.h b/smith-waterman_amd/csrc/sw_debug.h
--- a/smith-waterman_amd/csrc/sw_debug.h
+++ b/smith-waterman_amd/csrc/sw_debug.h
@@ -30,6 +30,7 @@
     DBG_NO_XCD_DEALING = 1 << 23,
     DBG_S2_IMPORTERS = 3 << 24,
     DBG_NO_PACING = 1 << 27,
+    DBG_NO_BANDS = 1 << 28,
 };
 constexpr int DBG_S2_IMPORTERS_SHIFT = 24;
 constexpr int DBG_BATCH_MASK = DBG_NO_STORES | DBG_PRODUCER_ONLY | DBG_GENERIC_PRODUCER;
diff --git a/smith-waterman_amd/csrc/sw_filler_producer.inc b/smith-waterman_amd/csrc/sw_filler_producer.inc
--- a/smith-waterman_amd/csrc/sw_filler_producer.inc
+++ b/smith-waterman_amd/csrc/sw_filler_producer.inc
@@ -1,6 +1,6 @@
 __device__ __forceinline__ int producer_perm2(u32 palo, u32 pahi, u32 pblo, u32 pbhi, u32 ngap_v, u32 wA, u32 wB, u32 voff, u32 z0, u32 ga1, u32 gb1, u32 ta,
                                               u32 tb, u32 expoff, u32 expoff_local, const unsigned char* cbase, u32 hb, u32 lowb, u32 cons_addr, u32 right_addr,
-                                              u32 prog_addr, int UT, int kc, int kr, sw_i32x4p erc, int (&polls)[2]) {
+                                              u32 prog_addr, int UT, int kc, int kr, sw_i32x4p erc, int (&polls)[2], int u0 = 0) {
     int status;
     const int kc32 = kc + 32, kr32 = kr + 32;
     asm volatile(
@@ -8,22 +8,24 @@
         "s_mov_b32 %[status], 0\n\t"
         "s_mov_b32 s94, 0\n\t"
         "s_mov_b32 s95, 0\n\t"
-        "s_mov_b32 s88, 1\n\t"
-        "s_mov_b32 s90, 0\n\t"
-        "s_mov_b32 s91, 0\n\t"
-        "s_mov_b32 s75, 0\n\t"
+        "s_add_i32 s88, %[u0], 1\n\t"
+        "s_lshl_b32 s75, %[u0], 2\n\t"
+        "s_and_b32 s90, s75, 1023\n\t"
+        "s_and_b32 s91, s75, 4095\n\t"
         "s_mov_b32 s76, %[e0]\n\t"
         "s_mov_b32 s77, %[e1]\n\t"
         "s_mov_b32 s78, %[e2]\n\t"
         "s_mov_b32 s79, %[e3]\n\t"
         "s_mov_b64 s[72:73], 1\n\t"
         "s_mov_b64 s[92:93], %[cbase]\n\t"
+        "s_add_u32 s92, s92, %[u0]\n\t"
+        "s_addc_u32 s93, s93, 0\n\t"
         "v_mov_b32 v96, %[voff]\n\t"
         "v_mov_b32 v97, %[expoff]\n\t"
         "v_mov_b32 v39, %[consaddr]\n\t"
         "v_mov_b32 v30, %[rightaddr]\n\t"
         "v_mov_b32 v31, %[progaddr]\n\t"
-        "v_mov_b32 v29, 0\n\t"
+        "v_mov_b32 v29, %[u0]\n\t"
         "v_mov_b32 v79, %[ga1]\n\t"
         "v_mov_b32 v95, %[gb1]\n\t"
         "v_mov_b32 v117, %[ta]\n\t"
@@ -86,7 +88,7 @@
         : [palo] "v"(palo), [pahi] "v"(pahi), [pblo] "v"(pblo), [pbhi] "v"(pbhi), [ngap] "v"(ngap_v), [wa] "v"(wA), [wb] "v"(wB), [voff] "v"(voff),
           [z0] "v"(z0), [ga1] "v"(ga1), [gb1] "v"(gb1), [ta] "v"(ta), [tb] "v"(tb), [expoff] "v"(expoff), [expoffl] "v"(expoff_local), [cbase] "s"(cbase), [hb] "s"(hb), [lowb] "s"(lowb),
           [consaddr] "s"(cons_addr), [rightaddr] "s"(right_addr), [progaddr] "s"(prog_addr), [ut] "s"(UT), [kc] "s"(kc), [kr] "s"(kr), [kc32] "s"(kc32),
-          [kr32] "s"(kr32), [e0] "s"(erc.x), [e1] "s"(erc.y), [e2] "s"(erc.z), [e3] "s"(erc.w)
+          [kr32] "s"(kr32), [e0] "s"(erc.x), [e1] "s"(erc.y), [e2] "s"(erc.z), [e3] "s"(erc.w), [u0] "s"(u0)
         : "vcc", "scc", "memory", "s72", "s73", "s75", "s76", "s77", "s78", "s79", "s85", "s86", "s87", "s88", "s89", "s90", "s91", "s92", "s93", "s94", "s95",
           "v27", "v28", "v29", "v30", "v31", "v32", "v33", "v34", "v35", "v36", "v37", "v38", "v39", "v40", "v41", "v42", "v43", "v44", "v45", "v46", "v47", "v48",
           "v49", "v50", "v51", "v52", "v53", "v54", "v55", "v56", "v57", "v58", "v59", "v60", "v61", "v62", "v63", "v64", "v65", "v66", "v67", "v68", "v69", "v70",
diff --git a/smith-waterman_amd/csrc/sw_kernels.h b/smith-waterman_amd/csrc/sw_kernels.h
--- a/smith-waterman_amd/csrc/sw_kernels.h
+++ b/smith-waterman_amd/csrc/sw_kernels.h
@@ -68,7 +68,12 @@
     int filler_end_steps;
     int filler_full_steps;
     int s2w;
+    unsigned int* ckpt;
+    int64_t ckpt_stride;
+    int band_rows, band_from, band_nb, band_helpers;
+    int band_scout_tau_ps;
 };
+constexpr int SW_CKPT_DWORDS = 5 * 64;
 constexpr int SW_XTAB_OFF = 448;
 constexpr int SW_PERM_PAD = -100;
 
diff --git a/smith-waterman_amd/csrc/sw_plan.cpp b/smith-waterman_amd/csrc/sw_plan.cpp
--- a/smith-waterman_amd/csrc/sw_plan.cpp
+++ b/smith-waterman_amd/csrc/sw_plan.cpp
@@ -18,6 +18,8 @@
 constexpr int64_t kXcdChainStrips = 384;
 constexpr double kScoutLeadSec = 21.5e-9;
 constexpr int64_t kSplitRows = 4096;
+constexpr double kScoutRowSec = 20e-9;
+constexpr int64_t kBandRows = 2048, kBandRestartSteps = 128, kBandAutoRows = 12288;
 
 constexpr int64_t kC4Cols = 256, kC8Cols = 512;
 constexpr int64_t kBndSlackRows = 160;
@@ -49,6 +51,40 @@
     return r;
 }
 
+double band_model_end(int64_t S2, int64_t rows16, int64_t R, int64_t from, int64_t helpers, double hop, double tf) {
+    const int64_t nb = (rows16 + R - 1) / R, K = S2 - from, jobs = K * (nb - 1);
+    const double whole = (double)(rows16 + 190) * tf;
+    double end = (double)(from - 1) * hop + whole;
+    end = std::max(end, (double)(S2 - 1) * hop + (double)(R + kBandRestartSteps) * tf);
+    double freeat[256];
+    for (int64_t h = 0; h < helpers; ++h) freeat[h] = (double)h * hop + whole;
+    for (int64_t j = 0; j < jobs; ++j) {
+        const int64_t b = 1 + j / K, s = from + j % K, h = j % helpers;
+        const double ready = (double)s * hop + (double)(b * R) * kScoutRowSec;
+        const double e = std::max(freeat[h], ready) + (double)(std::min(R, rows16 - b * R) + kBandRestartSteps) * tf;
+        freeat[h] = e;
+        end = std::max(end, e);
+    }
+    return end;
+}
+
+}
+
+int band_task_count(const TilePlan& t) { return t.band_rows > 0 ? (int)(t.strips - t.band_from) * (t.band_nb - 1) : 0; }
+
+void band_tasks(const TilePlan& t, int64_t rows, const PlanOptions& o, BandTask* out) {
+    const int64_t K = t.strips - t.band_from, rows16 = (rows + 15) / 16 * 16;
+    const double hop = (double)o.filler_hop_ps * 1e-12, tf = (double)o.filler_tau_ps * 1e-12;
+    double freeat[256];
+    for (int h = 0; h < t.band_helpers; ++h) freeat[h] = (double)h * hop + (double)(rows16 + 190) * tf;
+    for (int j = 0; j < band_task_count(t); ++j) {
+        BandTask& k = out[j];
+        k.band = 1 + (int)(j / K); k.strip = t.band_from + (int)(j % K); k.helper = j % t.band_helpers;
+        k.ready = (double)k.strip * hop + (double)((int64_t)k.band * t.band_rows) * kScoutRowSec;
+        k.start = std::max(freeat[k.helper], k.ready);
+        k.end = k.start + (double)(std::min<int64_t>(t.band_rows, rows16 - (int64_t)k.band * t.band_rows) + kBandRestartSteps) * tf;
+        freeat[k.helper] = k.end;
+    }
 }
 
 FillPlan plan_fill(const PlanJob& j, const DeviceFacts& dev, const PlanOptions& o) {
@@ -184,6 +220,42 @@
                 }
             }
         }
+        if (t.xcd_mode == 1 && !j.has_top && !j.has_top_gran && !j.has_bot_gran && o.filler_hop_ps > 0 && o.band_rows != 0 && S2 <= 256 && f.ntile == 1 &&
+            !(o.debug_flags & (DBG_NO_PACING | DBG_NO_BANDS))) {
+            const Deal d = deal_per_xcd(S2, true);
+            const double hop = (double)o.filler_hop_ps * 1e-12, tf = (double)o.filler_tau_ps * 1e-12;
+            const int64_t rows16 = (rows + 15) / 16 * 16;
+            const int64_t R = std::max<int64_t>(64, ((o.band_rows > 0 ? o.band_rows : kBandRows) + 63) / 64 * 64);
+            const int64_t nb = (rows16 + R - 1) / R;
+            int64_t from = 0, helpers = 0;
+            double best = 0;
+            if (d.fits && nb >= 2 && o.band_rows > 0) {
+                from = std::min<int64_t>(S2 - 1, std::max<int64_t>(1, o.band_from));
+                helpers = std::min<int64_t>(from, (S2 - from) * (nb - 1));
+                best = band_model_end(S2, rows16, R, from, helpers, hop, tf);
+            } else if (d.fits && nb >= 2 && rows >= kBandAutoRows) {
+                for (int64_t k = 8; k <= 64 && k < S2 - 8; k += 8)
+                    for (int64_t div = 1; div <= 4; div *= 2) {
+                        const int64_t fr = S2 - k, hl = std::max<int64_t>(1, std::min<int64_t>(fr / div, k * (nb - 1)));
+                        const double e = band_model_end(S2, rows16, R, fr, hl, hop, tf);
+                        if (from == 0 || e < best) { best = e; from = fr; helpers = hl; }
+                    }
+                t.split_end_sec = (double)(S2 - 1) * hop + (double)(t.split_blk > 0 ? t.filler_end_steps : rows16 + 190) * tf;
+                if (from > 0 && !(best < t.split_end_sec)) from = 0;
+            }
+            if (from > 0) {
+                t.band_rows = (int)R; t.band_from = (int)from; t.band_nb = (int)nb; t.band_helpers = (int)helpers;
+                t.band_scout_tau_ps = (int)(kScoutRowSec * 1e12);
+                t.band_end_sec = best;
+                t.split_blk = 0; t.split_from = 0; t.split_extra = 1;
+                t.nscout = d.scouts; t.scout_double = d.doubles;
+                t.filler_full_steps = (int)(rows16 + 190) / 64 * 64;
+                t.filler_end_steps = (int)std::max<int64_t>(R + kBandRestartSteps, (int64_t)((best - (double)(S2 - 1) * hop) / tf));
+                f.ckpt_stride = (size_t)((rows16 + 190) / R + 1) * 320;
+                f.ckpt_off = f.edge4_need;
+                f.edge4_need += f.ckpt_stride * (size_t)S2;
+            }
+        }
         const bool xcd_chain_pays = S2 >= kXcdChainStrips && W2 != 110;
         if (!scouts && dev.xcd_round_robin && t.grid >= 64 && !(o.debug_flags & DBG_NO_XCD_DEALING) &&
             (o.xcd_chain == 1 || (o.xcd_chain == 0 && xcd_chain_pays)))
diff --git a/smith-waterman_amd/csrc/sw_plan.h b/smith-waterman_amd/csrc/sw_plan.h
--- a/smith-waterman_amd/csrc/sw_plan.h
+++ b/smith-waterman_amd/csrc/sw_plan.h
@@ -41,6 +41,7 @@
 struct PlanOptions {
     int64_t engine = 0, strips_per_group = 0, consumers = 0, importers = 0, max_blocks = 0, waves_per_block = 4, store_policy = 0;
     int64_t s2w = 0, xcd_chain = 0, split_blk = 0, split_from = 0;
+    int64_t band_rows = 0, band_from = 0;
     int64_t filler_hop_ps = 2400000, filler_tau_ps = 25000, filler_bw_gbs = 4200;
     int64_t probe_foreign_pairs = 0, debug_flags = 0;
 };
@@ -50,6 +51,8 @@
     int grid = 0, nscout = 0, scout_double = 0, xcd_mode = 0;
     int split_blk = 0, split_from = 0, split_extra = 0, filler_end_steps = 0, filler_full_steps = 0;
     int filler_hop_ps = 0, filler_tau_ps = 0, filler_bw_gbs = 0;
+    int band_rows = 0, band_from = 0, band_nb = 0, band_helpers = 0, band_scout_tau_ps = 0;
+    double band_end_sec = 0, split_end_sec = 0;
     int store_nt = 0;
     int consumers = 0;
 };
@@ -72,11 +75,16 @@
     TilePlan tile[kMaxTiles];
     int64_t priv_stride = 0;
     size_t edge_need = 0, cb_need = 0, edge4_need = 0, priv_need = 0;
+    size_t ckpt_off = 0, ckpt_stride = 0;
     size_t h_bytes = 0, p_bytes = 0;
     bool probe_pair_class = false;
 };
 
 FillPlan plan_fill(const PlanJob& job, const DeviceFacts& dev, const PlanOptions& opt);
+
+struct BandTask { int strip, band, helper; double ready, start, end; };
+int band_task_count(const TilePlan& t);
+void band_tasks(const TilePlan& t, int64_t rows, const PlanOptions& opt, BandTask* out);
 
 struct BatchJob {
     int64_t cols = 0, rows = 0, npairs = 1;
diff --git a/smith-waterman_amd/csrc/sw_scout_producer.inc b/smith-waterman_amd/csrc/sw_scout_producer.inc
--- a/smith-waterman_amd/csrc/sw_scout_producer.inc
+++ b/smith-waterman_amd/csrc/sw_scout_producer.inc
@@ -1,5 +1,6 @@
 __device__ __forceinline__ int P2S_FN(u32 palo, u32 pahi, u32 pblo, u32 pbhi, u32 ngap_v, u32 voff, u32 z0, u32 ga1, u32 gb1, u32 ta, u32 tb,
-                                               u32 expoff, const unsigned char* cbase, u32 hb, u32 lowb, u32 prog_addr, int UT, sw_i32x4p erc, int (&polls)[2]) {
+                                               u32 expoff, const unsigned char* cbase, u32 hb, u32 lowb, u32 prog_addr, int UT, sw_i32x4p erc, int (&polls)[2],
+                                               int ck_next, int ck_every, u32 ckoff, sw_i32x4p crc) {
     int status;
     asm volatile(
         "s_setprio 3\n\t"
@@ -13,8 +14,12 @@
         "s_mov_b32 s78, %[e2]\n\t"
         "s_mov_b32 s79, %[e3]\n\t"
         "s_mov_b64 s[72:73], 1\n\t"
-        "s_mov_b32 s70, 0\n\t"
-        "s_mov_b32 s71, 0x80000000\n\t"
+        "s_mov_b32 s70, %[cknext]\n\t"
+        "s_mov_b32 s71, 0\n\t"
+        "s_mov_b32 s80, %[c0]\n\t"
+        "s_mov_b32 s81, %[c1]\n\t"
+        "s_mov_b32 s82, %[c2]\n\t"
+        "s_mov_b32 s83, %[c3]\n\t"
         "v_mov_b32 v26, %[hb]\n\t"
         "v_add_u32 v26, 0x8000, v26\n\t"
         "v_add_u32 v25, 0x800, v26\n\t"
@@ -63,6 +68,16 @@
         "s_add_u32 s92, s92, 64\n\t"
         "s_addc_u32 s93, s93, 0\n\t"
         "s_add_i32 s88, s88, 64\n\t"
+        "s_cmp_lg_u32 s88, s70\n\t"
+        "s_cbranch_scc1 Lnock_%=\n\t"
+        "buffer_store_dword v79, %[ckoff], s[80:83], s71 offen sc1\n\t"
+        "buffer_store_dword v95, %[ckoff], s[80:83], s71 offen offset:256 sc1\n\t"
+        "buffer_store_dword v117, %[ckoff], s[80:83], s71 offen offset:512 sc1\n\t"
+        "buffer_store_dword v119, %[ckoff], s[80:83], s71 offen offset:768 sc1\n\t"
+        "buffer_store_dword v121, %[ckoff], s[80:83], s71 offen offset:1024 sc1\n\t"
+        "s_add_i32 s70, s70, %[ckevery]\n\t"
+        "s_add_i32 s71, s71, 1280\n"
+        "Lnock_%=:\n\t"
         "s_cmp_gt_i32 s88, %[ut]\n\t"
         "s_cbranch_scc0 Lchunk_%=\n\t"
         "s_branch Lexit_%=\n"
@@ -76,8 +91,9 @@
         : [status] "=&s"(status), [nhalo] "=&s"(polls[1])
         : [palo] "v"(palo), [pahi] "v"(pahi), [pblo] "v"(pblo), [pbhi] "v"(pbhi), [ngap] "v"(ngap_v), [voff] "v"(voff),
           [z0] "v"(z0), [ga1] "v"(ga1), [gb1] "v"(gb1), [ta] "v"(ta), [tb] "v"(tb), [expoff] "v"(expoff), [cbase] "s"(cbase), [hb] "s"(hb), [lowb] "s"(lowb),
-          [progaddr] "s"(prog_addr), [ut] "s"(UT), [e0] "s"(erc.x), [e1] "s"(erc.y), [e2] "s"(erc.z), [e3] "s"(erc.w)
-        : "vcc", "scc", "memory", "s70", "s71", "s72", "s73", "s75", "s76", "s77", "s78", "s79", "s85", "s86", "s88", "s89", "s91", "s92", "s93", "s95",
+          [progaddr] "s"(prog_addr), [ut] "s"(UT), [e0] "s"(erc.x), [e1] "s"(erc.y), [e2] "s"(erc.z), [e3] "s"(erc.w),
+          [cknext] "s"(ck_next), [ckevery] "s"(ck_every), [ckoff] "v"(ckoff), [c0] "s"(crc.x), [c1] "s"(crc.y), [c2] "s"(crc.z), [c3] "s"(crc.w)
+        : "vcc", "scc", "memory", "s70", "s71", "s72", "s73", "s75", "s76", "s77", "s78", "s79", "s80", "s81", "s82", "s83", "s85", "s86", "s88", "s89", "s91", "s92", "s93", "s95",
           "v20", "v21", "v22", "v23", "v25", "v26", "v27", "v28", "v29", "v31", "v40", "v41", "v42", "v43", "v44", "v45", "v46", "v47", "v48",
           "v49", "v50", "v51", "v52", "v53", "v54", "v55", "v56", "v57", "v58", "v59", "v60", "v61", "v62", "v63", "v64", "v65", "v66", "v67", "v68", "v69", "v70",
           "v71", "v72", "v73", "v74", "v75", "v76", "v77", "v78", "v79", "v80", "v81", "v82", "v83", "v84", "v85", "v86", "v87", "v88", "v89", "v90", "v91", "v92",
diff --git a/smith-waterman_amd/csrc/sw_systolic2.inc b/smith-waterman_amd/csrc/sw_systolic2.inc
--- a/smith-waterman_amd/csrc/sw_systolic2.inc
+++ b/smith-waterman_amd/csrc/sw_systolic2.inc
@@ -338,7 +338,7 @@
 }
 
 struct S2Pace {
-    bool on = false, set = false;
+    bool on = false, set = false, helper = false;
     int S = 0, s = 0, steps = 0, bps = 0;
     float inv = 0.f, start = 0.f;
     __device__ __forceinline__ void calibrate(const FillParams& p, float t_first) {
@@ -353,14 +353,15 @@
         const float d_chain = (float)(S - 1) * hop + esteps * tau_min;
         const float x = bw_per_tick * hop / ((float)max(bps, 1) * wsteps);
         const float d_bw = (x < 20.f) ? (float)S * hop / (1.f - __expf(-x)) : 0.f;
-        const float d = fmaxf(d_chain, d_bw);
+        float d = fmaxf(d_chain, d_bw);
+        if (helper) d = fminf(d, (float)(p.band_from + s) * hop + (float)p.band_rows * (float)p.band_scout_tau_ps * 1e-4f);
         inv = (d > start + 1.f) ? fsteps / (d - start) : 0.f;
         set = true;
     }
 };
 template <bool OV>
 __device__ __forceinline__ bool s2_importer(S2Side& sd, const FillParams& p, int s_real, int phi, int UT, int rows, int gb, int ngap, int lane, bool synth = false,
-                                            S2Pace pace = S2Pace(), int stop_u = 0x7fffffff) {
+                                            S2Pace pace = S2Pace(), int stop_u = 0x7fffffff, int u0 = 0) {
     const int s = synth ? 0 : s_real;
     __builtin_amdgcn_s_setprio(2);
     const u32 row0v = (u32)(gb + sd.topv[0] + ngap * s_real * s2_stride<OV>());
@@ -368,7 +369,7 @@
     const int ulast = min(UT + 64, stop_u);
     const u32 tag = (u32)gb >> 24;
     const u32* e4 = (s > 0) ? p.edge4 + (int64_t)(s - 1) * p.e4stride : nullptr;
-    int impu = 1;
+    int impu = u0 + 1;
     bool wide = true;
     Spin spin; spin.code = 3;
     const uint64_t pace_t0 = __builtin_amdgcn_s_memrealtime();
@@ -435,7 +436,7 @@
 template <bool SCOUT, bool LOCAL, bool OV>
 __device__ __forceinline__ int s2_produce(S2Side& sd, Sys2Lds* full, const FillParams& p, const unsigned char* seq_a, const unsigned char* ltab,
                                           const unsigned char* bcode, int s, int S, int phi, int UT, int lane, int gb, int ngap, int mm, int xm, bool exports,
-                                          bool local_rt = false, bool stamps_as_scout = false, int ua = -1) {
+                                          bool local_rt = false, bool stamps_as_scout = false, int ua = -1, int u0 = 0, bool last_task = true) {
     const int jA = s * s2_stride<OV>() + 2 * lane - 1, jB = jA + 1;
     const int topA = lane >= 1 ? sd.topv[2 * lane - 1] : 0, topB = sd.topv[2 * lane];
     const int jn = jA + 2;
@@ -458,26 +459,58 @@
         const u32 pad4 = 0x01010101u * (u32)(unsigned char)(signed char)SW_PERM_PAD;
         pblo = pad4; pbhi = pad4;
     }
-    const u32 ga1 = lane == 0 ? (u32)gb : (u32)(gb + topA + ngap * (int)jA), gb1 = (u32)(gb + topB + ngap * (int)jB);
-    const u32 z0 = (u32)(gb + ngap * (1 - phi - lane + (int)jA));
+    u32 ga1 = lane == 0 ? (u32)gb : (u32)(gb + topA + ngap * (int)jA), gb1 = (u32)(gb + topB + ngap * (int)jB);
+    u32 z0 = (u32)(gb + ngap * (1 - phi - lane + (int)jA));
+    u32 ta1 = ga1 + (u32)SW_PERM_PAD, tb1 = gb1 + (u32)SW_PERM_PAD;
+    int ck_next = 0x7fffffff, ck_band = 0;
+    sw_i32x4p crc = {0, 0, 0, 0x00020000};
+    if (p.band_rows > 0 && s >= p.band_from) {
+        const int off = phi >= 1 ? (phi - 1) / 64 * 64 : -64;
+        const uint64_t cb = (uint64_t)(uintptr_t)(p.ckpt + (int64_t)s * p.ckpt_stride);
+        if constexpr (SCOUT) {
+            const int skip = (p.band_rows + off <= 0) ? 1 : 0;
+            const uint64_t cb1 = cb + (uint64_t)skip * (SW_CKPT_DWORDS * 4);
+            ck_next = __builtin_amdgcn_readfirstlane((1 + skip) * p.band_rows + off + 1);
+            crc.x = __builtin_amdgcn_readfirstlane((int)(u32)cb1); crc.y = __builtin_amdgcn_readfirstlane((int)(u32)(cb1 >> 32));
+            crc.z = __builtin_amdgcn_readfirstlane((int)((p.ckpt_stride - skip * SW_CKPT_DWORDS) * 4));
+        } else if (u0 > 0) {
+            ck_band = (u0 - off) / p.band_rows;
+            const u32* ck = p.ckpt + (int64_t)s * p.ckpt_stride + (int64_t)(ck_band - 1) * SW_CKPT_DWORDS + lane;
+            const u32 tag = (u32)gb >> 24;
+            Spin spin; spin.code = 18;
+            for (;;) {
+                ga1 = __hip_atomic_load((gu32*)ck, __ATOMIC_RELAXED, __HIP_MEMORY_SCOPE_AGENT);
+                gb1 = __hip_atomic_load((gu32*)(ck + 64), __ATOMIC_RELAXED, __HIP_MEMORY_SCOPE_AGENT);
+                ta1 = __hip_atomic_load((gu32*)(ck + 128), __ATOMIC_RELAXED, __HIP_MEMORY_SCOPE_AGENT);
+                tb1 = __hip_atomic_load((gu32*)(ck + 192), __ATOMIC_RELAXED, __HIP_MEMORY_SCOPE_AGENT);
+                z0 = __hip_atomic_load((gu32*)(ck + 256), __ATOMIC_RELAXED, __HIP_MEMORY_SCOPE_AGENT);
+                const bool ok = (ga1 >> 24) == tag && (gb1 >> 24) == tag && (ta1 >> 24) == tag && (tb1 >> 24) == tag && (z0 >> 24) == tag;
+                if (__builtin_amdgcn_ballot_w64(!ok) == 0) break;
+                if (spin.fail(p.abort_flag)) return 1;
+                __builtin_amdgcn_s_sleep(16);
+            }
+        }
+    }
     const unsigned char* cbase = bcode + (p.bfront - phi - 64);
     const u32 expoff = (exports && s + 1 < S && lane == s2_xlane<OV>()) ? 0u : SY_OOB;
     const uint64_t eb = (uint64_t)(uintptr_t)(p.edge4 + (int64_t)s * p.e4stride);
     const sw_i32x4p erc = {(int)(u32)eb, (int)(u32)(eb >> 32), 0x7FFFFF00, 0x00020000};
     int polls[2];
     u64* const dbg = p.dbg ? p.dbg + ((!SCOUT && p.nscout > 0 && !stamps_as_scout) ? 6 * p.nstrips + 32 : 0) : nullptr;
-    if (dbg && lane == 0) {
+    if (dbg && lane == 0 && u0 == 0) {
         dbg[2 * s] = __builtin_amdgcn_s_memrealtime();
         if (s == 0 && dbg == p.dbg) p.dbg[6 * p.nstrips + 16] = __builtin_amdgcn_s_memtime();
     }
     int st;
     if constexpr (SCOUT) {
         if constexpr (LOCAL) {
-            st = producer_scout2_local(palo, pahi, pblo, pbhi, (u32)ngap, 63u - (u32)lane, z0, ga1, gb1, ga1 + (u32)SW_PERM_PAD, gb1 + (u32)SW_PERM_PAD, expoff, cbase,
-                                       (u32)(size_t)&sd.halo[0], (u32)(size_t)&sd.lowv[0], (u32)(size_t)&sd.prod_u, UT, erc, polls);
+            st = producer_scout2_local(palo, pahi, pblo, pbhi, (u32)ngap, 63u - (u32)lane, z0, ga1, gb1, ta1, tb1, expoff, cbase,
+                                       (u32)(size_t)&sd.halo[0], (u32)(size_t)&sd.lowv[0], (u32)(size_t)&sd.prod_u, UT, erc, polls, ck_next, p.band_rows,
+                                       (u32)lane * 4u, crc);
         } else
-            st = producer_scout2(palo, pahi, pblo, pbhi, (u32)ngap, 63u - (u32)lane, z0, ga1, gb1, ga1 + (u32)SW_PERM_PAD, gb1 + (u32)SW_PERM_PAD, expoff, cbase,
-                                 (u32)(size_t)&sd.halo[0], (u32)(size_t)&sd.lowv[0], (u32)(size_t)&sd.prod_u, UT, erc, polls);
+            st = producer_scout2(palo, pahi, pblo, pbhi, (u32)ngap, 63u - (u32)lane, z0, ga1, gb1, ta1, tb1, expoff, cbase,
+                                 (u32)(size_t)&sd.halo[0], (u32)(size_t)&sd.lowv[0], (u32)(size_t)&sd.prod_u, UT, erc, polls, ck_next, p.band_rows,
+                                 (u32)lane * 4u, crc);
     } else {
         const u32 wA = (u32)(size_t)&full->ringA[0] + (u32)lane * (u32)SY_LSTR, wB = (u32)(size_t)&full->ringB[0] + (u32)lane * (u32)SY_LSTR;
         const int kc = 30 - SY_R - phi, kr = -SY_R - phi - 32;
@@ -486,11 +519,11 @@
                                      local_rt ? SY_OOB : expoff, local_rt ? expoff : SY_OOB, cbase, (u32)(size_t)&sd.halo[0], (u32)(size_t)&sd.lowv[0],
                                      (u32)(size_t)&full->cons_blk[0], (u32)(size_t)&sd.never, (u32)(size_t)&sd.prod_u, ua, UT, kc, kr, erc, polls);
         else
-        st = producer_perm2(palo, pahi, pblo, pbhi, (u32)ngap, wA, wB, 63u - (u32)lane, z0, ga1, gb1, ga1 + (u32)SW_PERM_PAD, gb1 + (u32)SW_PERM_PAD,
+        st = producer_perm2(palo, pahi, pblo, pbhi, (u32)ngap, wA, wB, 63u - (u32)lane, z0, ga1, gb1, ta1, tb1,
                             local_rt ? SY_OOB : expoff, local_rt ? expoff : SY_OOB, cbase, (u32)(size_t)&sd.halo[0], (u32)(size_t)&sd.lowv[0],
-                            (u32)(size_t)&full->cons_blk[0], (u32)(size_t)&sd.never, (u32)(size_t)&sd.prod_u, UT, kc, kr, erc, polls);
-    }
-    if (dbg && lane == 0) {
+                            (u32)(size_t)&full->cons_blk[0], (u32)(size_t)&sd.never, (u32)(size_t)&sd.prod_u, UT, kc, kr, erc, polls, u0);
+    }
+    if (dbg && lane == 0 && last_task) {
         dbg[2 * s + 1] = __builtin_amdgcn_s_memrealtime();
         if (s == 0 && dbg == p.dbg) p.dbg[6 * p.nstrips + 17] = __builtin_amdgcn_s_memtime();
         if (dbg == p.dbg) {
@@ -726,7 +759,10 @@
     const int split_blk = (p.xcd_mode == 1) ? p.split_blk : 0;
     bool sf = false;
     if (split_blk > 0 && sc_cnt == 1 && sc_s0 >= p.split_from) { sf = true; fill_s = sc_s0; fill_step = S; sc_cnt = 0; }
-    else if (sc_cnt == 1 && sc_s0 == S - 1) return;
+    else if (sc_cnt == 1 && sc_s0 == S - 1 && p.band_rows == 0) return;
+
+    const int band_rows = (p.xcd_mode == 1) ? p.band_rows : 0;
+    const int band_k = S - p.band_from, band_jobs = band_rows > 0 ? band_k * (p.band_nb - 1) : 0;
 
     if (sc_cnt) {
         S2Side* sides = (S2Side*)&lds;
@@ -750,7 +786,7 @@
             const int UT = ((rows + SY_U - 1) / SY_U * SY_U + 63 + phi + 63) / 64 * 64;
             if (producer) {
                 bool local = false;
-                if (p.xcd_mode == 1 && s != sc_far && my_xcc == (blockIdx.x & 7u)) {
+                if (p.xcd_mode == 1 && s != sc_far && my_xcc == (blockIdx.x & 7u) && !(band_rows > 0 && s + 1 >= p.band_from)) {
                     Spin spin; spin.code = 16;
                     if (!xcd_local_readers(p, S, s, my_xcc, sc_far_block, spin, local)) return;
                 }
@@ -777,11 +813,21 @@
     const int nc_eff = NC;
     const bool producer = wave == 0, consumer = off0 && k9 < nc_eff, importer = off0 && k9 >= nc_eff;
 
-    for (int s = fill_s; s < S; s += fill_step) {
+    const bool helper = band_jobs > 0 && fill_s < p.band_helpers;
+    int job = -1;
+    for (int s = fill_s; s < S;) {
         const int nblk_all = (rows + SY_U - 1) / SY_U;
         const bool upper = split_blk > 0 && !sf && s >= p.split_from && strip_has_single_scout(S, s, p.split_extra);
-        const int q_lo = sf ? min(split_blk, nblk_all) : 0, q_hi = upper ? min(split_blk, nblk_all) : nblk_all;
-        if (threadIdx.x == 0) { sd.prod_u = 0; sd.halo_ready = 1; sd.never = 0x7fffffff; }
+        int q_lo = sf ? min(split_blk, nblk_all) : 0, q_hi = upper ? min(split_blk, nblk_all) : nblk_all;
+        int u0 = 0;
+        if (band_rows > 0 && s >= p.band_from) {
+            const int b = job < 0 ? 0 : 1 + job / band_k;
+            const int ph = S - 1 - s;
+            q_lo = b * (band_rows / SY_U);
+            q_hi = min(q_lo + band_rows / SY_U, nblk_all);
+            if (b > 0) u0 = b * band_rows + (ph >= 1 ? (ph - 1) / 64 * 64 : -64);
+        }
+        if (threadIdx.x == 0) { sd.prod_u = u0; sd.halo_ready = 1; sd.never = 0x7fffffff; }
         if (threadIdx.x < 8) lds.cons_blk[threadIdx.x] = ((int)threadIdx.x < nc_eff) ? q_lo - 1 : 0x7fffffff;
         for (int i = threadIdx.x; i < SY_RH; i += blockDim.x) sd.halo[i] = 0u;
         if (threadIdx.x < 128) sd.lowv[threadIdx.x] = (u32)gb;
@@ -818,7 +864,7 @@
                 if (!xcd_local_readers(p, S, s, my_xcc, sc_far_block, spin, local)) return;
             }
             const int st = s2_produce<false, false, OV>(sd, &lds, p, seq_a, ltab, my_bcode, s, S, phi, UT, lane, gb, ngap, mm, xm, nscout == 0 || sf, local, sf,
-                                             sf ? max(0, (q_lo * SY_U + phi - 1) / 64 * 64) : -1);
+                                             sf ? max(0, (q_lo * SY_U + phi - 1) / 64 * 64) : -1, u0, q_hi == nblk_all);
             if (st) {
                 __hip_atomic_store((gu32*)p.abort_flag, 16u, __ATOMIC_RELAXED, __HIP_MEMORY_SCOPE_AGENT);
                 return;
@@ -1042,16 +1088,23 @@
             if (best > 0) atomicMax(p.result_key, ((u64)(u32)best << 40) | (SW_KEY_IDX_MASK - (u64)((int64_t)bestrow * M + jA + bestcol + p.idx_off)));
         } else if (importer) {
             S2Pace pace;
-            if (p.filler_hop_ps > 0 && nscout > 0 && !p.top_gran && !sf) {
+            if (p.filler_hop_ps > 0 && nscout > 0 && !p.top_gran && !sf && job < 0) {
                 pace.on = true;
                 pace.bps = s2_stride<OV>() * ((H ? (h64 ? 8 : 4) : 0) + (P ? (p8 ? 1 : 4) : 0));
                 pace.steps = UT + 64;
                 pace.S = S; pace.s = s;
+                pace.helper = helper;
                 if (s == 0) pace.calibrate(p, 0.f);
             }
-            if (!s2_importer<OV>(sd, p, s, phi, UT, rows, gb, ngap, lane, false, pace)) return;
+            if (!s2_importer<OV>(sd, p, s, phi, UT, rows, gb, ngap, lane, false, pace, 0x7fffffff, u0)) return;
         }
         __syncthreads();
+        if (helper) {
+            job = job < 0 ? fill_s : job + p.band_helpers;
+            if (job >= band_jobs) break;
+            s = p.band_from + job % band_k;
+        } else
+            s += fill_step;
     }
 }
 
```

Result: slower. 328.2 GCUPS (-1.9%).
